# ray-project/xgboost_ray

Measured on NVIDIA H100. Metric: boosting rounds/sec, higher is better.
Workload: dtype int64 fixed-point histograms (int32 shared-memory cells), f64 gain

## Files before the change

xgboost_ray_b200/build.py:

```python
import os
import subprocess
import sys
from concurrent.futures import ThreadPoolExecutor

HERE = os.path.dirname(os.path.abspath(__file__))
CSRC = os.path.join(HERE, "csrc")
OUT = os.path.join(HERE, "libb2hist.so")
OBJ_DIR = os.path.join(CSRC, "build")

NVCC = os.environ.get("NVCC", "/usr/local/cuda/bin/nvcc")
COMMON = ["-gencode", "arch=compute_90a,code=sm_90a", "-O3", "-lineinfo", "-std=c++17",
          "-Xcompiler", "-fPIC,-ffp-contract=off", "-ccbin", "/usr/bin/g++"]
SOURCES = {
    "hist_kernel.cu": [],
    "hist_tma_kernel.cu": [],
    "split_kernel.cu": ["--fmad=false"],
    "partition_kernel.cu": ["--fmad=false"],
    "control_kernel.cu": ["--fmad=false"],
    "objective_kernel.cu": ["--fmad=false"],
    "sketch.cu": ["--fmad=false"],
    "auc_kernel.cu": ["--fmad=false"],
    "p2p_exchange.cu": [],
    "shap_kernel.cu": [],
    "engine.cu": [],
}


def _stale(target, deps):
    if not os.path.exists(target):
        return True
    t = os.path.getmtime(target)
    return any(os.path.getmtime(d) > t for d in deps)


def build(force=False, verbose=False):
    os.makedirs(OBJ_DIR, exist_ok=True)
    headers = [os.path.join(CSRC, "common.cuh"), os.path.join(CSRC, "hist_common.cuh"), os.path.join(CSRC, "sampling.cuh"), os.path.join(CSRC, "p2p.cuh"), os.path.join(CSRC, "level_finalize.cuh"), os.path.join(HERE, "..", "include", "b2hist.h"), __file__]
    jobs = []
    objs = []
    for src, extra in SOURCES.items():
        sp = os.path.join(CSRC, src)
        op = os.path.join(OBJ_DIR, src.replace(".cu", ".o"))
        objs.append(op)
        if force or _stale(op, [sp] + headers):
            jobs.append([NVCC] + COMMON + extra + ["-c", sp, "-o", op])

    def run(cmd):
        if verbose:
            print(" ".join(cmd), flush=True)
        r = subprocess.run(cmd, capture_output=True, text=True)
        if r.returncode != 0:
            raise RuntimeError("nvcc failed:\n%s\n%s\n%s" % (" ".join(cmd), r.stdout, r.stderr))
        return r

    with ThreadPoolExecutor(max_workers=6) as ex:
        list(ex.map(run, jobs))
    if force or jobs or _stale(OUT, objs):
        run([NVCC, "-shared", "-o", OUT] + objs + ["-ldl", "-ccbin", "/usr/bin/g++"])
    return OUT


if __name__ == "__main__":
    print(build(force="--force" in sys.argv, verbose=True))
```

xgboost_ray_b200/csrc/common.cuh:

```cuda
#pragma once
#include <cuda_runtime.h>
#include <stdint.h>

#define B2_GROUP_SLOTS 32
#define B2_BINS 256
#define B2_MISSING_BIN 255
#define B2_PLANE_ELEMS (B2_BINS * B2_GROUP_SLOTS)
#define B2_GROUP_ELEMS (2 * B2_PLANE_ELEMS)

struct B2HistWork {
  int32_t seg_begin;
  int32_t seg_count;
  int32_t hist_index;
  int32_t chunk_begin;
};

#define B2_HIST_MAX_TYPES 8
struct B2HistPlan {
  int32_t n_types;
  int32_t cta_begin[B2_HIST_MAX_TYPES + 1];
  int32_t narrow_w;
};

struct B2SplitWork {
  int32_t seg_begin, seg_count;
  int32_t feature;
  int32_t split_bin;
  int32_t default_left;
  int32_t has_missing;
  int32_t chunk_begin;
  int32_t is_cat;
  uint32_t cat_bits[8];
};

struct B2SplitCand {
  float loss_chg;
  int32_t feature;
  int32_t bin;
  int32_t default_left;
  int64_t left_g, left_h;
  uint32_t order;
  int32_t is_cat;
  uint32_t cat_bits[8];
};

struct B2EvalNode {
  int64_t sum_g, sum_h;
  int32_t hist_index;
  float root_gain;
};

struct B2TreeNodeDev {
  int32_t left, right;
  int32_t feature;
  float cond;
  float value;
  int32_t default_left;
  int32_t cat_slot;
  int32_t pad;
};

#define B2_SHAP_MAX_PATH 16
#define B2_PATH_MISSING_OK 1u
#define B2_PATH_HAS_HI 2u
#define B2_PATH_OUTSIDE_OK 4u
struct B2PathElem {
  int32_t feature;
  int32_t cat_slot;
  float lo, hi;
  uint32_t flags;
  uint32_t pad;
  double zero_fraction;
};
struct B2PathInfo {
  int32_t elem_begin;
  int32_t len;
  int32_t cls;
  int32_t pad;
  double value;
};

__device__ __forceinline__ int b2_tree_step(const B2TreeNodeDev& nd, float v, float missing, int missing_is_nan,
                                            const uint32_t* __restrict__ cat_table) {
  const bool miss = isnan(v) || (!missing_is_nan && v == missing);
  if (miss) return nd.default_left ? nd.left : nd.right;
  if (nd.cat_slot >= 0) {
    bool in_set = false;
    if (v >= 0.0f && v < 256.0f) { const int c = (int)v; in_set = (cat_table[(size_t)nd.cat_slot * 8 + (c >> 5)] >> (c & 31)) & 1u; }
    return in_set ? nd.right : nd.left;
  }
  return v < nd.cond ? nd.left : nd.right;
}

__device__ __forceinline__ int b2_tree_leaf(const B2TreeNodeDev* __restrict__ tn, const float* __restrict__ x, float missing,
                                            int missing_is_nan, const uint32_t* __restrict__ cat_table, float* leaf_value) {
  int nid = 0;
  B2TreeNodeDev nd = tn[0];
  while (nd.feature >= 0) {
    nid = b2_tree_step(nd, x[nd.feature], missing, missing_is_nan, cat_table);
    nd = tn[nid];
  }
  *leaf_value = nd.value;
  return nid;
}

struct B2LevelCtl {
  int32_t n_nodes;
  int32_t n_split;
  int32_t part_chunks;
  int32_t hist_n_work;
  int32_t hist_total_chunks;
  int32_t hist_chunk_rows;
  int32_t n_pairs;
  int32_t leaf_base_next;
};
struct B2NodeSeg { int32_t nid, begin, count, buf; };
struct B2LeafDev { int32_t nid, buf, begin, count; };
struct B2SegWork {
  int32_t seg_begin, seg_count, id, chunk_begin;
  int32_t buf, pad0, pad1, pad2;
};
struct B2TreeDev {
  int32_t *left, *right, *parent, *feature, *split_bin, *default_left, *split_type;
  uint32_t* cat_bits;
  float* loss_chg;
  long long *sum_g, *sum_h;
  float *leaf_weight, *leaf_value;
  int32_t* n_nodes;
};
struct B2CtlParams { double mcw, lambda, alpha, max_delta_step; float gamma, eta; };

struct B2ColSample {
  const uint8_t* level_mask;
  const uint32_t* fwq;
  double bynode;
  int32_t n_level;
  int32_t n_features;
  uint32_t seed, tree;
};

struct B2FinalizeArgs {
  B2LevelCtl* ctl_nxt;
  B2NodeSeg* seg_nxt;
  B2EvalNode* ev_nxt;
  const int32_t* pair_parent_hist;
  B2HistWork* hist_work;
  int32_t* triples;
  long long* stat_rows;
  uint32_t* done;
  int32_t max_pairs, need_hist, n_streams, window_rows, chunk_rows_override;
};

struct B2SiblingSub {
  const long long* parent_level;
  const int32_t* triples;
  long long* sib_out;
  int32_t sib_base;
};

#define B2_P2P_MAX_WORLD 8
enum { kSlotHist = 0, kSlotCand = 1, kSlotAbsmax = 2, kSlotLeaf = 3, kSlotClose = 4, kP2PSlots = 5 };
struct B2P2P {
  long long* build[B2_P2P_MAX_WORLD];
  B2SplitCand* cands[B2_P2P_MAX_WORLD];
  long long* misc[B2_P2P_MAX_WORLD];
  uint32_t* flags[B2_P2P_MAX_WORLD];
  uint32_t* epoch;
  uint32_t* done;
  uint32_t* err;
  const uint32_t* abort_flag;
  int32_t world, rank;
  int32_t cand_cap, misc_stride;
  long long spin_limit;
};

struct B2TrainParamDev {
  double min_child_weight, lambda, alpha;
  double inv_scale_g, inv_scale_h;
  double max_delta_step;
  int32_t max_cat_to_onehot, max_cat_threshold;
};

#ifdef __CUDACC__
__device__ __forceinline__ double b2_thr_l1(double g, double a) {
  if (g > a) return __dadd_rn(g, -a);
  if (g < -a) return __dadd_rn(g, a);
  return 0.0;
}
__device__ __forceinline__ double b2_calc_weight(double G, double H, double mcw, double lambda, double alpha, double mds) {
  if (H < mcw || H <= 0.0) return 0.0;
  const double t = (alpha == 0.0) ? G : b2_thr_l1(G, alpha);
  double dw = __ddiv_rn(-t, __dadd_rn(H, lambda));
  if (mds != 0.0 && fabs(dw) > mds) dw = copysign(mds, dw);
  return dw;
}
__device__ __forceinline__ double b2_calc_gain(double G, double H, double mcw, double lambda, double alpha, double mds) {
  if (H < mcw || H <= 0.0) return 0.0;
  if (mds == 0.0) {
    const double t = (alpha == 0.0) ? G : b2_thr_l1(G, alpha);
    return __ddiv_rn(__dmul_rn(t, t), __dadd_rn(H, lambda));
  }
  const double w = b2_calc_weight(G, H, mcw, lambda, alpha, mds);
  const double ret = -__dadd_rn(__dmul_rn(__dmul_rn(2.0, G), w), __dmul_rn(__dadd_rn(H, lambda), __dmul_rn(w, w)));
  return alpha == 0.0 ? ret : __dadd_rn(ret, __dmul_rn(alpha, fabs(w)));
}
#endif
```

xgboost_ray_b200/csrc/control_kernel.cu:

```cuda
#include <string.h>

#include <cub/block/block_scan.cuh>

#include "common.cuh"
#include "p2p.cuh"

namespace b2 {

constexpr int kCtlThreads = 1024;
constexpr int kPartChunkRows = 2048;
constexpr int kSplitChunkRows = 8192;

__device__ __forceinline__ double c_calc_gain(double G, double H, const B2CtlParams& p) {
  return b2_calc_gain(G, H, p.mcw, p.lambda, p.alpha, p.max_delta_step);
}
__device__ __forceinline__ float c_calc_weight(double G, double H, const B2CtlParams& p) {
  return __double2float_rn(b2_calc_weight(G, H, p.mcw, p.lambda, p.alpha, p.max_delta_step));
}

struct TileScan {
  typedef cub::BlockScan<int, kCtlThreads> Scan;
  Scan::TempStorage* tmp;
  int carry;
  __device__ TileScan(Scan::TempStorage* t) : tmp(t), carry(0) {}
  __device__ int step(int v) {
    int ex, total;
    Scan(*tmp).ExclusiveSum(v, ex, total);
    __syncthreads();
    int r = carry + ex;
    carry += total;
    return r;
  }
};

__global__ void __launch_bounds__(kCtlThreads)
decide_kernel(B2LevelCtl* __restrict__ ctl_cur, B2LevelCtl* __restrict__ ctl_nxt, const B2NodeSeg* __restrict__ seg_cur,
              B2NodeSeg* __restrict__ seg_nxt, const B2EvalNode* __restrict__ ev_cur, B2EvalNode* __restrict__ ev_nxt,
              const B2SplitCand* __restrict__ cands, int cands_per_node, int cand_ranks, int cand_rank_stride, int can_split,
              B2TreeDev tree,
              B2SplitWork* __restrict__ split_work, int32_t* __restrict__ pair_parent_hist, B2LeafDev* __restrict__ leaves,
              int32_t* __restrict__ n_leaves, const uint8_t* __restrict__ has_missing, const int32_t* __restrict__ qexp,
              int qbits, B2CtlParams p, int32_t* __restrict__ part_counters, const B2SplitCand* __restrict__ local_cands,
              int use_p2p, B2P2P pp) {
  __shared__ typename TileScan::Scan::TempStorage tmp;
  __shared__ int s_node_base, s_leaf_base;
  const int n = ctl_cur->n_nodes;
  if (part_counters) for (int i = threadIdx.x; i < 2 * n; i += kCtlThreads) part_counters[i] = 0;
  if (use_p2p && can_split) {
    constexpr int kWords = sizeof(B2SplitCand) / 8;
    static_assert(sizeof(B2SplitCand) % 8 == 0, "candidates are copied as 64-bit words");
    const uint32_t epoch = p2p_next_epoch(pp, kSlotCand);
    const int total = n * cands_per_node * kWords;
    for (int w = 0; w < pp.world; ++w) {
      long long* dst = reinterpret_cast<long long*>(pp.cands[w] + (size_t)pp.rank * pp.cand_cap);
      for (int t = threadIdx.x; t < total; t += kCtlThreads) st_volatile_u64(dst + t, reinterpret_cast<const long long*>(local_cands)[t]);
    }
    __syncthreads();
    p2p_signal(pp, kSlotCand, epoch);
    p2p_wait(pp, kSlotCand, epoch);
    p2p_finish_single(pp, kSlotCand, epoch);
  }
  const double inv_sg = ldexp(1.0, qexp[0] - qbits), inv_sh = ldexp(1.0, qexp[1] - qbits);
  if (threadIdx.x == 0) { s_node_base = *tree.n_nodes; s_leaf_base = *n_leaves; }
  __syncthreads();
  TileScan scan_split(&tmp), scan_leaf(&tmp), scan_chunks(&tmp);
  for (int base = 0; base < n; base += kCtlThreads) {
    const int i = base + threadIdx.x;
    const bool in = i < n;
    B2SplitCand best; best.feature = -1; best.loss_chg = 0.f; best.order = 0xffffffffu; best.bin = 0; best.default_left = 0;
    best.left_g = 0; best.left_h = 0; best.is_cat = 0;
    B2EvalNode nd; nd.sum_g = 0; nd.sum_h = 0; nd.hist_index = 0; nd.root_gain = 0.f;
    B2NodeSeg sg; sg.nid = 0; sg.begin = 0; sg.count = 0; sg.buf = 0;
    bool expand = false;
    if (in) {
      nd = ev_cur[i]; sg = seg_cur[i];
      if (can_split) {
        for (int w = 0; w < cand_ranks; ++w)
          for (int g = 0; g < cands_per_node; ++g) {
            B2SplitCand c;
            if (use_p2p) {
              constexpr int kW = sizeof(B2SplitCand) / 8;
              const long long* src = reinterpret_cast<const long long*>(cands + (size_t)w * cand_rank_stride + (size_t)i * cands_per_node + g);
#pragma unroll
              for (int t = 0; t < kW; ++t) reinterpret_cast<unsigned long long*>(&c)[t] = ld_volatile_u64(src + t);
            } else c = cands[(size_t)w * cand_rank_stride + (size_t)i * cands_per_node + g];
            if (c.feature < 0) continue;
            if (best.feature < 0 || c.loss_chg > best.loss_chg || (c.loss_chg == best.loss_chg && c.order < best.order)) best = c;
          }
        if (best.feature >= 0)
          expand = best.loss_chg > 1e-6f && best.left_h != 0 && (nd.sum_h - best.left_h) != 0 && !(best.loss_chg < p.gamma);
      }
    }
    const int rank = scan_split.step(expand ? 1 : 0);
    const int lrank = scan_leaf.step((in && !expand) ? 1 : 0);
    const int chunks = expand ? (sg.count + kSplitChunkRows - 1) / kSplitChunkRows : 0;
    const int chunk_begin = scan_chunks.step(chunks);
    if (in && !expand) {
      B2LeafDev lf; lf.nid = sg.nid; lf.buf = sg.buf; lf.begin = sg.begin; lf.count = sg.count;
      leaves[s_leaf_base + lrank] = lf;
    }
    if (expand) {
      const int l = s_node_base + 2 * rank, r = l + 1;
      const int nid = sg.nid;
      tree.left[nid] = l; tree.right[nid] = r; tree.feature[nid] = best.feature; tree.split_bin[nid] = best.bin;
      tree.default_left[nid] = best.default_left; tree.loss_chg[nid] = best.loss_chg;
      tree.split_type[nid] = best.is_cat;
      if (best.is_cat) {
#pragma unroll
        for (int w8 = 0; w8 < 8; ++w8) tree.cat_bits[(size_t)nid * 8 + w8] = best.cat_bits[w8];
      }
      tree.left[l] = -1; tree.right[l] = -1; tree.feature[l] = -1; tree.parent[l] = nid;
      tree.left[r] = -1; tree.right[r] = -1; tree.feature[r] = -1; tree.parent[r] = nid;
      const long long lg = best.left_g, lh = best.left_h, rg = nd.sum_g - lg, rh = nd.sum_h - lh;
      tree.sum_g[l] = lg; tree.sum_h[l] = lh; tree.sum_g[r] = rg; tree.sum_h[r] = rh;
      B2SplitWork sw;
      sw.seg_begin = sg.begin; sw.seg_count = sg.count; sw.feature = best.feature; sw.split_bin = best.bin;
      sw.default_left = best.default_left; sw.has_missing = has_missing[best.feature]; sw.chunk_begin = chunk_begin;
      sw.is_cat = best.is_cat;
#pragma unroll
      for (int w8 = 0; w8 < 8; ++w8) sw.cat_bits[w8] = best.is_cat ? best.cat_bits[w8] : 0u;
      split_work[rank] = sw;
      pair_parent_hist[rank] = nd.hist_index;
      const double GL = __dmul_rn(__ll2double_rn(lg), inv_sg), HL = __dmul_rn(__ll2double_rn(lh), inv_sh);
      const double GR = __dmul_rn(__ll2double_rn(rg), inv_sg), HR = __dmul_rn(__ll2double_rn(rh), inv_sh);
      B2EvalNode el, er;
      el.sum_g = lg; el.sum_h = lh; el.hist_index = -1; el.root_gain = __double2float_rn(c_calc_gain(GL, HL, p));
      er.sum_g = rg; er.sum_h = rh; er.hist_index = -1; er.root_gain = __double2float_rn(c_calc_gain(GR, HR, p));
      ev_nxt[2 * rank] = el; ev_nxt[2 * rank + 1] = er;
      B2NodeSeg sl, sr;
      sl.nid = l; sl.buf = sg.buf ^ 1; sl.begin = sg.begin; sl.count = 0;
      sr.nid = r; sr.buf = sg.buf ^ 1; sr.begin = sg.begin; sr.count = sg.count;
      seg_nxt[2 * rank] = sl; seg_nxt[2 * rank + 1] = sr;
    }
  }
  __syncthreads();
  if (threadIdx.x == 0) {
    const int n_split = scan_split.carry;
    ctl_cur->n_split = n_split; ctl_cur->part_chunks = scan_chunks.carry;
    ctl_cur->leaf_base_next = s_leaf_base + scan_leaf.carry;
    ctl_nxt->n_nodes = 2 * n_split; ctl_nxt->n_split = 0; ctl_nxt->part_chunks = 0;
    ctl_nxt->hist_n_work = 0; ctl_nxt->hist_total_chunks = 0; ctl_nxt->n_pairs = 0;
    *tree.n_nodes = s_node_base + 2 * n_split;
    *n_leaves = s_leaf_base + scan_leaf.carry;
  }
}

__global__ void __launch_bounds__(kCtlThreads)
leaf_plan_kernel(const B2LeafDev* __restrict__ leaves, const int32_t* __restrict__ n_leaves, B2SegWork* __restrict__ work,
                 B2LevelCtl* __restrict__ leaf_ctl) {
  __shared__ typename TileScan::Scan::TempStorage tmp;
  const int n = *n_leaves;
  TileScan scan(&tmp);
  for (int base = 0; base < n; base += kCtlThreads) {
    const int i = base + threadIdx.x;
    int chunks = 0; B2LeafDev lf; lf.nid = 0; lf.buf = 0; lf.begin = 0; lf.count = 0;
    if (i < n) { lf = leaves[i]; chunks = (lf.count + kPartChunkRows - 1) / kPartChunkRows; }
    const int cb = scan.step(chunks);
    if (i < n) {
      B2SegWork w; w.seg_begin = lf.begin; w.seg_count = lf.count; w.id = i; w.chunk_begin = cb; w.buf = lf.buf;
      w.pad0 = lf.nid == 0 ? 1 : 0;
      w.pad1 = w.pad2 = 0; work[i] = w;
    }
  }
  __syncthreads();
  if (threadIdx.x == 0) { leaf_ctl->hist_n_work = n; leaf_ctl->hist_total_chunks = scan.carry; }
}

__global__ void leaf_values_kernel(const B2LeafDev* __restrict__ leaves, const int32_t* __restrict__ n_leaves,
                                   const long long* __restrict__ sums, const int32_t* __restrict__ qexp, int leaf_bits,
                                   B2CtlParams p, float* __restrict__ leaf_value, B2TreeDev tree, int32_t* __restrict__ qexp_out) {
  const int n = *n_leaves;
  if (blockIdx.x == 0 && threadIdx.x < 2) qexp_out[threadIdx.x] = qexp[threadIdx.x];
  const double kg = ldexp(1.0, leaf_bits - qexp[0]), kh = ldexp(1.0, leaf_bits - qexp[1]);
  for (int i = blockIdx.x * blockDim.x + threadIdx.x; i < n; i += gridDim.x * blockDim.x) {
    const double G = __ddiv_rn(__ll2double_rn(sums[2 * i]), kg), H = __ddiv_rn(__ll2double_rn(sums[2 * i + 1]), kh);
    const float w = c_calc_weight(G, H, p);
    const float v = __fmul_rn(w, p.eta);
    leaf_value[i] = v;
    tree.leaf_weight[leaves[i].nid] = w;
    tree.leaf_value[leaves[i].nid] = v;
  }
}

__global__ void tree_init_kernel(B2TreeDev tree, B2LevelCtl* ctl0, B2NodeSeg* seg0, B2EvalNode* ev0, int32_t* n_leaves,
                                 int n_rows, B2HistWork* hist_work0) {
  if (threadIdx.x == 0 && blockIdx.x == 0) {
    B2HistWork hw; hw.seg_begin = 0; hw.seg_count = n_rows; hw.hist_index = 0; hw.chunk_begin = 0; hist_work0[0] = hw;
    ctl0->leaf_base_next = 0;
    *tree.n_nodes = 1; *n_leaves = 0;
    tree.left[0] = -1; tree.right[0] = -1; tree.parent[0] = -1; tree.feature[0] = -1;
    ctl0->n_nodes = 1; ctl0->n_split = 0; ctl0->part_chunks = 0; ctl0->hist_n_work = 0; ctl0->hist_total_chunks = 0;
    ctl0->n_pairs = 0;
    B2NodeSeg s; s.nid = 0; s.buf = 0; s.begin = 0; s.count = n_rows; seg0[0] = s;
    B2EvalNode e; e.sum_g = 0; e.sum_h = 0; e.hist_index = 0; e.root_gain = 0.f; ev0[0] = e;
  }
}

}

extern "C" {
int b2_launch_decide(B2LevelCtl* ctl_cur, B2LevelCtl* ctl_nxt, const B2NodeSeg* seg_cur, B2NodeSeg* seg_nxt,
                     const B2EvalNode* ev_cur, B2EvalNode* ev_nxt, const B2SplitCand* cands, int cands_per_node, int cand_ranks,
                     int cand_rank_stride, int can_split, B2TreeDev tree, B2SplitWork* split_work, int32_t* pair_parent_hist, B2LeafDev* leaves, int32_t* n_leaves,
                     const uint8_t* has_missing, const int32_t* qexp, int qbits, B2CtlParams p, int32_t* part_counters,
                     const B2SplitCand* local_cands, const void* p2p, cudaStream_t s) {
  B2P2P pp;
  if (p2p) pp = *reinterpret_cast<const B2P2P*>(p2p); else memset(&pp, 0, sizeof(pp));
  b2::decide_kernel<<<1, b2::kCtlThreads, 0, s>>>(ctl_cur, ctl_nxt, seg_cur, seg_nxt, ev_cur, ev_nxt, cands, cands_per_node,
                                                 cand_ranks, cand_rank_stride, can_split, tree, split_work, pair_parent_hist, leaves, n_leaves, has_missing, qexp, qbits, p,
                                                 part_counters, local_cands, p2p ? 1 : 0, pp);
  return (int)cudaGetLastError();
}
int b2_launch_leaf_plan(const B2LeafDev* leaves, const int32_t* n_leaves, B2SegWork* work, B2LevelCtl* leaf_ctl, cudaStream_t s) {
  b2::leaf_plan_kernel<<<1, b2::kCtlThreads, 0, s>>>(leaves, n_leaves, work, leaf_ctl);
  return (int)cudaGetLastError();
}
int b2_launch_leaf_values(const B2LeafDev* leaves, const int32_t* n_leaves, const long long* sums, const int32_t* qexp,
                          int leaf_bits, B2CtlParams p, float* leaf_value, B2TreeDev tree, int32_t* qexp_out, cudaStream_t s) {
  b2::leaf_values_kernel<<<8, 256, 0, s>>>(leaves, n_leaves, sums, qexp, leaf_bits, p, leaf_value, tree, qexp_out);
  return (int)cudaGetLastError();
}
int b2_launch_tree_init(B2TreeDev tree, B2LevelCtl* ctl0, B2NodeSeg* seg0, B2EvalNode* ev0, int32_t* n_leaves, int n_rows,
                        B2HistWork* hist_work0, cudaStream_t s) {
  b2::tree_init_kernel<<<1, 32, 0, s>>>(tree, ctl0, seg0, ev0, n_leaves, n_rows, hist_work0);
  return (int)cudaGetLastError();
}
}
```

xgboost_ray_b200/csrc/engine.cu:

```cuda
#include <cuda_runtime.h>
#include <dlfcn.h>
#include <errno.h>
#include <sys/types.h>
#include <sys/uio.h>
#include <math.h>
#include <stdarg.h>
#include <stdio.h>
#include <stdlib.h>
#include <string.h>

#include <algorithm>
#include <atomic>
#include <chrono>
#include <map>
#include <mutex>
#include <set>
#include <string>
#include <thread>
#include <vector>

#include "../../include/b2hist.h"
#include "common.cuh"
#include "sampling.cuh"

extern "C" {
int b2_launch_hist(const uint8_t*, int, const int2*, const int32_t*, const B2HistWork*, int, int, int, int, int, long long*,
                   const B2LevelCtl*, int, int, int, int, cudaStream_t);
int b2_make_bins_tensor_map(void*, const uint8_t*, int64_t, int, int);
int b2_launch_hist_tma(const uint8_t*, int, const void*, const int2*, const int32_t*, const B2HistWork*, int, int, int, int, int, long long*,
                       const B2LevelCtl*, int, int, int64_t, int, cudaStream_t);
int b2_launch_hist_subtract(const long long*, long long*, const int32_t*, int, int64_t, const B2LevelCtl*, cudaStream_t);
int b2_launch_eval_splits(const long long*, int, const B2EvalNode*, int, const int32_t*, const int32_t*, const int32_t*,
                          const uint8_t*, const uint8_t*, const int32_t*, int, B2TrainParamDev, B2SplitCand*, int, const B2LevelCtl*,
                          int, int, B2ColSample, const B2NodeSeg*, B2SiblingSub, cudaStream_t);
int b2_launch_subsample(float2*, int64_t, uint32_t, uint32_t, uint32_t, double, int, cudaStream_t);
int b2_p2p_flag_words(int);
int b2_launch_p2p_reduce_subtract(const void*, const long long*, long long*, const int32_t*, const B2LevelCtl*, int, int, int64_t, int,
                                  cudaStream_t);
int b2_launch_p2p_quant_exponent(const void*, const uint32_t*, int32_t*, cudaStream_t);
int b2_launch_p2p_leaf_sums(const void*, const int32_t*, long long*, cudaStream_t);
int b2_hist_variant();
int b2_launch_p2p_close(const void*, cudaStream_t);
int b2_launch_gather_interleaved_rows(const void*, float*, int, cudaStream_t);
int b2_launch_final_assign(const uint8_t*, int64_t, const int32_t*, const B2SplitWork*, const B2LevelCtl*, int, const float2*,
                           const int32_t*, int, long long*, uint16_t*, int, int, cudaStream_t);
int b2_launch_margin_update(float*, int, int, const uint16_t*, const float*, int64_t, int, cudaStream_t);
int b2_leaf_acc_max_depth();
int b2_launch_leaf_accumulate(const float2*, const uint16_t*, int64_t, int, const int32_t*, int, long long*, int, cudaStream_t);
int b2_gradient_fused_max_classes();
int b2_launch_sum_fixed(const float2*, int64_t, const int32_t*, int, long long*, int, cudaStream_t);
int b2_cat_ctas();
int b2_launch_eval_cat_splits(const long long*, int, const B2EvalNode*, int, const int32_t*, int, const int32_t*, const int32_t*,
                              const int32_t*, int, B2TrainParamDev, B2SplitCand*, int, int, const B2LevelCtl*, int, int,
                              B2ColSample, const B2NodeSeg*, cudaStream_t);
int b2_launch_cat_stats(const float*, int64_t, int, float, const int32_t*, int, int32_t*, int, cudaStream_t);
int b2_launch_root_totals(const long long*, int, B2EvalNode*, const int32_t*, int, B2TrainParamDev, int, long long*, long long*,
                          cudaStream_t);
int b2_part_chunk_rows();
int b2_split_chunk_rows();
int b2_launch_partition(const uint8_t*, int64_t, const int32_t*, int32_t*, const B2SplitWork*, const B2LevelCtl*, int, int32_t*,
                        int, B2FinalizeArgs, int, cudaStream_t);
int b2_launch_leaf_sums(const float2*, const int32_t*, const int32_t*, const void*, const B2LevelCtl*, int, const int32_t*, int,
                        long long*, uint16_t*, int, cudaStream_t);
int b2_launch_pred_update(float*, int, int, const int32_t*, const int32_t*, const void*, const B2LevelCtl*, int, const float*, int,
                          cudaStream_t);
int b2_launch_decide(B2LevelCtl*, B2LevelCtl*, const B2NodeSeg*, B2NodeSeg*, const B2EvalNode*, B2EvalNode*, const B2SplitCand*,
                     int, int, int, int, B2TreeDev, B2SplitWork*, int32_t*, B2LeafDev*, int32_t*, const uint8_t*, const int32_t*, int,
                     B2CtlParams, int32_t*, const B2SplitCand*, const void*, cudaStream_t);
int b2_launch_leaf_plan(const B2LeafDev*, const int32_t*, B2SegWork*, B2LevelCtl*, cudaStream_t);
int b2_launch_leaf_values(const B2LeafDev*, const int32_t*, const long long*, const int32_t*, int, B2CtlParams, float*, B2TreeDev,
                          int32_t*, cudaStream_t);
int b2_launch_tree_init(B2TreeDev, B2LevelCtl*, B2NodeSeg*, B2EvalNode*, int32_t*, int, B2HistWork*, cudaStream_t);
int b2_launch_iota(int32_t*, int64_t, cudaStream_t);
int b2_launch_gradient(int, int, const float*, const float*, const float*, int64_t, float, float, float2*, uint32_t*, uint32_t*, int,
                       cudaStream_t);
int b2_launch_label_check(int, const float*, int64_t, uint32_t*, int, cudaStream_t);
int b2_launch_pack_custom(const float*, const float*, int, int64_t, float2*, int, cudaStream_t);
int b2_launch_absmax(const float2*, int64_t, uint32_t*, int, cudaStream_t);
int b2_launch_quant_exponent(const uint32_t*, int32_t*, cudaStream_t);
int b2_launch_quantize(const float2*, int64_t, const int32_t*, int, int2*, int, cudaStream_t);
int b2_launch_metric(int, int, int, float, const float*, const float*, const float*, int64_t, double*, int, cudaStream_t);
int b2_launch_predict(const float*, int64_t, int, float, const B2TreeNodeDev*, const int32_t*, const uint32_t*, int, int, int, int,
                      float*, int, cudaStream_t);
int b2_launch_fill(float*, int64_t, float, int, cudaStream_t);
size_t b2_shap_contribs_smem(int, int, int);
int b2_launch_shap_contribs(const float*, int64_t, int64_t, int, float, const B2PathElem*, const B2PathInfo*, int, int,
                            const uint32_t*, int, const double*, const float*, float, double*, int, size_t, float*, int, cudaStream_t);
int b2_launch_shap_interactions(const float*, int64_t, int64_t, int, float, const B2PathElem*, const B2PathInfo*, int, int,
                                const uint32_t*, int, const double*, const float*, float, double*, float*, int, cudaStream_t);
int b2_launch_leaf_index(const float*, int64_t, int64_t, int, float, const B2TreeNodeDev*, const int32_t*, const uint32_t*, int, int,
                         float*, int, cudaStream_t);
size_t b2_auc_temp_bytes(int64_t);
int b2_auc_binary(const float*, const float*, const float*, int64_t, void*, size_t, double*, int, cudaStream_t);
int b2_launch_transform(int, int, float*, int64_t, int, cudaStream_t);
int b2_extract_batch();
int b2_launch_extract_keys(const float*, int64_t, int, int, int, float, uint32_t*, int64_t, int, cudaStream_t);
size_t b2_sort_temp_bytes(int64_t);
int b2_sketch_column(const uint32_t*, const int32_t*, uint32_t*, int32_t*, long long*, int64_t, long long, void*, size_t, int32_t*,
                     int32_t*, float*, long long*, int32_t*, long long*, int, float*, int32_t*, float*, int32_t*, int, cudaStream_t);
int b2_launch_weight_absmax(const float*, int64_t, uint32_t*, int, cudaStream_t);
int b2_launch_weight_quantize(const float*, int64_t, int64_t, const uint32_t*, int32_t*, int, cudaStream_t);
int b2_launch_bin(const float*, int64_t, int, float, const int32_t*, const float*, const int32_t*, const uint8_t*, int, uint8_t*,
                  uint8_t*, int64_t, int, cudaStream_t);
}

namespace {

thread_local std::string g_last_error;
struct B2Error { std::string msg; };
[[noreturn]] void fail(const char* fmt, ...) {
  char buf[1024];
  va_list ap; va_start(ap, fmt); vsnprintf(buf, sizeof(buf), fmt, ap); va_end(ap);
  throw B2Error{buf};
}
#define CUDA_CHECK(expr)                                                                       \
  do {                                                                                         \
    cudaError_t e_ = (expr);                                                                   \
    if (e_ != cudaSuccess) fail("CUDA error %s at %s:%d: %s", cudaGetErrorName(e_), __FILE__, __LINE__, cudaGetErrorString(e_)); \
  } while (0)
#define LAUNCH_CHECK(expr)                                                                     \
  do {                                                                                         \
    int e_ = (expr);                                                                           \
    if (e_ != 0) fail("kernel launch failed (%s) at %s:%d", cudaGetErrorString((cudaError_t)e_), __FILE__, __LINE__); \
  } while (0)
#define API_BEGIN try {
#define API_END                                            \
  }                                                        \
  catch (const B2Error& e) { g_last_error = e.msg; return -1; } \
  catch (const std::exception& e) { g_last_error = e.what(); return -1; } \
  return 0;

struct Ctx {
  int device = -1;
  cudaStream_t stream = nullptr;
  int num_sms = 0;
};
std::mutex g_ctx_mu;
std::map<int, Ctx*> g_ctx;
Ctx* get_ctx(int device) {
  std::lock_guard<std::mutex> lk(g_ctx_mu);
  auto it = g_ctx.find(device);
  if (it != g_ctx.end()) { CUDA_CHECK(cudaSetDevice(device)); return it->second; }
  int n = 0;
  cudaError_t e = cudaGetDeviceCount(&n);
  if (e != cudaSuccess || n == 0) fail("no CUDA device available (%s): libb2hist has no CPU fallback", cudaGetErrorString(e));
  if (device < 0 || device >= n) fail("invalid device %d (have %d)", device, n);
  CUDA_CHECK(cudaSetDevice(device));
  Ctx* c = new Ctx();
  c->device = device;
  CUDA_CHECK(cudaStreamCreateWithFlags(&c->stream, cudaStreamNonBlocking));
  cudaDeviceProp prop;
  CUDA_CHECK(cudaGetDeviceProperties(&prop, device));
  if (prop.major != 9 || prop.minor != 0)
    fail("device %d is sm_%d%d; this engine is built for sm_90a (H100) only", device, prop.major, prop.minor);
  c->num_sms = prop.multiProcessorCount;
  g_ctx[device] = c;
  return c;
}

struct DevPool {
  std::mutex mu;
  std::multimap<size_t, void*> free_blocks;
  size_t cached = 0;
};
DevPool g_dev_pool[64];
size_t pool_cap_bytes() {
  static size_t cap = 0;
  if (!cap) { const char* e = getenv("B2_POOL_MAX_GB"); double gb = e ? atof(e) : 24.0; cap = (size_t)(gb < 0 ? 0 : gb * 1e9) + 1; }
  return cap;
}
void pool_trim(DevPool& pool, size_t keep) {
  while (pool.cached > keep && !pool.free_blocks.empty()) {
    auto it = std::prev(pool.free_blocks.end());
    cudaFree(it->second);
    pool.cached -= it->first;
    pool.free_blocks.erase(it);
  }
}
void* pool_alloc(size_t bytes, size_t* got, int* dev_out) {
  int dev = 0; cudaGetDevice(&dev);
  if (dev < 0 || dev >= 64) dev = 0;
  *dev_out = dev;
  bytes = (bytes + 511) & ~(size_t)511;
  DevPool& pool = g_dev_pool[dev];
  {
    std::lock_guard<std::mutex> lk(pool.mu);
    auto it = pool.free_blocks.lower_bound(bytes);
    if (it != pool.free_blocks.end() && it->first <= bytes + bytes / 4 + ((size_t)1 << 20)) {
      void* p = it->second; *got = it->first;
      pool.cached -= it->first;
      pool.free_blocks.erase(it);
      return p;
    }
  }
  void* p = nullptr;
  cudaError_t e = cudaMalloc(&p, bytes);
  if (e != cudaSuccess) {
    cudaGetLastError();
    { std::lock_guard<std::mutex> lk(pool.mu); pool_trim(pool, 0); }
    e = cudaMalloc(&p, bytes);
  }
  if (e != cudaSuccess) { cudaGetLastError(); fail("cudaMalloc of %zu bytes failed: %s", bytes, cudaGetErrorString(e)); }
  *got = bytes;
  return p;
}
void pool_free(void* p, size_t bytes, int dev) {
  if (!p) return;
  if (dev < 0 || dev >= 64) dev = 0;
  DevPool& pool = g_dev_pool[dev];
  std::lock_guard<std::mutex> lk(pool.mu);
  if (bytes > pool_cap_bytes()) { cudaFree(p); return; }
  pool.free_blocks.emplace(bytes, p);
  pool.cached += bytes;
  if (pool.cached > pool_cap_bytes()) pool_trim(pool, pool_cap_bytes() / 2);
}

template <typename T>
struct DevBuf {
  T* p = nullptr;
  size_t cap = 0;
  size_t block_bytes = 0;
  int dev = 0;
  void ensure(size_t n) {
    if (n <= cap) return;
    release();
    size_t got = 0;
    p = (T*)pool_alloc(n * sizeof(T), &got, &dev);
    block_bytes = got;
    cap = n;
  }
  void release() { if (p) pool_free(p, block_bytes, dev); p = nullptr; cap = 0; block_bytes = 0; }
  ~DevBuf() { release(); }
};

struct PinnedPool {
  static constexpr int kWorkers = 16, kSlots = 2;
  static constexpr size_t kSlice = (size_t)8 << 20;
  void* buf[kWorkers][kSlots] = {};
  cudaStream_t stream[kWorkers] = {};
  cudaEvent_t done[kWorkers][kSlots] = {};
  bool ready = false;
  std::mutex mu;
  int n_init = 0;
  void init(int n) {
    for (int w = n_init; w < n; ++w) {
      CUDA_CHECK(cudaStreamCreateWithFlags(&stream[w], cudaStreamNonBlocking));
      for (int k = 0; k < kSlots; ++k) {
        CUDA_CHECK(cudaMallocHost(&buf[w][k], kSlice));
        CUDA_CHECK(cudaEventCreateWithFlags(&done[w][k], cudaEventDisableTiming));
      }
      n_init = w + 1;
    }
  }
};
std::map<int, PinnedPool*> g_pools;

struct UploadSource {
  const void* src = nullptr;
  long long pid = 0;
  uint64_t remote_addr = 0;
  size_t row_bytes = 0, row_stride = 0;
};
bool fetch_slice(const UploadSource& u, void* dst, size_t off, size_t len, std::string* err) {
  if (u.pid == 0) { memcpy(dst, (const char*)u.src + off, len); return true; }
  if (u.row_stride == u.row_bytes) {
    size_t done = 0;
    while (done < len) {
      struct iovec l = {(char*)dst + done, len - done}, r = {(void*)(uintptr_t)(u.remote_addr + off + done), len - done};
      const ssize_t got = process_vm_readv((pid_t)u.pid, &l, 1, &r, 1, 0);
      if (got <= 0) { if (err) *err = std::string("process_vm_readv: ") + strerror(errno); return false; }
      done += (size_t)got;
    }
    return true;
  }
  constexpr size_t kSpan = (size_t)4 << 20;
  static thread_local std::vector<char> scratch;
  if (scratch.size() < kSpan + u.row_stride) scratch.resize(kSpan + u.row_stride);
  const size_t rows_per_batch = std::max<size_t>(1, kSpan / u.row_stride);
  size_t done = 0;
  while (done < len) {
    const size_t pos = off + done, row0 = pos / u.row_bytes;
    const size_t last_byte = std::min(off + len, (row0 + rows_per_batch) * u.row_bytes) - 1;
    const size_t row1 = last_byte / u.row_bytes;
    const size_t span = (row1 - row0) * u.row_stride + u.row_bytes;
    size_t got_total = 0;
    while (got_total < span) {
      struct iovec l = {scratch.data() + got_total, span - got_total};
      struct iovec r = {(void*)(uintptr_t)(u.remote_addr + row0 * u.row_stride + got_total), span - got_total};
      const ssize_t got = process_vm_readv((pid_t)u.pid, &l, 1, &r, 1, 0);
      if (got <= 0) { if (err) *err = std::string("process_vm_readv: ") + strerror(errno); return false; }
      got_total += (size_t)got;
    }
    for (size_t row = row0; row <= row1; ++row) {
      const size_t b0 = std::max(pos, row * u.row_bytes), b1 = std::min(off + len, (row + 1) * u.row_bytes);
      memcpy((char*)dst + (b0 - off), scratch.data() + (row - row0) * u.row_stride + (b0 - row * u.row_bytes), b1 - b0);
    }
    done = std::min(off + len, (row1 + 1) * u.row_bytes) - off;
  }
  return true;
}

void upload_pipelined(Ctx* ctx, void* dst, const UploadSource& u, size_t bytes);
void upload_pipelined(Ctx* ctx, void* dst, const void* src, size_t bytes) {
  UploadSource u; u.src = src;
  upload_pipelined(ctx, dst, u, bytes);
}
void upload_pipelined(Ctx* ctx, void* dst, const UploadSource& u, size_t bytes) {
  const void* src = u.src;
  if (u.pid == 0 && bytes < ((size_t)64 << 20)) {
    if (bytes) CUDA_CHECK(cudaMemcpyAsync(dst, src, bytes, cudaMemcpyHostToDevice, ctx->stream));
    CUDA_CHECK(cudaStreamSynchronize(ctx->stream));
    return;
  }
  PinnedPool* pool;
  {
    std::lock_guard<std::mutex> lk(g_ctx_mu);
    PinnedPool*& p = g_pools[ctx->device];
    if (!p) p = new PinnedPool();
    pool = p;
  }
  std::lock_guard<std::mutex> lk(pool->mu);
  CUDA_CHECK(cudaStreamSynchronize(ctx->stream));
  const size_t n_slices = (bytes + PinnedPool::kSlice - 1) / PinnedPool::kSlice;
  static int n_workers = 0;
  if (n_workers == 0) {
    const char* e = getenv("B2_UPLOAD_WORKERS");
    n_workers = e ? atoi(e) : 8;
    if (n_workers < 1) n_workers = 1;
    if (n_workers > PinnedPool::kWorkers) n_workers = PinnedPool::kWorkers;
  }
  const int W = n_workers;
  pool->init(W);
  std::atomic<int> failed{0};
  std::mutex err_mu; std::string fetch_err;
  auto worker = [&](int w) {
    if (cudaSetDevice(ctx->device) != cudaSuccess) { failed = 1; return; }
    int use = 0;
    for (size_t i = w; i < n_slices; i += W, ++use) {
      const int k = use % PinnedPool::kSlots;
      const size_t off = i * PinnedPool::kSlice, len = std::min(PinnedPool::kSlice, bytes - off);
      if (use >= PinnedPool::kSlots && cudaEventSynchronize(pool->done[w][k]) != cudaSuccess) { failed = 1; return; }
      std::string e;
      if (!fetch_slice(u, pool->buf[w][k], off, len, &e)) { std::lock_guard<std::mutex> lk(err_mu); fetch_err = e; failed = 2; return; }
      if (cudaMemcpyAsync((char*)dst + off, pool->buf[w][k], len, cudaMemcpyHostToDevice, pool->stream[w]) != cudaSuccess ||
          cudaEventRecord(pool->done[w][k], pool->stream[w]) != cudaSuccess) { failed = 1; return; }
    }
    if (cudaStreamSynchronize(pool->stream[w]) != cudaSuccess) failed = 1;
  };
  std::vector<std::thread> th;
  for (int w = 0; w < W; ++w) th.emplace_back(worker, w);
  for (auto& t : th) t.join();
  if (failed.load() == 2) fail("reading the shard out of the driver process failed: %s", fetch_err.c_str());
  if (failed.load()) fail("pipelined host->device upload failed: %s", cudaGetErrorString(cudaGetLastError()));
}

typedef struct ncclComm* ncclComm_t;
typedef struct { char internal[128]; } ncclUniqueId;
enum { kNcclSum = 0, kNcclMax = 2, kNcclMin = 3 };
enum { kNcclUint8 = 1, kNcclInt32 = 2, kNcclUint32 = 3, kNcclInt64 = 4, kNcclUint64 = 5, kNcclFloat32 = 7, kNcclFloat64 = 8 };
struct NcclApi {
  void* lib = nullptr;
  int (*GetUniqueId)(ncclUniqueId*) = nullptr;
  int (*CommInitRank)(ncclComm_t*, int, ncclUniqueId, int) = nullptr;
  int (*AllReduce)(const void*, void*, size_t, int, int, ncclComm_t, cudaStream_t) = nullptr;
  int (*AllGather)(const void*, void*, size_t, int, ncclComm_t, cudaStream_t) = nullptr;
  int (*ReduceScatter)(const void*, void*, size_t, int, int, ncclComm_t, cudaStream_t) = nullptr;
  int (*CommAbort)(ncclComm_t) = nullptr;
  int (*CommDestroy)(ncclComm_t) = nullptr;
  const char* (*GetErrorString)(int) = nullptr;
};
NcclApi* nccl() {
// ... 98 lines not shown
  m->feat_byte.assign(F, 0);
  m->narrow_w = 0;
  const int r = F % B2_GROUP_SLOTS;
  const bool v4_layout = b2_hist_variant() == 4 && F > 96 && F <= 112;
  const bool narrow = (narrow_on || v4_layout) && r > 0 && r <= 16;
  if (narrow) { m->narrow_w = 1; while (m->narrow_w < r) m->narrow_w <<= 1; }
  const int base = F / m->n_groups, rem = F % m->n_groups;
  int f = 0;
  for (int g = 0; g < m->n_groups; ++g) {
    const int sz = narrow ? (g + 1 < m->n_groups ? B2_GROUP_SLOTS : r) : base + (g < rem ? 1 : 0);
    m->group_first[g] = f; m->group_size[g] = sz;
    for (int s = 0; s < sz; ++s) m->feat_byte[f + s] = g * B2_GROUP_SLOTS + s;
    f += sz;
  }
}

template <typename T>
void upload(DevBuf<T>& d, const std::vector<T>& h, cudaStream_t s) {
  d.ensure(h.size() ? h.size() : 1);
  if (!h.empty()) CUDA_CHECK(cudaMemcpyAsync(d.p, h.data(), h.size() * sizeof(T), cudaMemcpyHostToDevice, s));
}

void upload_cuts(Matrix* m) {
  cudaStream_t s = m->ctx->stream;
  m->nbins.resize(m->F);
  for (int f = 0; f < m->F; ++f) m->nbins[f] = m->cut_ptrs[f + 1] - m->cut_ptrs[f];
  upload(m->d_group_first, m->group_first, s); upload(m->d_group_size, m->group_size, s);
  upload(m->d_feat_byte, m->feat_byte, s); upload(m->d_cut_ptrs, m->cut_ptrs, s);
  upload(m->d_cut_vals, m->cut_vals, s); upload(m->d_nbins, m->nbins, s);
  upload(m->d_has_missing, m->has_missing, s);
  if (m->is_cat.empty()) m->is_cat.assign(m->F, 0);
  upload(m->d_is_cat, m->is_cat, s); upload(m->d_cat_feats, m->cat_feats, s);
  CUDA_CHECK(cudaStreamSynchronize(s));
}

void make_cuts(Matrix* m, Comm* comm, int max_bin) {
  Ctx* ctx = m->ctx; cudaStream_t s = ctx->stream;
  if (max_bin < 2 || max_bin > 256) fail("max_bin must be in [2, 256] (uint8 bin matrix), got %d", max_bin);
  if (!m->has_raw) fail("matrix has no raw data to sketch");
  const int world = comm ? comm->world : 1, rank = comm ? comm->rank : 0;
  DevBuf<long long> d_cnt; d_cnt.ensure(2);
  long long h_cnt[2] = {m->n, m->n};
  if (world > 1) {
    CUDA_CHECK(cudaMemcpyAsync(d_cnt.p, h_cnt, sizeof(h_cnt), cudaMemcpyHostToDevice, s));
    allreduce(comm, d_cnt.p, 1, kNcclInt64, kNcclMax, s);
    allreduce(comm, d_cnt.p + 1, 1, kNcclInt64, kNcclSum, s);
    CUDA_CHECK(cudaMemcpyAsync(h_cnt, d_cnt.p, sizeof(h_cnt), cudaMemcpyDeviceToHost, s));
    CUDA_CHECK(cudaStreamSynchronize(s));
  }
  const int64_t n_pad = h_cnt[0], n_total = n_pad * world; const long long n_global = h_cnt[1];
  const int B = b2_extract_batch(); const int F = m->F;
  DevBuf<uint32_t> keys_local, keys_all, keys_sorted;
  DevBuf<int32_t> flags, idx, m_scratch; DevBuf<float> uval; DevBuf<long long> rmin, nvalid;
  DevBuf<int32_t> d_tab;
  DevBuf<uint8_t> temp;
  const size_t nt = (size_t)std::max<int64_t>(n_total, 1);
  keys_local.ensure((size_t)std::max<int64_t>(n_pad, 1) * B);
  if (world > 1) keys_all.ensure(nt);
  keys_sorted.ensure(nt); flags.ensure(nt); idx.ensure(nt); uval.ensure(nt); rmin.ensure(nt); m_scratch.ensure(1); nvalid.ensure(2);
  DevBuf<int32_t> wq_local, wq_all, wq_sorted; DevBuf<long long> wpre; DevBuf<uint32_t> d_wmax;
  const int32_t* wq = nullptr;
  {
    long long h_has[1] = {m->n_weight > 0 ? 1 : 0};
    if (world > 1) {
      CUDA_CHECK(cudaMemcpyAsync(d_cnt.p, h_has, sizeof(h_has), cudaMemcpyHostToDevice, s));
      allreduce(comm, d_cnt.p, 1, kNcclInt64, kNcclMax, s);
      CUDA_CHECK(cudaMemcpyAsync(h_has, d_cnt.p, sizeof(h_has), cudaMemcpyDeviceToHost, s));
      CUDA_CHECK(cudaStreamSynchronize(s));
    }
    if (h_has[0]) {
      if (m->n_weight != m->n) fail("sample weights are set on some ranks only (this rank has %lld for %lld rows)", (long long)m->n_weight, (long long)m->n);
      d_wmax.ensure(2);
      CUDA_CHECK(cudaMemsetAsync(d_wmax.p, 0, 2 * sizeof(uint32_t), s));
      LAUNCH_CHECK(b2_launch_weight_absmax(m->weight.p, m->n, d_wmax.p, ctx->num_sms, s));
      allreduce(comm, d_wmax.p, 2, kNcclUint32, kNcclMax, s);
      uint32_t h_w[2];
      CUDA_CHECK(cudaMemcpyAsync(h_w, d_wmax.p, sizeof(h_w), cudaMemcpyDeviceToHost, s));
      CUDA_CHECK(cudaStreamSynchronize(s));
      if (h_w[1]) fail("sample weights must be finite and non-negative");
      wq_local.ensure((size_t)std::max<int64_t>(n_pad, 1));
      LAUNCH_CHECK(b2_launch_weight_quantize(m->weight.p, m->n, n_pad, d_wmax.p, wq_local.p, ctx->num_sms, s));
      wq = wq_local.p;
      if (world > 1) {
        wq_all.ensure(nt);
        NCCL_CHECK(nccl()->AllGather(wq_local.p, wq_all.p, (size_t)n_pad, kNcclInt32, comm->comm, s));
        wq = wq_all.p;
      }
      wq_sorted.ensure(nt); wpre.ensure(nt);
    }
  }
  const size_t temp_bytes = b2_sort_temp_bytes(n_total > 0 ? n_total : 1);
  temp.ensure(temp_bytes ? temp_bytes : 1);
  const size_t tab_n = (size_t)F * 256 + 3 * (size_t)F;
  d_tab.ensure(tab_n);
  CUDA_CHECK(cudaMemsetAsync(d_tab.p, 0, tab_n * sizeof(int32_t), s));
  float* d_cuts = (float*)d_tab.p; int32_t* d_ncuts = d_tab.p + (size_t)F * 256;
  float* d_mins = (float*)(d_ncuts + F); int32_t* d_hasmiss = d_ncuts + 2 * (size_t)F;
  if (m->is_cat.empty()) m->is_cat.assign(F, 0);
  for (int f0 = 0; f0 < F; f0 += B) {
    const int nf = std::min(B, F - f0);
    bool any_numeric = false;
    for (int j = 0; j < nf; ++j) any_numeric = any_numeric || !m->is_cat[f0 + j];
    if (!any_numeric) continue;
    LAUNCH_CHECK(b2_launch_extract_keys(m->raw.p, m->n, F, f0, nf, m->missing, keys_local.p, n_pad, ctx->num_sms, s));
    for (int j = 0; j < nf; ++j) {
      const int f = f0 + j;
      if (m->is_cat[f]) continue;
      const uint32_t* kin = keys_local.p + (size_t)j * n_pad;
      if (world > 1) {
        NCCL_CHECK(nccl()->AllGather(kin, keys_all.p, (size_t)n_pad, kNcclUint32, comm->comm, s));
        kin = keys_all.p;
        if (f % world != rank) continue;
      }
      LAUNCH_CHECK(b2_sketch_column(kin, wq, keys_sorted.p, wq_sorted.p, wpre.p, n_total, n_global, temp.p, temp_bytes, flags.p, idx.p, uval.p, rmin.p,
                                    m_scratch.p, nvalid.p, max_bin, d_cuts + (size_t)f * 256, d_ncuts + f, d_mins + f,
                                    d_hasmiss + f, ctx->num_sms, s));
    }
  }
  allreduce(comm, d_tab.p, tab_n, kNcclInt32, kNcclSum, s);
  std::vector<int32_t> h_tab(tab_n);
  CUDA_CHECK(cudaMemcpyAsync(h_tab.data(), d_tab.p, tab_n * sizeof(int32_t), cudaMemcpyDeviceToHost, s));
  const int n_cat = (int)m->cat_feats.size();
  std::vector<int32_t> h_cat((size_t)std::max(n_cat, 1) * 3, 0);
  DevBuf<int32_t> d_cat, d_catf;
  if (n_cat > 0) {
    for (int i = 0; i < n_cat; ++i) { h_cat[i * 3] = -1; h_cat[i * 3 + 1] = 0; h_cat[i * 3 + 2] = 0; }
    d_cat.ensure((size_t)n_cat * 3); d_catf.ensure((size_t)n_cat);
    CUDA_CHECK(cudaMemcpyAsync(d_cat.p, h_cat.data(), (size_t)n_cat * 3 * sizeof(int32_t), cudaMemcpyHostToDevice, s));
    CUDA_CHECK(cudaMemcpyAsync(d_catf.p, m->cat_feats.data(), (size_t)n_cat * sizeof(int32_t), cudaMemcpyHostToDevice, s));
    LAUNCH_CHECK(b2_launch_cat_stats(m->raw.p, m->n, F, m->missing, d_catf.p, n_cat, d_cat.p, ctx->num_sms, s));
    allreduce(comm, d_cat.p, (size_t)n_cat * 3, kNcclInt32, kNcclMax, s);
    CUDA_CHECK(cudaMemcpyAsync(h_cat.data(), d_cat.p, (size_t)n_cat * 3 * sizeof(int32_t), cudaMemcpyDeviceToHost, s));
  }
  CUDA_CHECK(cudaStreamSynchronize(s));
  for (int i = 0; i < n_cat; ++i) {
    const int f = m->cat_feats[i], mx = h_cat[i * 3], miss = h_cat[i * 3 + 1];
    if (h_cat[i * 3 + 2] || (miss && mx > 254))
      fail("categorical feature %d: category codes must be integers in [0, %d]%s", f, miss ? 254 : 255,
           miss ? " (the feature has missing values; bin 255 is the missing sentinel)" : "");
    int32_t* t = h_tab.data();
    float* cuts_f = (float*)t + (size_t)f * 256;
    const int nc = mx < 0 ? 1 : mx + 1;
    for (int k = 0; k < nc; ++k) cuts_f[k] = (float)k;
    t[(size_t)F * 256 + f] = nc;
    ((float*)(t + (size_t)F * 256 + F))[f] = -1e-5f;
    t[(size_t)F * 256 + 2 * (size_t)F + f] = miss;
  }
  const float* h_cuts = (const float*)h_tab.data(); const int32_t* h_nc = h_tab.data() + (size_t)F * 256;
  const float* h_mins = (const float*)(h_nc + F); const int32_t* h_hm = h_nc + 2 * (size_t)F;
  m->cut_ptrs.assign(F + 1, 0);
  m->cut_vals.clear(); m->min_vals.assign(h_mins, h_mins + F); m->has_missing.assign(F, 0);
  for (int f = 0; f < F; ++f) {
    if (h_nc[f] < 1 || h_nc[f] > 256) fail("sketch produced %d cuts for feature %d", h_nc[f], f);
    m->cut_ptrs[f + 1] = m->cut_ptrs[f] + h_nc[f];
    m->cut_vals.insert(m->cut_vals.end(), h_cuts + (size_t)f * 256, h_cuts + (size_t)f * 256 + h_nc[f]);
    m->has_missing[f] = h_hm[f] ? 1 : 0;
  }
  m->max_bin = max_bin;
}

void bin_matrix(Matrix* m) {
  Ctx* ctx = m->ctx; cudaStream_t s = ctx->stream;
  setup_groups(m);
  upload_cuts(m);
  m->bins.ensure((size_t)std::max<int64_t>(m->n, 1) * m->row_stride);
  CUDA_CHECK(cudaMemsetAsync(m->bins.p, 0, (size_t)std::max<int64_t>(m->n, 1) * m->row_stride, s));
  m->col_stride = (std::max<int64_t>(m->n, 1) + 127) & ~(int64_t)127;
  m->bins_col.ensure((size_t)m->col_stride * m->F);
  LAUNCH_CHECK(b2_launch_bin(m->raw.p, m->n, m->F, m->missing, m->d_cut_ptrs.p, m->d_cut_vals.p, m->d_feat_byte.p,
                             m->any_cat() ? m->d_is_cat.p : nullptr, m->row_stride, m->bins.p, m->bins_col.p, m->col_stride,
                             ctx->num_sms, s));
  CUDA_CHECK(cudaStreamSynchronize(s));
  m->has_tmap = b2_make_bins_tensor_map(m->tmap_tile, m->bins.p, m->n, m->row_stride, 64) == 0;
  m->quantized = true;
}

enum { kObjSquaredError = 0, kObjLogistic = 1, kObjSoftprob = 2, kObjRegLogistic = 3, kObjLogitRaw = 4, kObjSquaredLog = 5,
       kObjPseudoHuber = 6, kObjPoisson = 7, kObjGamma = 8, kObjTweedie = 9 };
bool obj_log_link(int o) { return o == kObjPoisson || o == kObjGamma || o == kObjTweedie; }
bool obj_sigmoid(int o) { return o == kObjLogistic || o == kObjRegLogistic; }
bool obj_checks_finite(int o) { return o >= kObjSquaredLog; }
struct Params {
  int objective = kObjSquaredError;
  std::string objective_name = "reg:squarederror";
  int num_class = 1;
  int num_parallel_tree = 1;
  int max_depth = 6;
  float eta = 0.3f, gamma = 0.0f, min_child_weight = 1.0f, lambda = 1.0f, alpha = 0.0f, base_score = 0.5f;
  int qbits = 18;
  int hist_chunk_rows = 0;
  int profile = 1;
  int num_feature = 0;
  int device = 0;
  int max_cat_to_onehot = 4, max_cat_threshold = 64;
  float scale_pos_weight = 1.0f, max_delta_step = 0.0f;
  bool max_delta_step_set = false;
  float huber_slope = 1.0f;
  float tweedie_variance_power = 1.5f;
  float subsample = 1.0f, colsample_bytree = 1.0f, colsample_bylevel = 1.0f, colsample_bynode = 1.0f;
  int seed = 0;
  bool base_score_set = false;
  bool use_cols() const { return colsample_bytree < 1.0f || colsample_bylevel < 1.0f || colsample_bynode < 1.0f; }
};

struct TreeHost {
  std::vector<int32_t> left, right, parent, feature, split_bin;
  std::vector<float> cond, value, base_weight, loss_chg;
  std::vector<double> sum_hess;
  std::vector<uint8_t> default_left;
  std::vector<uint8_t> split_type;
  std::vector<uint32_t> cat_bits;
  bool any_cat = false;
  int add(int par) {
    int id = (int)left.size();
    left.push_back(-1); right.push_back(-1); parent.push_back(par); feature.push_back(-1); split_bin.push_back(-1);
    cond.push_back(0.f); value.push_back(0.f); base_weight.push_back(0.f); loss_chg.push_back(0.f); sum_hess.push_back(0.0);
    default_left.push_back(0); split_type.push_back(0); cat_bits.insert(cat_bits.end(), 8, 0u);
    return id;
  }
  int size() const { return (int)left.size(); }
};


struct Timers {
  double hist_ms = 0, round_ms = 0;
  double shap_ms = 0;
  long long shap_rows = 0;
  double phase_ms[8] = {0, 0, 0, 0, 0, 0, 0, 0};
  long long hist_launches = 0, hist_rows = 0, kernel_launches = 0, rounds = 0;
  double hist_bytes = 0, allreduce_bytes = 0;
  void reset() { *this = Timers(); }
};

struct EvalCache { DevBuf<float> margin; int n_trees_applied = 0; int64_t n = 0; uint64_t margin_version = 0; };

struct Booster : HandleBase {
  Ctx* ctx = nullptr;
  Params p;
  Matrix* train = nullptr;
  int n_features = 0;
  Comm* comm = nullptr;
  std::vector<TreeHost> trees;
  std::atomic<bool> cancel{false};
  DevBuf<B2TreeNodeDev> d_nodes; DevBuf<int32_t> d_tree_offset; int d_trees_synced = 0;
  std::vector<B2TreeNodeDev> h_nodes; std::vector<int32_t> h_tree_offset;
  DevBuf<uint32_t> d_cat_table; std::vector<uint32_t> h_cat_table;
  DevBuf<B2PathElem> d_path_elems; DevBuf<B2PathInfo> d_paths; DevBuf<uint32_t> d_path_cats;
  std::vector<int32_t> tree_path_offset;
  std::vector<double> tree_expected;
  int paths_synced = -1;
  bool margin_ready = false;
  DevBuf<float> margin;
  DevBuf<float2> gh;
  DevBuf<float2> gh_round;
  DevBuf<int2> q;
  DevBuf<int32_t> ridx[2];
  DevBuf<long long> hist[2];
  template <typename T> struct View { T* p = nullptr; };
  DevBuf<uint8_t> xarena;
  size_t xoff_cands = 0, xoff_misc = 0, xoff_flags = 0, x_misc_stride = 0;
  View<long long> hist_build;
  View<B2SplitCand> d_cands_all;
  int shards = 1, log2_shards = 0, sp = 32, cpn = 1;
  int cpn_num = 1;
  View<uint32_t> t_cat;
  DevBuf<uint8_t> d_col_masks;
  struct P2PState {
    bool enabled = false, tried = false;
    B2P2P pp;
    DevBuf<uint32_t> words;
    uint32_t* flags = nullptr;
    long long* misc = nullptr;
    std::vector<void*> opened;
    int cand_cap = 0;
  } p2p;
  struct TreeGraph {
    cudaGraphExec_t exec = nullptr;
    std::vector<std::pair<cudaEvent_t, cudaEvent_t>> hist_ev;
    long long hist_launches = 0, kernel_launches = 0;
    double allreduce_bytes = 0;
  };
  std::map<int, TreeGraph> graphs;
  std::map<int, int> direct_trees;
  bool graph_failed = false;
  bool absmax_fused = false;
  bool labels_checked = false;
  DevBuf<uint32_t> d_grad_err;
  uint32_t* h_grad_err = nullptr;
  DevBuf<uint16_t> pos;
  size_t slice_elems = 0;
  size_t node_elems = 0;
  DevBuf<uint32_t> d_absmax; DevBuf<int32_t> d_qexp;
  int ctl_depth = 0;
  DevBuf<uint8_t> t_block;
  View<int32_t> t_i32;
  View<float> t_f32;
  View<long long> t_i64;
  View<int32_t> t_qexp;
  DevBuf<B2LevelCtl> d_ctl;
  DevBuf<B2NodeSeg> d_seg[2]; DevBuf<B2EvalNode> d_ev[2];
  DevBuf<B2HistWork> d_hist_work; DevBuf<B2SplitWork> d_split_work; DevBuf<B2SegWork> d_seg_work;
  DevBuf<B2SplitCand> d_cands; DevBuf<int32_t> d_counters, d_triples, d_pair_parent;
  DevBuf<uint32_t> d_part_done;
  DevBuf<B2LeafDev> d_leaves;
  DevBuf<long long> d_leaf_sums; DevBuf<float> d_leaf_values; DevBuf<double> d_metric;
  std::vector<void*> staging;
  size_t staging_bytes = 0;
  DevBuf<float> d_custom_g, d_custom_h;
  std::map<uint64_t, EvalCache*> eval_cache;
  Timers t;
  std::vector<cudaEvent_t> ev_pool; size_t ev_used = 0;
  std::vector<std::pair<cudaEvent_t, cudaEvent_t>> hist_events;
  std::vector<std::pair<int, cudaEvent_t>> phase_marks;
  cudaEvent_t round_start = nullptr, round_stop = nullptr;
  ~Booster() {
    for (auto& kv : graphs) {
      if (kv.second.exec) cudaGraphExecDestroy(kv.second.exec);
      for (auto& pr : kv.second.hist_ev) { cudaEventDestroy(pr.first); cudaEventDestroy(pr.second); }
    }
    if (ctx) cudaStreamSynchronize(ctx->stream);
    for (void* q : p2p.opened) cudaIpcCloseMemHandle(q);
    for (auto e : ev_pool) cudaEventDestroy(e);
    if (round_start) cudaEventDestroy(round_start);
    if (round_stop) cudaEventDestroy(round_stop);
    for (auto& kv : eval_cache) delete kv.second;
    for (void* h : staging) cudaFreeHost(h);
    if (h_grad_err) cudaFreeHost(h_grad_err);
  }
};

cudaEvent_t get_event(Booster* b) {
  if (b->ev_used == b->ev_pool.size()) { cudaEvent_t e; CUDA_CHECK(cudaEventCreate(&e)); b->ev_pool.push_back(e); }
  return b->ev_pool[b->ev_used++];
}
void mark_phase(Booster* b, int phase) {
  if (b->p.profile < 2) return;
  cudaEvent_t e = get_event(b);
  CUDA_CHECK(cudaEventRecord(e, b->ctx->stream));
  b->phase_marks.push_back({phase, e});
}
void resolve_events(Booster* b) {
  for (size_t i = 1; i < b->phase_marks.size(); ++i) {
    float ms = 0.f;
    if (b->phase_marks[i].first >= 0 && cudaEventElapsedTime(&ms, b->phase_marks[i - 1].second, b->phase_marks[i].second) == cudaSuccess)
      b->t.phase_ms[b->phase_marks[i].first] += ms;
  }
  b->phase_marks.clear();
  for (auto& pr : b->hist_events) {
    float ms = 0.f;
    if (cudaEventElapsedTime(&ms, pr.first, pr.second) == cudaSuccess) b->t.hist_ms += ms;
  }
  b->hist_events.clear();
  b->ev_used = 0;
}

void parse_params(const char* text, Params* p, int* max_bin_out) {
  std::string s(text ? text : "");
  size_t pos = 0;
  while (pos < s.size()) {
    size_t nl = s.find('\n', pos);
    if (nl == std::string::npos) nl = s.size();
    std::string line = s.substr(pos, nl - pos);
    pos = nl + 1;
    size_t eq = line.find('=');
    if (eq == std::string::npos) continue;
    std::string k = line.substr(0, eq), v = line.substr(eq + 1);
    auto f = [&]() { return (float)atof(v.c_str()); };
    auto i = [&]() { return atoi(v.c_str()); };
    if (k == "objective") {
      p->objective_name = v;
      if (v == "reg:squarederror" || v == "reg:linear") p->objective = kObjSquaredError;
      else if (v == "binary:logistic") p->objective = kObjLogistic;
      else if (v == "multi:softprob" || v == "multi:softmax") p->objective = kObjSoftprob;
      else if (v == "reg:logistic") p->objective = kObjRegLogistic;
      else if (v == "binary:logitraw") p->objective = kObjLogitRaw;
      else if (v == "reg:squaredlogerror") p->objective = kObjSquaredLog;
      else if (v == "reg:pseudohubererror") p->objective = kObjPseudoHuber;
      else if (v == "count:poisson") p->objective = kObjPoisson;
      else if (v == "reg:gamma") p->objective = kObjGamma;
      else if (v == "reg:tweedie") p->objective = kObjTweedie;
      else fail("unsupported objective '%s' (supported: reg:squarederror, reg:logistic, binary:logistic, binary:logitraw, "
                "reg:squaredlogerror, reg:pseudohubererror, count:poisson, reg:gamma, reg:tweedie, multi:softprob, "
                "multi:softmax)", v.c_str());
    } else if (k == "num_class") p->num_class = i();
    else if (k == "num_parallel_tree") p->num_parallel_tree = i();
    else if (k == "max_depth") p->max_depth = i();
    else if (k == "eta" || k == "learning_rate") p->eta = f();
    else if (k == "gamma" || k == "min_split_loss") p->gamma = f();
    else if (k == "min_child_weight") p->min_child_weight = f();
    else if (k == "lambda" || k == "reg_lambda") p->lambda = f();
    else if (k == "alpha" || k == "reg_alpha") p->alpha = f();
    else if (k == "base_score") { p->base_score = f(); p->base_score_set = true; }
    else if (k == "hist_qbits") p->qbits = i();
    else if (k == "hist_chunk_rows") p->hist_chunk_rows = i();
    else if (k == "profile") p->profile = i();
    else if (k == "num_feature") p->num_feature = i();
    else if (k == "device") p->device = i();
    else if (k == "subsample") p->subsample = f();
    else if (k == "colsample_bytree") p->colsample_bytree = f();
    else if (k == "colsample_bylevel") p->colsample_bylevel = f();
    else if (k == "colsample_bynode") p->colsample_bynode = f();
    else if (k == "seed" || k == "random_state") p->seed = i();
    else if (k == "scale_pos_weight") p->scale_pos_weight = f();
    else if (k == "max_delta_step") { p->max_delta_step = f(); p->max_delta_step_set = true; }
    else if (k == "huber_slope") p->huber_slope = f();
    else if (k == "tweedie_variance_power") p->tweedie_variance_power = f();
    else if (k == "max_cat_to_onehot") p->max_cat_to_onehot = i();
    else if (k == "max_cat_threshold") p->max_cat_threshold = i();
    else if (k == "max_bin") { if (max_bin_out) *max_bin_out = i(); }
  }
  if (p->objective != kObjSoftprob) p->num_class = 1;
  if (p->objective == kObjSoftprob && p->num_class < 2) fail("multi:softprob needs num_class >= 2");
  if (p->max_depth < 1 || p->max_depth > 14) fail("max_depth must be in [1, 14], got %d", p->max_depth);
  if (p->num_parallel_tree < 1 || p->num_parallel_tree > 4096) fail("num_parallel_tree must be in [1, 4096], got %d", p->num_parallel_tree);
  if (p->qbits < 8 || p->qbits > 24) fail("hist_qbits must be in [8, 24], got %d", p->qbits);
  for (float v : {p->subsample, p->colsample_bytree, p->colsample_bylevel, p->colsample_bynode})
    if (!(v > 0.0f && v <= 1.0f)) fail("subsample / colsample_* must be in (0, 1], got %g", (double)v);
  if (p->max_cat_to_onehot < 1) fail("max_cat_to_onehot must be >= 1, got %d", p->max_cat_to_onehot);
  if (p->max_cat_threshold < 1) fail("max_cat_threshold must be >= 1, got %d", p->max_cat_threshold);
  if (p->objective == kObjPoisson) {
    if (!p->max_delta_step_set) p->max_delta_step = 0.7f;
    if (!(p->max_delta_step >= 0.0f)) fail("max_delta_step must be >= 0 for count:poisson, got %g", (double)p->max_delta_step);
  }
  if (p->objective == kObjPseudoHuber && !(p->huber_slope > 0.0f))
    fail("huber_slope must be > 0 for reg:pseudohubererror, got %g", (double)p->huber_slope);
  if (p->objective == kObjTweedie && !(p->tweedie_variance_power >= 1.0f && p->tweedie_variance_power < 2.0f))
    fail("tweedie_variance_power must be in [1, 2), got %g", (double)p->tweedie_variance_power);
  if (p->base_score_set) {
    if (p->objective == kObjRegLogistic && !(p->base_score > 0.0f && p->base_score < 1.0f))
      fail("base_score must be in (0, 1) for reg:logistic, got %g", (double)p->base_score);
    if (obj_log_link(p->objective) && !(p->base_score > 0.0f))
      fail("base_score must be > 0 for %s, got %g", p->objective_name.c_str(), (double)p->base_score);
  }
}

float objective_param(const Params& p) {
  if (p.objective == kObjPseudoHuber) return p.huber_slope;
  if (p.objective == kObjPoisson) return p.max_delta_step;
  if (p.objective == kObjTweedie) return p.tweedie_variance_power;
  return 0.0f;
}

float base_margin_value(const Params& p) {
  if (obj_sigmoid(p.objective)) return -logf(1.0f / p.base_score - 1.0f);
  if (obj_log_link(p.objective)) return logf(p.base_score);
  return p.base_score;
}

double h_thr_l1(double g, double a) { if (g > a) return g - a; if (g < -a) return g + a; return 0.0; }
float h_calc_weight(const Params& p, double G, double H) {
  if (H < (double)p.min_child_weight || H <= 0.0) return 0.0f;
  double t = p.alpha == 0.0f ? G : h_thr_l1(G, (double)p.alpha);
  double dw = -t / (H + (double)p.lambda);
  if (p.max_delta_step != 0.0f && fabs(dw) > (double)p.max_delta_step) dw = copysign((double)p.max_delta_step, dw);
  return (float)dw;
}

int window_rows_for(int qbits) {
  return 1 << (30 - qbits);
}

int pick_chunk_rows(Booster* b, int64_t rows) {
  if (b->p.hist_chunk_rows > 0) return b->p.hist_chunk_rows;
  const int n_streams = std::max(1, b->ctx->num_sms * 3 / b->train->n_groups);
  const int64_t per_stream = rows / n_streams;
  int64_t target = per_stream >= 16384 ? per_stream / 4 : per_stream;
  int c = 512;
  while (c < target && c < 8192) c <<= 1;
  const int w = window_rows_for(b->p.qbits);
  if (c > w) c = w;
  return c;
}

struct TreeLayout {
  size_t max_nodes, i32_count, f32_count, i64_count, bytes;
  size_t off_f32, off_i64, off_qexp, off_cat;
};
TreeLayout tree_layout(int max_depth) {
  TreeLayout L;
  L.max_nodes = ((size_t)1 << (max_depth + 1));
  L.i32_count = 7 * L.max_nodes + 2;
  L.f32_count = 3 * L.max_nodes;
  L.i64_count = 2 * L.max_nodes + (size_t)max_depth + 2;
  L.off_f32 = L.i32_count * 4;
  L.off_i64 = (L.off_f32 + L.f32_count * 4 + 7) & ~(size_t)7;
  L.off_qexp = L.off_i64 + L.i64_count * 8;
  L.off_cat = L.off_qexp + 16;
  L.bytes = L.off_cat + L.max_nodes * 8 * sizeof(uint32_t);
  return L;
}
B2TreeDev tree_dev(Booster* b) {
  const TreeLayout L = tree_layout(b->ctl_depth);
  B2TreeDev t;
  int32_t* i = b->t_i32.p; const size_t m = L.max_nodes;
  t.left = i; t.right = i + m; t.parent = i + 2 * m; t.feature = i + 3 * m; t.split_bin = i + 4 * m; t.default_left = i + 5 * m;
  t.split_type = i + 6 * m;
  t.n_nodes = i + 7 * m;
  t.cat_bits = b->t_cat.p;
  t.loss_chg = b->t_f32.p; t.leaf_weight = b->t_f32.p + m; t.leaf_value = b->t_f32.p + 2 * m;
  t.sum_g = b->t_i64.p; t.sum_h = b->t_i64.p + m;
  return t;
}

int p2p_timeout_seconds() {
  const char* e = getenv("B2_P2P_TIMEOUT_S");
  int v = e ? atoi(e) : 60;
  return v < 1 ? 1 : v;
}
void p2p_setup(Booster* b) {
  Booster::P2PState& st = b->p2p;
  if (st.tried || b->shards <= 1) return;
  st.tried = true;
  const char* env = getenv("B2_EXCHANGE");
  if (env && (strcmp(env, "nccl") == 0 || strcmp(env, "NCCL") == 0)) return;
  Comm* c = b->comm; cudaStream_t s = b->ctx->stream; const int W = c->world;
  if (W > B2_P2P_MAX_WORLD) return;
  const size_t misc_stride = b->x_misc_stride;
  const size_t n_flags = (size_t)b2_p2p_flag_words(W), n_words = 2 * (size_t)kP2PSlots + 2;
  st.words.ensure(n_words);
  CUDA_CHECK(cudaMemsetAsync(st.flags, 0, n_flags * sizeof(uint32_t), s));
  CUDA_CHECK(cudaMemsetAsync(st.words.p, 0, n_words * sizeof(uint32_t), s));
  CUDA_CHECK(cudaMemsetAsync(st.misc, 0, (size_t)W * misc_stride * sizeof(long long), s));
  cudaIpcMemHandle_t mine; int ok = 1;
  if (cudaIpcGetMemHandle(&mine, b->xarena.p) != cudaSuccess) { ok = 0; cudaGetLastError(); memset(&mine, 0, sizeof(mine)); }
  DevBuf<uint8_t> d_mine, d_all; d_mine.ensure(sizeof(mine)); d_all.ensure(sizeof(mine) * (size_t)W);
  CUDA_CHECK(cudaMemcpyAsync(d_mine.p, &mine, sizeof(mine), cudaMemcpyHostToDevice, s));
  NCCL_CHECK(nccl()->AllGather(d_mine.p, d_all.p, sizeof(mine), kNcclUint8, c->comm, s));
  std::vector<cudaIpcMemHandle_t> all((size_t)W);
  CUDA_CHECK(cudaMemcpyAsync(all.data(), d_all.p, sizeof(mine) * (size_t)W, cudaMemcpyDeviceToHost, s));
  CUDA_CHECK(cudaStreamSynchronize(s));
  memset(&st.pp, 0, sizeof(st.pp));
  st.pp.world = W; st.pp.rank = c->rank; st.pp.cand_cap = st.cand_cap; st.pp.misc_stride = (int32_t)misc_stride;
  st.pp.epoch = st.words.p; st.pp.done = st.words.p + kP2PSlots; st.pp.err = st.words.p + 2 * kP2PSlots;
  st.pp.abort_flag = c->d_abort ? c->d_abort : st.words.p + 2 * kP2PSlots + 1;
  st.pp.spin_limit = (long long)p2p_timeout_seconds() * 1000000LL;
  for (int w = 0; w < W && ok; ++w) {
    uint8_t* base = b->xarena.p;
    if (w != c->rank) {
      void* q = nullptr;
      if (cudaIpcOpenMemHandle(&q, all[w], cudaIpcMemLazyEnablePeerAccess) != cudaSuccess) { ok = 0; cudaGetLastError(); break; }
      st.opened.push_back(q);
      base = (uint8_t*)q;
    }
    st.pp.build[w] = (long long*)base; st.pp.cands[w] = (B2SplitCand*)(base + b->xoff_cands);
    st.pp.misc[w] = (long long*)(base + b->xoff_misc); st.pp.flags[w] = (uint32_t*)(base + b->xoff_flags);
  }
  DevBuf<int32_t> d_ok; d_ok.ensure(1);
  int32_t neg = ok ? 0 : 1;
  CUDA_CHECK(cudaMemcpyAsync(d_ok.p, &neg, sizeof(neg), cudaMemcpyHostToDevice, s));
  allreduce(c, d_ok.p, 1, kNcclInt32, kNcclMax, s);
  CUDA_CHECK(cudaMemcpyAsync(&neg, d_ok.p, sizeof(neg), cudaMemcpyDeviceToHost, s));
  CUDA_CHECK(cudaStreamSynchronize(s));
  if (neg) {
    for (void* q : st.opened) cudaIpcCloseMemHandle(q);
    st.opened.clear();
    if (getenv("B2_EXCHANGE")) fprintf(stderr, "[b2hist] peer mapping failed on some rank; histogram exchange stays on NCCL\n");
    return;
  }
  st.enabled = true;
}

void ensure_ctl_tables(Booster* b) {
  const int D = b->p.max_depth; const int G = b->train->n_groups;
  if (b->ctl_depth == D) return;
  if (b->ctl_depth != 0 && b->p2p.enabled) fail("max_depth cannot change while the peer-memory exchange is mapped");
  for (auto& kv : b->graphs) {
    if (kv.second.exec) cudaGraphExecDestroy(kv.second.exec);
    for (auto& pr : kv.second.hist_ev) { cudaEventDestroy(pr.first); cudaEventDestroy(pr.second); }
  }
  b->graphs.clear(); b->direct_trees.clear();
  b->ctl_depth = D;
  const TreeLayout L = tree_layout(D);
  const size_t lcap = (size_t)1 << D, half = (size_t)1 << (D > 0 ? D - 1 : 0);
  b->t_block.ensure(L.bytes);
  b->t_i32.p = (int32_t*)b->t_block.p; b->t_f32.p = (float*)(b->t_block.p + L.off_f32);
  b->t_i64.p = (long long*)(b->t_block.p + L.off_i64); b->t_qexp.p = (int32_t*)(b->t_block.p + L.off_qexp);
  b->t_cat.p = (uint32_t*)(b->t_block.p + L.off_cat);
  b->d_ctl.ensure(3);
  for (int k = 0; k < 2; ++k) { b->d_seg[k].ensure(lcap); b->d_ev[k].ensure(lcap); }
  b->d_hist_work.ensure(half); b->d_split_work.ensure(half);
  b->d_counters.ensure(2 * half); b->d_triples.ensure(3 * half); b->d_pair_parent.ensure(half);
  if (!b->d_part_done.p) { b->d_part_done.ensure(1); CUDA_CHECK(cudaMemsetAsync(b->d_part_done.p, 0, sizeof(uint32_t), b->ctx->stream)); }
  b->d_leaves.ensure(L.max_nodes); b->d_seg_work.ensure(L.max_nodes);
  b->d_leaf_sums.ensure(2 * lcap); b->d_leaf_values.ensure(lcap);
  b->node_elems = (size_t)G * B2_GROUP_ELEMS;
  const int world = b->comm ? b->comm->world : 1;
  b->shards = (world > 1 && world <= 32 && (32 % world) == 0) ? world : 1;
  b->log2_shards = 0; while ((1 << b->log2_shards) < b->shards) b->log2_shards++;
  b->sp = B2_GROUP_SLOTS / b->shards;
  b->slice_elems = (size_t)G * 2 * B2_BINS * b->sp;
  b->cpn_num = (G * b->sp + 31) / 32;
  b->cpn = b->cpn_num + (b->train->any_cat() ? b2_cat_ctas() : 0);
  b->hist[0].ensure(half * b->slice_elems); b->hist[1].ensure(half * b->slice_elems);
  if (b->shards > 1) {
    auto up = [](size_t v) { return (v + 255) & ~(size_t)255; };
    const size_t build_bytes = up(half * b->node_elems * sizeof(long long));
    const size_t cands_bytes = up(half * b->cpn * b->shards * sizeof(B2SplitCand));
    b->x_misc_stride = 2 + 2 * lcap;
    const size_t misc_bytes = up((size_t)b->shards * b->x_misc_stride * sizeof(long long));
    const size_t flag_bytes = up((size_t)b2_p2p_flag_words(b->shards) * sizeof(uint32_t));
    b->xoff_cands = build_bytes; b->xoff_misc = b->xoff_cands + cands_bytes; b->xoff_flags = b->xoff_misc + misc_bytes;
    b->xarena.ensure(b->xoff_flags + flag_bytes);
    b->hist_build.p = (long long*)b->xarena.p;
    b->d_cands_all.p = (B2SplitCand*)(b->xarena.p + b->xoff_cands);
    b->p2p.misc = (long long*)(b->xarena.p + b->xoff_misc);
    b->p2p.flags = (uint32_t*)(b->xarena.p + b->xoff_flags);
  }
  b->d_cands.ensure(half * b->cpn);
  CUDA_CHECK(cudaMemsetAsync(b->t_i64.p, 0, L.i64_count * 8, b->ctx->stream));
  b->p2p.cand_cap = (int)(half * b->cpn);
  p2p_setup(b);
}

struct TreeStats {
  long long hist_launches = 0, kernel_launches = 0;
  double allreduce_bytes = 0;
  std::vector<std::pair<cudaEvent_t, cudaEvent_t>> hist_ev;
  bool capturing = false;
};
void record_hist_launch(Booster* b, TreeStats& st, cudaEvent_t& e0, cudaEvent_t& e1, bool begin) {
  if (!b->p.profile) return;
  cudaStream_t s = b->ctx->stream;
  if (begin) {
    if (st.capturing) { CUDA_CHECK(cudaEventCreate(&e0)); CUDA_CHECK(cudaEventCreate(&e1)); }
    else { e0 = get_event(b); e1 = get_event(b); }
    CUDA_CHECK(cudaEventRecordWithFlags(e0, s, st.capturing ? cudaEventRecordExternal : cudaEventRecordDefault));
  } else {
    CUDA_CHECK(cudaEventRecordWithFlags(e1, s, st.capturing ? cudaEventRecordExternal : cudaEventRecordDefault));
    st.hist_ev.push_back({e0, e1});
  }
}

bool use_tma_hist() {
  static int v = -1;
  if (v < 0) { const char* e = getenv("B2_HIST_TMA"); v = (e && atoi(e) != 0) ? 1 : 0; }
  return v == 1;
}
bool env_flag(const char* name, bool dflt) {
  const char* e = getenv(name);
  return e ? atoi(e) != 0 : dflt;
}

long long* build_target(Booster* b, long long* level_buf) { return b->shards > 1 ? b->hist_build.p : level_buf; }

void exchange_and_subtract(Booster* b, TreeStats& st, const long long* parent_level, long long* level_buf, const int32_t* triples,
                           const B2LevelCtl* ctl_nxt, int nb, int node_cap) {
  cudaStream_t s = b->ctx->stream;
  const bool multi = b->comm && b->comm->world > 1;
  if (multi && b->comm->aborted.load()) fail("communicator aborted");
  if (multi && b->p2p.enabled) {
    LAUNCH_CHECK(b2_launch_p2p_reduce_subtract(&b->p2p.pp, parent_level, level_buf, triples, ctl_nxt, nb, node_cap,
                                               (int64_t)b->slice_elems, b->ctx->num_sms, s));
    st.allreduce_bytes += (double)nb * b->node_elems * 8 * (b->shards - 1) / b->shards;
    st.kernel_launches++;
    mark_phase(b, 2);
    return;
  }
  if (multi && b->shards > 1) {
    NCCL_CHECK(nccl()->ReduceScatter(b->hist_build.p, level_buf, (size_t)nb * b->slice_elems, kNcclInt64, kNcclSum, b->comm->comm, s));
    st.allreduce_bytes += (double)nb * b->node_elems * 8 * (b->shards - 1) / b->shards;
  } else if (multi) {
    NCCL_CHECK(nccl()->AllReduce(level_buf, level_buf, (size_t)nb * b->node_elems, kNcclInt64, kNcclSum, b->comm->comm, s));
    st.allreduce_bytes += (double)nb * b->node_elems * 8;
  }
  mark_phase(b, 2);
  if (triples) {
    LAUNCH_CHECK(b2_launch_hist_subtract(parent_level, level_buf, triples, nb, (int64_t)b->slice_elems, ctl_nxt, s));
    st.kernel_launches++;
  }
  mark_phase(b, 3);
}

void grow_tree(Booster* b, int k, int slot, TreeStats& st) {
  Matrix* m = b->train; Ctx* ctx = b->ctx; cudaStream_t s = ctx->stream; const Params& p = b->p;
  const int64_t n = m->n; const int K = p.num_class; const int G = m->n_groups; const int D = p.max_depth;
  const float2* gh = b->gh.p + (size_t)k * n;
  ensure_ctl_tables(b);
  const TreeLayout L = tree_layout(D);
  const bool multi = b->comm && b->comm->world > 1;
  const bool p2p = multi && b->p2p.enabled;
  static const bool leaf_fused = env_flag("B2_LEAF_FUSED", true);
  const bool leaf_stream = leaf_fused && D >= 1 && D <= b2_leaf_acc_max_depth();
  const bool sub_in_scan = !p2p && !m->any_cat();
  mark_phase(b, -1);
  const uint32_t tree_index = (uint32_t)b->trees.size() + (uint32_t)slot;
  uint32_t* d_absmax = b->d_absmax.p + 2 * k;
  if (p.subsample < 1.0f) {
    LAUNCH_CHECK(b2_launch_subsample(b->gh.p + (size_t)k * n, n, (uint32_t)p.seed, tree_index, b->comm ? (uint32_t)b->comm->rank : 0u,
                                     (double)p.subsample, ctx->num_sms, s));
    st.kernel_launches++;
  }
  std::vector<int> n_level_feats(D > 0 ? D : 1, m->F);
  if (p.use_cols()) {
    const int F = m->F;
    const uint32_t* fwq = m->fwq.empty() ? nullptr : m->fwq.data();
    std::vector<uint8_t> mask_tree(F), masks((size_t)std::max(D, 1) * F);
    for (int f = 0; f < F; ++f)
      mask_tree[f] = b2_col_selected((uint32_t)p.seed, tree_index, B2_SCOPE_TREE, f, nullptr, fwq, F, b2_sample_count((double)p.colsample_bytree, F));
    int n_tree = 0; for (int f = 0; f < F; ++f) n_tree += mask_tree[f];
    for (int d = 0; d < D; ++d) {
      int cnt = 0;
      for (int f = 0; f < F; ++f) {
        masks[(size_t)d * F + f] = b2_col_selected((uint32_t)p.seed, tree_index, B2_SCOPE_LEVEL(d), f, mask_tree.data(), fwq, F,
                                                   b2_sample_count((double)p.colsample_bylevel, n_tree));
        cnt += masks[(size_t)d * F + f];
      }
      n_level_feats[d] = cnt;
    }
    b->d_col_masks.ensure(masks.size());
    CUDA_CHECK(cudaMemcpyAsync(b->d_col_masks.p, masks.data(), masks.size(), cudaMemcpyHostToDevice, s));
  }
  if (!b->absmax_fused) {
    CUDA_CHECK(cudaMemsetAsync(d_absmax, 0, 2 * sizeof(uint32_t), s));
    LAUNCH_CHECK(b2_launch_absmax(gh, n, d_absmax, ctx->num_sms, s));
    st.kernel_launches++;
  }
  if (p2p) LAUNCH_CHECK(b2_launch_p2p_quant_exponent(&b->p2p.pp, d_absmax, b->d_qexp.p, s));
  else {
    allreduce(b->comm, d_absmax, 2, kNcclUint32, kNcclMax, s);
    LAUNCH_CHECK(b2_launch_quant_exponent(d_absmax, b->d_qexp.p, s));
  }
  LAUNCH_CHECK(b2_launch_quantize(gh, n, b->d_qexp.p, p.qbits, b->q.p, ctx->num_sms, s));
  st.kernel_launches += 2;

  B2TrainParamDev dp;
  dp.min_child_weight = (double)p.min_child_weight; dp.lambda = (double)p.lambda; dp.alpha = (double)p.alpha;
  dp.inv_scale_g = dp.inv_scale_h = 1.0;
  dp.max_cat_to_onehot = p.max_cat_to_onehot; dp.max_cat_threshold = p.max_cat_threshold;
  dp.max_delta_step = (double)p.max_delta_step;
  B2CtlParams cp; cp.mcw = dp.min_child_weight; cp.lambda = dp.lambda; cp.alpha = dp.alpha; cp.max_delta_step = dp.max_delta_step; cp.gamma = p.gamma; cp.eta = p.eta / (float)p.num_parallel_tree;
  const B2TreeDev tree = tree_dev(b);
  int32_t* d_n_leaves = tree.n_nodes + 1;
  long long* d_level_rows = b->t_i64.p + 2 * L.max_nodes;
  B2LevelCtl* ctl = b->d_ctl.p;
  const int window = window_rows_for(p.qbits);
  const int n_streams = std::max(1, ctx->num_sms * 3 / G);
  const int pchunk = b2_split_chunk_rows(), lchunk = b2_part_chunk_rows();
  const int max_part_chunks_total = (int)((n + pchunk - 1) / pchunk);
  const size_t lcap = (size_t)1 << D;
  const int max_leaf_chunks = (int)((n + lchunk - 1) / lchunk) + (int)lcap;

  LAUNCH_CHECK(b2_launch_tree_init(tree, ctl, b->d_seg[0].p, b->d_ev[0].p, d_n_leaves, (int)n, b->d_hist_work.p, s));
  CUDA_CHECK(cudaMemsetAsync(b->d_leaf_sums.p, 0, 2 * lcap * sizeof(long long), s));
  mark_phase(b, 0);
  const int sh = b->log2_shards;
  const int shard_rank = b->shards > 1 ? b->comm->rank : 0;
  CUDA_CHECK(cudaMemsetAsync(build_target(b, b->hist[0].p), 0, b->node_elems * sizeof(long long), s));
  {
    const int chunk_rows = pick_chunk_rows(b, n);
    const int chunks = (int)((n + chunk_rows - 1) / chunk_rows);
    if (n > 0) {
      cudaEvent_t e0 = nullptr, e1 = nullptr;
      record_hist_launch(b, st, e0, e1, true);
      if (use_tma_hist() && m->has_tmap)
        LAUNCH_CHECK(b2_launch_hist_tma(m->bins.p, m->row_stride, m->tmap_tile, b->q.p, nullptr, b->d_hist_work.p, 1, chunks, chunk_rows, window, G,
                                        build_target(b, b->hist[0].p), nullptr, sh, 1, n, ctx->num_sms, s));
      else
        LAUNCH_CHECK(b2_launch_hist(m->bins.p, m->row_stride, b->q.p, nullptr, b->d_hist_work.p, 1, chunks, chunk_rows, window, G,
                                    build_target(b, b->hist[0].p), nullptr, sh, 1, m->narrow_w, ctx->num_sms, s));
      record_hist_launch(b, st, e0, e1, false);
      st.hist_launches++; st.kernel_launches++;
    }
  }
  mark_phase(b, 1);
  exchange_and_subtract(b, st, nullptr, b->hist[0].p, nullptr, nullptr, 1, 1);
  LAUNCH_CHECK(b2_launch_root_totals(b->hist[0].p, G, b->d_ev[0].p, b->d_qexp.p, p.qbits, dp, sh, tree.sum_g, tree.sum_h, s));
  st.kernel_launches += 2;
  int hb = 0;
  for (int d = 0; d <= D; ++d) {
    const int cur = d & 1, nxt = cur ^ 1;
    const int max_nodes_level = 1 << d;
    const bool can_split = d < D;
    const bool last_split_level = d == D - 1;
    const B2SplitCand* cands_for_decide = b->d_cands.p;
    int cand_rank_stride = max_nodes_level * b->cpn;
    if (can_split) {
      B2ColSample cs;
      cs.level_mask = p.use_cols() ? b->d_col_masks.p + (size_t)d * m->F : nullptr;
      cs.fwq = m->fwq.empty() ? nullptr : m->d_fwq.p;
      cs.bynode = (double)p.colsample_bynode; cs.n_level = n_level_feats[d]; cs.n_features = m->F;
      cs.seed = (uint32_t)p.seed; cs.tree = p.use_cols() ? tree_index : 0u;
      B2SiblingSub sub{nullptr, nullptr, nullptr, 0};
      if (sub_in_scan && d > 0) {
        sub.parent_level = b->hist[hb ^ 1].p; sub.triples = b->d_triples.p;
        sub.sib_out = d + 1 < D ? b->hist[hb].p : nullptr; sub.sib_base = max_nodes_level / 2;
      }
      LAUNCH_CHECK(b2_launch_eval_splits(b->hist[hb].p, G, b->d_ev[cur].p, max_nodes_level, m->d_group_first.p, m->d_group_size.p,
                                         m->d_nbins.p, m->d_has_missing.p, m->any_cat() ? m->d_is_cat.p : nullptr, b->d_qexp.p,
                                         p.qbits, dp, b->d_cands.p, b->cpn, ctl + cur, sh, shard_rank, cs, b->d_seg[cur].p, sub, s));
      st.kernel_launches++;
      if (m->any_cat()) {
        LAUNCH_CHECK(b2_launch_eval_cat_splits(b->hist[hb].p, G, b->d_ev[cur].p, max_nodes_level, m->d_cat_feats.p,
                                               (int)m->cat_feats.size(), m->d_feat_byte.p, m->d_nbins.p, b->d_qexp.p, p.qbits, dp,
                                               b->d_cands.p, b->cpn, b->cpn_num, ctl + cur, sh, shard_rank, cs, b->d_seg[cur].p, s));
        st.kernel_launches++;
      }
      if (p2p) {
        cands_for_decide = b->d_cands_all.p;
        cand_rank_stride = b->p2p.cand_cap;
      } else if (b->shards > 1) {
        const size_t bytes = (size_t)max_nodes_level * b->cpn * sizeof(B2SplitCand);
        NCCL_CHECK(nccl()->AllGather(b->d_cands.p, b->d_cands_all.p, bytes, kNcclUint8, b->comm->comm, s));
        cands_for_decide = b->d_cands_all.p;
      }
    }
    LAUNCH_CHECK(b2_launch_decide(ctl + cur, ctl + nxt, b->d_seg[cur].p, b->d_seg[nxt].p, b->d_ev[cur].p, b->d_ev[nxt].p,
                                  cands_for_decide, b->cpn, b->shards, cand_rank_stride, can_split ? 1 : 0, tree,
                                  b->d_split_work.p, b->d_pair_parent.p, b->d_leaves.p,
                                  d_n_leaves, m->d_has_missing.p, b->d_qexp.p, p.qbits, cp, can_split ? b->d_counters.p : nullptr, b->d_cands.p,
                                  (p2p && can_split) ? &b->p2p.pp : nullptr, s));
    st.kernel_launches++;
    mark_phase(b, 4);
    if (!can_split) break;
    const int32_t* ridx_in = d == 0 ? nullptr : b->ridx[cur].p;
    if (last_split_level && leaf_fused) {
      long long* sums = leaf_stream ? nullptr : b->d_leaf_sums.p;
      LAUNCH_CHECK(b2_launch_leaf_plan(b->d_leaves.p, &ctl[cur].leaf_base_next, b->d_seg_work.p, ctl + 2, s));
      LAUNCH_CHECK(b2_launch_leaf_sums(gh, b->ridx[0].p, b->ridx[1].p, b->d_seg_work.p, ctl + 2, max_leaf_chunks, b->d_qexp.p, 40,
                                       sums, b->pos.p, ctx->num_sms, s));
      LAUNCH_CHECK(b2_launch_final_assign(m->bins_col.p, m->col_stride, ridx_in, b->d_split_work.p, ctl + cur,
                                          max_part_chunks_total + max_nodes_level, gh, b->d_qexp.p, 40, sums, b->pos.p,
                                          m->any_cat() ? 1 : 0, ctx->num_sms, s));
      st.kernel_launches += 3;
      mark_phase(b, 5);
      continue;
    }
    const bool need_hist = d + 1 < D;
    B2FinalizeArgs fin;
    fin.ctl_nxt = ctl + nxt; fin.seg_nxt = b->d_seg[nxt].p; fin.ev_nxt = b->d_ev[nxt].p; fin.pair_parent_hist = b->d_pair_parent.p;
    fin.hist_work = b->d_hist_work.p; fin.triples = b->d_triples.p; fin.stat_rows = d_level_rows + d + 1; fin.done = b->d_part_done.p;
    fin.max_pairs = max_nodes_level; fin.need_hist = need_hist ? 1 : 0; fin.n_streams = n_streams; fin.window_rows = window;
    fin.chunk_rows_override = p.hist_chunk_rows;
    LAUNCH_CHECK(b2_launch_partition(m->bins_col.p, m->col_stride, ridx_in, b->ridx[nxt].p, b->d_split_work.p, ctl + cur,
                                     max_part_chunks_total + max_nodes_level, b->d_counters.p, m->any_cat() ? 1 : 0, fin,
                                     ctx->num_sms, s));
    st.kernel_launches++;
    mark_phase(b, 5);
    if (need_hist) {
      const int nh = hb ^ 1;
      long long* tgt = build_target(b, b->hist[nh].p);
      CUDA_CHECK(cudaMemsetAsync(tgt, 0, (size_t)max_nodes_level * b->node_elems * sizeof(long long), s));
      cudaEvent_t e0 = nullptr, e1 = nullptr;
      record_hist_launch(b, st, e0, e1, true);
      if (use_tma_hist() && m->has_tmap)
        LAUNCH_CHECK(b2_launch_hist_tma(m->bins.p, m->row_stride, m->tmap_tile, b->q.p, b->ridx[nxt].p, b->d_hist_work.p, 0, 0, 0, window, G, tgt, ctl + nxt, sh,
                                        max_nodes_level, n, ctx->num_sms, s));
      else
        LAUNCH_CHECK(b2_launch_hist(m->bins.p, m->row_stride, b->q.p, b->ridx[nxt].p, b->d_hist_work.p, 0, 0, 0, window, G, tgt,
                                    ctl + nxt, sh, max_nodes_level, m->narrow_w, ctx->num_sms, s));
      record_hist_launch(b, st, e0, e1, false);
      st.hist_launches++; st.kernel_launches++;
      mark_phase(b, 1);
      exchange_and_subtract(b, st, b->hist[hb].p, b->hist[nh].p, sub_in_scan ? nullptr : b->d_triples.p, ctl + nxt,
                            max_nodes_level, max_nodes_level);
      hb = nh;
    }
  }
  if (!leaf_fused) {
    LAUNCH_CHECK(b2_launch_leaf_plan(b->d_leaves.p, d_n_leaves, b->d_seg_work.p, ctl + 2, s));
    LAUNCH_CHECK(b2_launch_leaf_sums(gh, b->ridx[0].p, b->ridx[1].p, b->d_seg_work.p, ctl + 2, max_leaf_chunks, b->d_qexp.p, 40,
                                     b->d_leaf_sums.p, nullptr, ctx->num_sms, s));
    st.kernel_launches += 2;
  } else if (leaf_stream) {
    LAUNCH_CHECK(b2_launch_leaf_accumulate(gh, b->pos.p, n, D, b->d_qexp.p, 40, b->d_leaf_sums.p, ctx->num_sms, s));
    st.kernel_launches++;
  }
  if (p2p) { LAUNCH_CHECK(b2_launch_p2p_leaf_sums(&b->p2p.pp, d_n_leaves, b->d_leaf_sums.p, s)); st.kernel_launches++; }
  else allreduce(b->comm, b->d_leaf_sums.p, 2 * lcap, kNcclInt64, kNcclSum, s);
  LAUNCH_CHECK(b2_launch_leaf_values(b->d_leaves.p, d_n_leaves, b->d_leaf_sums.p, b->d_qexp.p, 40, cp, b->d_leaf_values.p, tree, b->t_qexp.p, s));
  if (leaf_fused)
    LAUNCH_CHECK(b2_launch_margin_update(b->margin.p, K, k, b->pos.p, b->d_leaf_values.p, n, ctx->num_sms, s));
  else
    LAUNCH_CHECK(b2_launch_pred_update(b->margin.p, K, k, b->ridx[0].p, b->ridx[1].p, b->d_seg_work.p, ctl + 2, max_leaf_chunks,
                                       b->d_leaf_values.p, ctx->num_sms, s));
  st.kernel_launches += 2;
  mark_phase(b, 6);
  char* stg = (char*)b->staging[slot];
  CUDA_CHECK(cudaMemcpyAsync(stg, b->t_block.p, m->any_cat() ? L.bytes : L.off_cat, cudaMemcpyDeviceToHost, s));
}

void apply_tree_stats(Booster* b, long long hist_launches, long long kernel_launches, double allreduce_bytes,
                      const std::vector<std::pair<cudaEvent_t, cudaEvent_t>>& ev) {
  b->t.hist_launches += hist_launches; b->t.kernel_launches += kernel_launches; b->t.allreduce_bytes += allreduce_bytes;
  for (auto& pr : ev) b->hist_events.push_back(pr);
}

void prepare_tree_buffers(Booster* b, int slot) {
  Matrix* m = b->train; const int64_t n = m->n;
  ensure_ctl_tables(b);
  const TreeLayout L = tree_layout(b->p.max_depth);
  const size_t rows = (size_t)std::max<int64_t>(n, 1);
  b->d_absmax.ensure(2 * (size_t)b->p.num_class); b->d_qexp.ensure(2);
  b->q.ensure(rows); b->ridx[0].ensure(rows); b->ridx[1].ensure(rows); b->pos.ensure(rows);
  if (b->staging_bytes != L.bytes) {
    for (void* h : b->staging) cudaFreeHost(h);
    b->staging.clear(); b->staging_bytes = L.bytes;
  }
  while ((int)b->staging.size() <= slot) { void* h = nullptr; CUDA_CHECK(cudaMallocHost(&h, L.bytes)); b->staging.push_back(h); }
}

void run_tree(Booster* b, int k, int slot) {
  cudaStream_t s = b->ctx->stream; const Params& p = b->p;
  prepare_tree_buffers(b, slot);
  static const bool want_graph = env_flag("B2_GRAPH", true);
  const bool eligible = want_graph && !b->graph_failed && b->absmax_fused && p.subsample >= 1.0f && !p.use_cols() &&
                        p.profile < 2 && !use_tma_hist() && p.num_parallel_tree == 1;
  auto direct = [&]() {
    TreeStats st;
    grow_tree(b, k, slot, st);
    apply_tree_stats(b, st.hist_launches, st.kernel_launches, st.allreduce_bytes, st.hist_ev);
    b->direct_trees[k]++;
  };
  if (!eligible) { direct(); return; }
  auto it = b->graphs.find(k);
  if (it == b->graphs.end()) {
    if (b->direct_trees[k] == 0) { direct(); return; }
    TreeStats st; st.capturing = true;
    cudaGraph_t graph = nullptr; cudaGraphExec_t exec = nullptr;
    bool ok = cudaStreamBeginCapture(s, cudaStreamCaptureModeThreadLocal) == cudaSuccess;
    if (ok) {
      try { grow_tree(b, k, slot, st); }
      catch (const B2Error& e) { cudaStreamEndCapture(s, &graph); if (graph) cudaGraphDestroy(graph); cudaGetLastError(); throw; }
      ok = cudaStreamEndCapture(s, &graph) == cudaSuccess && graph != nullptr;
    }
    if (ok) ok = cudaGraphInstantiate(&exec, graph, 0) == cudaSuccess;
    if (graph) cudaGraphDestroy(graph);
    if (!ok) {
      cudaGetLastError();
      for (auto& pr : st.hist_ev) { cudaEventDestroy(pr.first); cudaEventDestroy(pr.second); }
      b->graph_failed = true;
      fprintf(stderr, "[b2hist] CUDA graph capture of the tree failed; continuing with direct launches\n");
      direct();
      return;
    }
    Booster::TreeGraph g;
    g.exec = exec; g.hist_ev = st.hist_ev; g.hist_launches = st.hist_launches; g.kernel_launches = st.kernel_launches;
    g.allreduce_bytes = st.allreduce_bytes;
    it = b->graphs.emplace(k, std::move(g)).first;
  }
  CUDA_CHECK(cudaGraphLaunch(it->second.exec, s));
  apply_tree_stats(b, it->second.hist_launches, it->second.kernel_launches, it->second.allreduce_bytes, it->second.hist_ev);
}

void materialize_tree(Booster* b, int slot) {
  Matrix* m = b->train; const Params& p = b->p;
  const TreeLayout L = tree_layout(p.max_depth);
  const char* st = (const char*)b->staging[slot];
  const int32_t* i32 = (const int32_t*)st; const size_t mx = L.max_nodes;
  const float* f32 = (const float*)(st + L.off_f32);
  const long long* i64 = (const long long*)(st + L.off_i64);
  const int32_t* qexp = (const int32_t*)(st + L.off_qexp);
  const int nn = i32[7 * mx];
  const uint32_t* cat = (const uint32_t*)(st + L.off_cat);
  if (nn < 1 || (size_t)nn > mx) fail("corrupt tree read-back (n_nodes=%d)", nn);
  const double inv_sg = ldexp(1.0, qexp[0] - p.qbits), inv_sh = ldexp(1.0, qexp[1] - p.qbits);
  TreeHost t;
  for (int i = 0; i < nn; ++i) {
    t.add(i32[2 * mx + i]);
    t.left[i] = i32[i]; t.right[i] = i32[mx + i]; t.feature[i] = i32[3 * mx + i];
    const double G = (double)i64[i] * inv_sg, H = (double)i64[mx + i] * inv_sh;
    t.sum_hess[i] = H;
    if (t.feature[i] >= 0) {
      const int f = t.feature[i], bin = i32[4 * mx + i];
      t.split_bin[i] = bin; t.default_left[i] = (uint8_t)i32[5 * mx + i]; t.loss_chg[i] = f32[i];
      if (m->any_cat() && i32[6 * mx + i]) {
        t.split_type[i] = 1; t.any_cat = true;
        for (int w8 = 0; w8 < 8; ++w8) t.cat_bits[(size_t)i * 8 + w8] = cat[(size_t)i * 8 + w8];
        t.cond[i] = bin >= 0 ? (float)bin : NAN;
      } else
      t.cond[i] = bin < 0 ? m->min_vals[f] : m->cut_vals[m->cut_ptrs[f] + bin];
      t.base_weight[i] = h_calc_weight(p, G, H);
      t.value[i] = t.base_weight[i];
    } else {
      t.base_weight[i] = f32[mx + i];
      t.value[i] = f32[2 * mx + i];
    }
  }
  const long long* level_rows = i64 + 2 * mx;
  long long rows = m->n; int launches_nonempty = m->n > 0 ? 1 : 0;
  for (int d = 1; d < p.max_depth; ++d) { rows += level_rows[d]; if (level_rows[d] > 0) launches_nonempty++; }
  long long gathered = rows - m->n;
  int built_nodes = 0;
  for (int i = 0; i < nn; ++i) if (t.feature[i] >= 0) built_nodes++;
  b->t.hist_rows += rows;
  b->t.hist_bytes += (double)rows * (m->F + 8) + (double)gathered * 4 + (double)(built_nodes + 1) * m->F * 256.0 * 16.0;
  b->trees.push_back(std::move(t));
}

void sync_device_trees(Booster* b) {
  if (b->d_trees_synced == (int)b->trees.size()) return;
  b->h_nodes.clear(); b->h_tree_offset.clear(); b->h_cat_table.clear();
  for (auto& t : b->trees) {
    b->h_tree_offset.push_back((int32_t)b->h_nodes.size());
    for (int i = 0; i < t.size(); ++i) {
      int32_t cat_slot = -1;
      if (t.feature[i] >= 0 && t.split_type[i]) {
        cat_slot = (int32_t)(b->h_cat_table.size() / 8);
        b->h_cat_table.insert(b->h_cat_table.end(), t.cat_bits.begin() + (size_t)i * 8, t.cat_bits.begin() + (size_t)i * 8 + 8);
      }
      b->h_nodes.push_back(B2TreeNodeDev{t.left[i], t.right[i], t.feature[i], t.cond[i], t.value[i], (int32_t)t.default_left[i],
                                         cat_slot, 0});
    }
  }
  cudaStream_t s = b->ctx->stream;
  upload(b->d_nodes, b->h_nodes, s); upload(b->d_tree_offset, b->h_tree_offset, s); upload(b->d_cat_table, b->h_cat_table, s);
  CUDA_CHECK(cudaStreamSynchronize(s));
  b->d_trees_synced = (int)b->trees.size();
}

struct PathBuildElem {
  int32_t feature; bool is_cat; float lo, hi; uint32_t flags; uint32_t bits[8]; double z;
};
void walk_paths(const TreeHost& t, int nid, std::vector<PathBuildElem>& path, int tree, int cls, Booster* b,
                std::vector<B2PathElem>& elems, std::vector<B2PathInfo>& infos, std::vector<uint32_t>& cats, double* expected) {
  if (t.feature[nid] < 0) {
    if (path.size() + 1 > B2_SHAP_MAX_PATH)
      fail("tree %d has a leaf below %d distinct features; TreeSHAP supports at most %d (max_depth <= 14)", tree,
           (int)path.size(), B2_SHAP_MAX_PATH - 1);
    B2PathInfo pi{(int32_t)elems.size(), (int32_t)path.size() + 1, cls, 0, (double)t.value[nid]};
    elems.push_back(B2PathElem{-1, -1, 0.f, 0.f, 0u, 0u, 1.0});
    double zprod = 1.0;
    for (const PathBuildElem& e : path) {
      int32_t slot = -1;
      if (e.is_cat) { slot = (int32_t)(cats.size() / 8); cats.insert(cats.end(), e.bits, e.bits + 8); }
      elems.push_back(B2PathElem{e.feature, slot, e.lo, e.hi, e.flags, 0u, e.z});
      zprod *= e.z;
    }
    *expected += (double)t.value[nid] * zprod;
    infos.push_back(pi);
    return;
  }
  const int f = t.feature[nid];
  const bool is_cat = t.split_type[nid] != 0;
  const double cover = t.sum_hess[nid];
  for (int side = 0; side < 2; ++side) {
    const int child = side == 0 ? t.left[nid] : t.right[nid];
    const bool left = side == 0;
    std::vector<PathBuildElem> next = path;
    PathBuildElem* e = nullptr;
    for (auto& x : next) if (x.feature == f) e = &x;
    if (!e) {
      PathBuildElem ne;
      ne.feature = f; ne.is_cat = is_cat; ne.lo = -INFINITY; ne.hi = INFINITY;
      ne.flags = B2_PATH_MISSING_OK | B2_PATH_OUTSIDE_OK; ne.z = 1.0;
      for (int w = 0; w < 8; ++w) ne.bits[w] = 0xffffffffu;
      next.push_back(ne); e = &next.back();
    }
    e->z *= cover > 0.0 ? t.sum_hess[child] / cover : 0.0;
    if ((t.default_left[nid] != 0) != left) e->flags &= ~B2_PATH_MISSING_OK;
    if (is_cat) {
      e->is_cat = true;
      for (int w = 0; w < 8; ++w) e->bits[w] &= left ? ~t.cat_bits[(size_t)nid * 8 + w] : t.cat_bits[(size_t)nid * 8 + w];
      if (!left) e->flags &= ~B2_PATH_OUTSIDE_OK;
    } else if (left) {
      if (!(e->flags & B2_PATH_HAS_HI) || t.cond[nid] < e->hi) e->hi = t.cond[nid];
      e->flags |= B2_PATH_HAS_HI;
    } else if (t.cond[nid] > e->lo) {
      e->lo = t.cond[nid];
    }
    walk_paths(t, child, next, tree, cls, b, elems, infos, cats, expected);
  }
}

void build_paths(Booster* b) {
  if (b->paths_synced == (int)b->trees.size()) return;
  std::vector<B2PathElem> elems; std::vector<B2PathInfo> infos; std::vector<uint32_t> cats;
  b->tree_path_offset.assign(1, 0); b->tree_expected.clear();
  const int K = b->p.num_class, npt = std::max(1, b->p.num_parallel_tree);
  for (int t = 0; t < (int)b->trees.size(); ++t) {
    std::vector<PathBuildElem> path;
    double expected = 0.0;
    walk_paths(b->trees[t], 0, path, t, (t / npt) % K, b, elems, infos, cats, &expected);
    b->tree_path_offset.push_back((int32_t)infos.size());
    b->tree_expected.push_back(expected);
  }
  cudaStream_t s = b->ctx->stream;
  upload(b->d_path_elems, elems, s); upload(b->d_paths, infos, s); upload(b->d_path_cats, cats, s);
  CUDA_CHECK(cudaStreamSynchronize(s));
  b->paths_synced = (int)b->trees.size();
}

void init_margin(Booster* b, float* margin, Matrix* m) {
  const int K = b->p.num_class; cudaStream_t s = b->ctx->stream;
  if (m->n_base_margin > 0) {
    if (m->n_base_margin != m->n * K) fail("base_margin has %lld values, expected %lld", (long long)m->n_base_margin, (long long)(m->n * K));
    CUDA_CHECK(cudaMemcpyAsync(margin, m->base_margin.p, (size_t)m->n * K * sizeof(float), cudaMemcpyDeviceToDevice, s));
  } else {
    LAUNCH_CHECK(b2_launch_fill(margin, m->n * K, base_margin_value(b->p), b->ctx->num_sms, s));
  }
}

void estimate_base_score(Booster* b) {
  Matrix* m = b->train; cudaStream_t s = b->ctx->stream; Params& p = b->p;
  if (p.base_score_set || p.objective == kObjSoftprob) { p.base_score_set = true; return; }
  if (!b->trees.empty()) fail("continuing from existing trees needs an explicit base_score (the source model's intercept)");
  if (m->n_label != m->n) fail("train matrix has %lld labels for %lld rows", (long long)m->n_label, (long long)m->n);
  const int64_t n = m->n;
  DevBuf<float> zeros; DevBuf<float2> gh; DevBuf<long long> sums;
  zeros.ensure((size_t)std::max<int64_t>(n, 1)); gh.ensure((size_t)std::max<int64_t>(n, 1)); sums.ensure(2);
  CUDA_CHECK(cudaMemsetAsync(zeros.p, 0, (size_t)std::max<int64_t>(n, 1) * sizeof(float), s));
  LAUNCH_CHECK(b2_launch_gradient(p.objective, 1, zeros.p, m->label.p, m->n_weight ? m->weight.p : nullptr, n, p.scale_pos_weight,
                                  objective_param(p), gh.p, nullptr, nullptr, b->ctx->num_sms, s));
  b->d_absmax.ensure(2); b->d_qexp.ensure(2);
  CUDA_CHECK(cudaMemsetAsync(b->d_absmax.p, 0, 2 * sizeof(uint32_t), s));
  LAUNCH_CHECK(b2_launch_absmax(gh.p, n, b->d_absmax.p, b->ctx->num_sms, s));
  allreduce(b->comm, b->d_absmax.p, 2, kNcclUint32, kNcclMax, s);
  LAUNCH_CHECK(b2_launch_quant_exponent(b->d_absmax.p, b->d_qexp.p, s));
  CUDA_CHECK(cudaMemsetAsync(sums.p, 0, 2 * sizeof(long long), s));
  LAUNCH_CHECK(b2_launch_sum_fixed(gh.p, n, b->d_qexp.p, 40, sums.p, b->ctx->num_sms, s));
  allreduce(b->comm, sums.p, 2, kNcclInt64, kNcclSum, s);
  long long h_s[2]; int32_t h_e[2];
  CUDA_CHECK(cudaMemcpyAsync(h_s, sums.p, sizeof(h_s), cudaMemcpyDeviceToHost, s));
  CUDA_CHECK(cudaMemcpyAsync(h_e, b->d_qexp.p, sizeof(h_e), cudaMemcpyDeviceToHost, s));
  CUDA_CHECK(cudaStreamSynchronize(s));
// ... 952 lines not shown
```

xgboost_ray_b200/csrc/partition_kernel.cu:

```cuda
#include <stdlib.h>

#include "common.cuh"
#include "level_finalize.cuh"

namespace b2 {

constexpr int kPartThreads = 256;
constexpr int kPartChunk = 2048;

typedef B2SegWork SegWork;

constexpr int kSplitChunk = 8192;
constexpr int kSplitPasses = kSplitChunk / kPartChunk;

template <int kMode, bool kRoot>
__global__ void __launch_bounds__(kPartThreads)
partition_kernel(const uint8_t* __restrict__ bins_col, int64_t col_stride, const int32_t* __restrict__ ridx_in,
                 int32_t* __restrict__ ridx_out, const B2SplitWork* __restrict__ work, const B2LevelCtl* __restrict__ ctl,
                 int32_t* counters , B2FinalizeArgs fin) {
  const int n_work = ctl->n_split, total_chunks = ctl->part_chunks;
  constexpr int kIters = kPartChunk / kPartThreads;
  constexpr int kWarps = kPartThreads / 32;
  constexpr int kCounts = kSplitPasses * kIters * kWarps;
  __shared__ uint32_t s_rid[kSplitChunk];
  __shared__ int s_cnt[kCounts];
  __shared__ int s_base_left, s_base_right;
  __shared__ uint32_t s_cat[8];
  const int lane = threadIdx.x & 31, warp = threadIdx.x >> 5;
  for (int chunk = blockIdx.x; chunk < total_chunks; chunk += gridDim.x) {
    int lo = 0, hi = n_work - 1;
    while (lo < hi) {
      int mid = (lo + hi + 1) >> 1;
      if (__ldg(&work[mid].chunk_begin) <= chunk) lo = mid; else hi = mid - 1;
    }
    const B2SplitWork w = work[lo];
    const int row0 = (chunk - w.chunk_begin) * kSplitChunk;
    const int nrows = min(kSplitChunk, w.seg_count - row0);
    constexpr bool kCat = kMode != 0;
    if (kMode == 1) {
      if (threadIdx.x < 8) s_cat[threadIdx.x] = w.is_cat ? __ldg(&work[lo].cat_bits[threadIdx.x]) : 0u;
      __syncthreads();
    }
    const bool is_cat = kCat && w.is_cat != 0, has_missing = w.has_missing != 0, default_left = w.default_left != 0;
#pragma unroll 1
    for (int pass = 0; pass < kSplitPasses; ++pass) {
      const int pbase = pass * kPartChunk;
      if (pbase >= nrows) {
        if (threadIdx.x < kIters * kWarps) s_cnt[pass * kIters * kWarps + threadIdx.x] = 0;
        continue;
      }
      int rid[kIters]; bool left[kIters]; int bin[kIters];
      const int32_t* rsrc = kRoot ? nullptr : ridx_in + w.seg_begin + row0 + pbase + threadIdx.x;
#pragma unroll
      for (int it = 0; it < kIters; ++it) {
        const int r = pbase + it * kPartThreads + threadIdx.x;
        rid[it] = kRoot ? (r < nrows ? w.seg_begin + row0 + r : 0) : (r < nrows ? __ldg(rsrc + it * kPartThreads) : 0);
      }
      const uint8_t* col = bins_col + (int64_t)w.feature * col_stride;
#pragma unroll
      for (int it = 0; it < kIters; ++it) bin[it] = (int)__ldg(col + rid[it]);
#pragma unroll
      for (int it = 0; it < kIters; ++it) {
        const int r = pbase + it * kPartThreads + threadIdx.x;
        const bool valid = r < nrows;
        const int b = bin[it];
        bool l;
        if (kCat) {
          const uint32_t word = s_cat[b >> 5];
          const bool in_set = ((word >> (b & 31)) & 1u) != 0u;
          const bool go_left = is_cat ? !in_set : (b <= w.split_bin);
          l = (has_missing && b == B2_MISSING_BIN) ? default_left : go_left;
        } else {
          l = (w.has_missing && b == B2_MISSING_BIN) ? (w.default_left != 0) : (b <= w.split_bin);
        }
        left[it] = valid && l;
      }
#pragma unroll
      for (int it = 0; it < kIters; ++it) {
        const unsigned bal = __ballot_sync(0xffffffffu, left[it]);
        if (lane == 0) s_cnt[(pass * kIters + it) * kWarps + warp] = __popc(bal);
        s_rid[pbase + it * kPartThreads + threadIdx.x] = (uint32_t)rid[it] | (left[it] ? 0x80000000u : 0u);
      }
    }
    __syncthreads();
    if (warp == 0) {
      int c[kCounts / 32], sum = 0;
#pragma unroll
      for (int k = 0; k < kCounts / 32; ++k) { c[k] = s_cnt[lane * (kCounts / 32) + k]; sum += c[k]; }
      int incl = sum;
#pragma unroll
      for (int o = 1; o < 32; o <<= 1) { const int v = __shfl_up_sync(0xffffffffu, incl, o); if (lane >= o) incl += v; }
      int run = incl - sum;
#pragma unroll
      for (int k = 0; k < kCounts / 32; ++k) { s_cnt[lane * (kCounts / 32) + k] = run; run += c[k]; }
      if (lane == 31) {
        const unsigned long long old = atomicAdd(reinterpret_cast<unsigned long long*>(counters + 2 * lo),
                                                 ((unsigned long long)(unsigned)nrows << 32) | (unsigned long long)(unsigned)incl);
        s_base_left = (int)(unsigned)(old & 0xffffffffull);
        s_base_right = (int)(unsigned)(old >> 32) - s_base_left;
      }
    }
    __syncthreads();
    const int base_l = s_base_left, base_r = s_base_right;
#pragma unroll 1
    for (int pass = 0; pass < kSplitPasses; ++pass) {
      const int pbase = pass * kPartChunk;
      if (pbase >= nrows) break;
#pragma unroll
      for (int it = 0; it < kIters; ++it) {
        const int r = pbase + it * kPartThreads + threadIdx.x;
        const uint32_t v = s_rid[r];
        const bool l = (v & 0x80000000u) != 0u;
        const unsigned bal = __ballot_sync(0xffffffffu, l);
        if (r < nrows) {
          const int lrank = s_cnt[(pass * kIters + it) * kWarps + warp] + __popc(bal & ((1u << lane) - 1u));
          if (l) ridx_out[w.seg_begin + base_l + lrank] = (int32_t)(v & 0x7fffffffu);
          else {
            const int rrank = r - lrank;
            ridx_out[w.seg_begin + w.seg_count - 1 - (base_r + rrank)] = (int32_t)v;
          }
        }
      }
    }
    __syncthreads();
  }
  __shared__ FinalizeScratch<kPartThreads> s_fin;
  __shared__ bool s_last;
  __syncthreads();
  if (threadIdx.x == 0) {
    __threadfence();
    const unsigned prev = atomicAdd(fin.done, 1u);
    s_last = prev == gridDim.x - 1;
    if (s_last) { __threadfence(); *fin.done = 0u; }
  }
  __syncthreads();
  if (!s_last) return;
  finalize_level_block<kPartThreads>(s_fin, ctl, work, counters, fin);
}

__global__ void __launch_bounds__(256)
leaf_sums_kernel(const float2* __restrict__ gh, const int32_t* __restrict__ ridx0, const int32_t* __restrict__ ridx1,
                 const SegWork* __restrict__ work, const B2LevelCtl* __restrict__ ctl, const int32_t* __restrict__ qexp,
                 int leaf_bits, long long* __restrict__ sums ,
                 uint16_t* __restrict__ pos ) {
  const int n_work = ctl->hist_n_work, total_chunks = ctl->hist_total_chunks;
  __shared__ long long sg[8], sh[8];
  const double kg = ldexp(1.0, leaf_bits - qexp[0]), kh = ldexp(1.0, leaf_bits - qexp[1]);
  for (int chunk = blockIdx.x; chunk < total_chunks; chunk += gridDim.x) {
    int lo = 0, hi = n_work - 1;
    while (lo < hi) {
      int mid = (lo + hi + 1) >> 1;
      if (__ldg(&work[mid].chunk_begin) <= chunk) lo = mid; else hi = mid - 1;
    }
    const SegWork w = work[lo];
    const int32_t* ridx = w.pad0 ? nullptr : (w.buf ? ridx1 : ridx0);
    const int row0 = (chunk - w.chunk_begin) * kPartChunk;
    const int nrows = min(kPartChunk, w.seg_count - row0);
    if (!sums) {
      for (int r = threadIdx.x; r < nrows; r += blockDim.x)
        pos[ridx ? __ldg(ridx + w.seg_begin + row0 + r) : (w.seg_begin + row0 + r)] = (uint16_t)w.id;
      continue;
    }
    long long ag = 0, ah = 0;
    for (int r = threadIdx.x; r < nrows; r += blockDim.x) {
      const int row = ridx ? __ldg(ridx + w.seg_begin + row0 + r) : (w.seg_begin + row0 + r);
      if (pos) pos[row] = (uint16_t)w.id;
      const float2 v = __ldg(gh + row);
      ag += __double2ll_rn(__dmul_rn((double)v.x, kg));
      ah += __double2ll_rn(__dmul_rn((double)v.y, kh));
    }
#pragma unroll
    for (int o = 16; o > 0; o >>= 1) { ag += __shfl_xor_sync(0xffffffffu, ag, o); ah += __shfl_xor_sync(0xffffffffu, ah, o); }
    if ((threadIdx.x & 31) == 0) { sg[threadIdx.x >> 5] = ag; sh[threadIdx.x >> 5] = ah; }
    __syncthreads();
    if (threadIdx.x == 0) {
      long long tg = 0, th = 0;
      for (int i = 0; i < 8; ++i) { tg += sg[i]; th += sh[i]; }
      atomicAdd((unsigned long long*)&sums[2 * w.id], (unsigned long long)tg);
      atomicAdd((unsigned long long*)&sums[2 * w.id + 1], (unsigned long long)th);
    }
    __syncthreads();
  }
}

__global__ void __launch_bounds__(256)
pred_update_kernel(float* __restrict__ margin, int K, int k, const int32_t* __restrict__ ridx0,
                   const int32_t* __restrict__ ridx1, const SegWork* __restrict__ work, const B2LevelCtl* __restrict__ ctl,
                   const float* __restrict__ leaf_value) {
  const int n_work = ctl->hist_n_work, total_chunks = ctl->hist_total_chunks;
  for (int chunk = blockIdx.x; chunk < total_chunks; chunk += gridDim.x) {
    int lo = 0, hi = n_work - 1;
    while (lo < hi) {
      int mid = (lo + hi + 1) >> 1;
      if (__ldg(&work[mid].chunk_begin) <= chunk) lo = mid; else hi = mid - 1;
    }
    const SegWork w = work[lo];
    const int32_t* ridx = w.pad0 ? nullptr : (w.buf ? ridx1 : ridx0);
    const int row0 = (chunk - w.chunk_begin) * kPartChunk;
    const int nrows = min(kPartChunk, w.seg_count - row0);
    const float v = __ldg(leaf_value + w.id);
    for (int r = threadIdx.x; r < nrows; r += blockDim.x) {
      const int64_t row = ridx ? __ldg(ridx + w.seg_begin + row0 + r) : (w.seg_begin + row0 + r);
      margin[row * K + k] += v;
    }
  }
}

template <bool kCat, bool kRoot, bool kSums>
__global__ void __launch_bounds__(kPartThreads)
final_assign_kernel(const uint8_t* __restrict__ bins_col, int64_t col_stride, const int32_t* __restrict__ ridx_in,
                    const B2SplitWork* __restrict__ work, const B2LevelCtl* __restrict__ ctl, const float2* __restrict__ gh,
                    const int32_t* __restrict__ qexp, int leaf_bits, long long* __restrict__ sums,
                    uint16_t* __restrict__ pos) {
  const int n_work = ctl->n_split, total_chunks = ctl->part_chunks, leaf_base = ctl->leaf_base_next;
  __shared__ long long s_acc[kPartThreads / 32][4];
  const double kg = kSums ? ldexp(1.0, leaf_bits - qexp[0]) : 0.0, kh = kSums ? ldexp(1.0, leaf_bits - qexp[1]) : 0.0;
  const int lane = threadIdx.x & 31, warp = threadIdx.x >> 5;
  for (int chunk = blockIdx.x; chunk < total_chunks; chunk += gridDim.x) {
    int lo = 0, hi = n_work - 1;
    while (lo < hi) {
      int mid = (lo + hi + 1) >> 1;
      if (__ldg(&work[mid].chunk_begin) <= chunk) lo = mid; else hi = mid - 1;
    }
    const B2SplitWork w = work[lo];
    const int row0 = (chunk - w.chunk_begin) * kSplitChunk;
    const int nrows = min(kSplitChunk, w.seg_count - row0);
    const bool is_cat = kCat && w.is_cat != 0;
    const int leaf_l = leaf_base + 2 * lo;
    long long lg = 0, lh = 0, rg = 0, rh = 0;
    constexpr int kBatch = kSums ? 4 : 8;
    const uint8_t* col = bins_col + (int64_t)w.feature * col_stride;
    for (int r0 = threadIdx.x; r0 < nrows; r0 += kBatch * kPartThreads) {
      int rid[kBatch]; int bin[kBatch]; float2 v[kBatch];
#pragma unroll
      for (int k = 0; k < kBatch; ++k) {
        const int r = r0 + k * kPartThreads;
        rid[k] = r < nrows ? (kRoot ? w.seg_begin + row0 + r : __ldg(ridx_in + w.seg_begin + row0 + r)) : -1;
      }
#pragma unroll
      for (int k = 0; k < kBatch; ++k) {
        bin[k] = (int)__ldg(col + (rid[k] < 0 ? 0 : rid[k]));
        if (kSums) v[k] = __ldg(gh + (rid[k] < 0 ? 0 : rid[k]));
      }
#pragma unroll
      for (int k = 0; k < kBatch; ++k) {
        if (rid[k] < 0) continue;
        const int b = bin[k];
        bool go_left = b <= w.split_bin;
        if (kCat && is_cat) go_left = ((__ldg(&work[lo].cat_bits[b >> 5]) >> (b & 31)) & 1u) == 0u;
        const bool l = (w.has_missing && b == B2_MISSING_BIN) ? (w.default_left != 0) : go_left;
        if (kSums) {
          const long long qg = __double2ll_rn(__dmul_rn((double)v[k].x, kg)), qh = __double2ll_rn(__dmul_rn((double)v[k].y, kh));
          if (l) { lg += qg; lh += qh; } else { rg += qg; rh += qh; }
        }
        pos[rid[k]] = (uint16_t)(leaf_l + (l ? 0 : 1));
      }
    }
    if (!kSums) continue;
#pragma unroll
    for (int o = 16; o > 0; o >>= 1) {
      lg += __shfl_xor_sync(0xffffffffu, lg, o); lh += __shfl_xor_sync(0xffffffffu, lh, o);
      rg += __shfl_xor_sync(0xffffffffu, rg, o); rh += __shfl_xor_sync(0xffffffffu, rh, o);
    }
    if (lane == 0) { s_acc[warp][0] = lg; s_acc[warp][1] = lh; s_acc[warp][2] = rg; s_acc[warp][3] = rh; }
    __syncthreads();
    if (threadIdx.x < 4) {
      long long t = 0;
      for (int i = 0; i < kPartThreads / 32; ++i) t += s_acc[i][threadIdx.x];
      atomicAdd((unsigned long long*)&sums[2 * leaf_l + threadIdx.x], (unsigned long long)t);
    }
    __syncthreads();
  }
}

__global__ void __launch_bounds__(256)
margin_update_kernel(float* __restrict__ margin, int K, int k, const uint16_t* __restrict__ pos,
                     const float* __restrict__ leaf_value, int64_t n) {
  for (int64_t i = (int64_t)blockIdx.x * blockDim.x + threadIdx.x; i < n; i += (int64_t)gridDim.x * blockDim.x)
    margin[i * K + k] += __ldg(leaf_value + pos[i]);
}

constexpr int kLeafAccThreads = 512;
constexpr int kLeafAccMaxDepth = 11;
constexpr int kLeafAccSmem = 32 * 1024;
__device__ __forceinline__ void acc_add64(uint32_t* lo, uint32_t* hi, long long q) {
  const uint32_t l = (uint32_t)(unsigned long long)q, h = (uint32_t)((unsigned long long)q >> 32);
  const uint32_t old = atomicAdd(lo, l);
  const uint32_t hadd = h + ((uint32_t)(old + l) < old ? 1u : 0u);
  if (hadd != 0u) atomicAdd(hi, hadd);
}
__global__ void __launch_bounds__(kLeafAccThreads)
leaf_accumulate_kernel(const float2* __restrict__ gh, const uint16_t* __restrict__ pos, int64_t n, int n_acc, int log2_copies,
                       const int32_t* __restrict__ qexp, int leaf_bits, long long* __restrict__ sums ) {
  extern __shared__ uint32_t s_acc[];
  const int copies = 1 << log2_copies, plane = n_acc << log2_copies;
  for (int i = threadIdx.x; i < 4 * plane; i += blockDim.x) s_acc[i] = 0u;
  __syncthreads();
  uint32_t *glo = s_acc, *ghi = s_acc + plane, *hlo = s_acc + 2 * plane, *hhi = s_acc + 3 * plane;
  const int copy = threadIdx.x & (copies - 1);
  const double kg = ldexp(1.0, leaf_bits - qexp[0]), kh = ldexp(1.0, leaf_bits - qexp[1]);
  constexpr int kBatch = 4;
  const int64_t stride = (int64_t)gridDim.x * blockDim.x;
  int64_t i = (int64_t)blockIdx.x * blockDim.x + threadIdx.x;
  for (; i + (kBatch - 1) * stride < n; i += kBatch * stride) {
    int leaf[kBatch]; float2 v[kBatch];
#pragma unroll
    for (int b = 0; b < kBatch; ++b) { leaf[b] = pos[i + b * stride]; v[b] = __ldg(gh + i + b * stride); }
#pragma unroll
    for (int b = 0; b < kBatch; ++b) {
      const int a = (leaf[b] << log2_copies) + copy;
      acc_add64(glo + a, ghi + a, __double2ll_rn(__dmul_rn((double)v[b].x, kg)));
      acc_add64(hlo + a, hhi + a, __double2ll_rn(__dmul_rn((double)v[b].y, kh)));
    }
  }
  for (; i < n; i += stride) {
    const int a = ((int)pos[i] << log2_copies) + copy;
    const float2 v = __ldg(gh + i);
    acc_add64(glo + a, ghi + a, __double2ll_rn(__dmul_rn((double)v.x, kg)));
    acc_add64(hlo + a, hhi + a, __double2ll_rn(__dmul_rn((double)v.y, kh)));
  }
  __syncthreads();
  for (int j = threadIdx.x; j < 2 * n_acc; j += blockDim.x) {
    const uint32_t* lo = (j & 1) ? hlo : glo;
    const uint32_t* hi = (j & 1) ? hhi : ghi;
    unsigned long long t = 0ull;
    for (int c = 0; c < copies; ++c) {
      const int a = ((j >> 1) << log2_copies) + c;
      t += ((unsigned long long)hi[a] << 32) | (unsigned long long)lo[a];
    }
    if (t != 0ull) atomicAdd((unsigned long long*)&sums[j], t);
  }
}

__global__ void iota_kernel(int32_t* out, int64_t n) {
  for (int64_t i = (int64_t)blockIdx.x * blockDim.x + threadIdx.x; i < n; i += (int64_t)gridDim.x * blockDim.x) out[i] = (int32_t)i;
}

}

extern "C" {
int b2_part_chunk_rows() { return b2::kPartChunk; }
int b2_split_chunk_rows() { return b2::kSplitChunk; }

int b2_launch_partition(const uint8_t* bins_col, int64_t col_stride, const int32_t* ridx_in, int32_t* ridx_out,
                        const B2SplitWork* work, const B2LevelCtl* ctl, int max_chunks, int32_t* counters, int any_categorical,
                        B2FinalizeArgs fin, int num_sms, cudaStream_t stream) {
  if (max_chunks <= 0) max_chunks = 1;
  int grid = max_chunks < num_sms * 6 ? max_chunks : num_sms * 6;
#define B2_PART_LAUNCH(MODE)                                                                                                  \
  do {                                                                                                                        \
    if (ridx_in) b2::partition_kernel<MODE, false><<<grid, b2::kPartThreads, 0, stream>>>(bins_col, col_stride, ridx_in, ridx_out, work, ctl, counters, fin); \
    else b2::partition_kernel<MODE, true><<<grid, b2::kPartThreads, 0, stream>>>(bins_col, col_stride, ridx_in, ridx_out, work, ctl, counters, fin);    \
  } while (0)
  if (any_categorical) B2_PART_LAUNCH(1);
  else B2_PART_LAUNCH(0);
#undef B2_PART_LAUNCH
  return (int)cudaGetLastError();
}
int b2_launch_leaf_sums(const float2* gh, const int32_t* ridx0, const int32_t* ridx1, const void* work, const B2LevelCtl* ctl,
                        int max_chunks, const int32_t* qexp, int leaf_bits, long long* sums, uint16_t* pos, int num_sms,
                        cudaStream_t stream) {
  if (max_chunks <= 0) return 0;
  int grid = max_chunks < num_sms * 8 ? max_chunks : num_sms * 8;
  b2::leaf_sums_kernel<<<grid, 256, 0, stream>>>(gh, ridx0, ridx1, (const b2::SegWork*)work, ctl, qexp, leaf_bits, sums, pos);
  return (int)cudaGetLastError();
}
int b2_launch_final_assign(const uint8_t* bins_col, int64_t col_stride, const int32_t* ridx_in, const B2SplitWork* work,
                           const B2LevelCtl* ctl, int max_chunks, const float2* gh, const int32_t* qexp, int leaf_bits,
                           long long* sums, uint16_t* pos, int any_categorical, int num_sms, cudaStream_t stream) {
  if (max_chunks <= 0) return 0;
  int grid = max_chunks < num_sms * 8 ? max_chunks : num_sms * 8;
#define B2_FA_LAUNCH(CAT, ROOT)                                                                                               \
  do {                                                                                                                        \
    if (sums) b2::final_assign_kernel<CAT, ROOT, true><<<grid, b2::kPartThreads, 0, stream>>>(bins_col, col_stride, ridx_in, work, ctl, gh, qexp, leaf_bits, sums, pos); \
    else b2::final_assign_kernel<CAT, ROOT, false><<<grid, b2::kPartThreads, 0, stream>>>(bins_col, col_stride, ridx_in, work, ctl, gh, qexp, leaf_bits, sums, pos);    \
  } while (0)
  if (any_categorical) { if (ridx_in) B2_FA_LAUNCH(true, false); else B2_FA_LAUNCH(true, true); }
  else { if (ridx_in) B2_FA_LAUNCH(false, false); else B2_FA_LAUNCH(false, true); }
#undef B2_FA_LAUNCH
  return (int)cudaGetLastError();
}
int b2_leaf_acc_max_depth() { return b2::kLeafAccMaxDepth; }
int b2_launch_leaf_accumulate(const float2* gh, const uint16_t* pos, int64_t n, int max_depth, const int32_t* qexp, int leaf_bits,
                              long long* sums, int num_sms, cudaStream_t stream) {
  if (n <= 0) return 0;
  if (max_depth > b2::kLeafAccMaxDepth) return (int)cudaErrorInvalidValue;
  const int n_acc = 1 << max_depth;
  int log2_copies = 0;
  while (log2_copies < 3 && ((size_t)n_acc * 16 << (log2_copies + 1)) <= (size_t)b2::kLeafAccSmem) ++log2_copies;
  const size_t smem = (size_t)n_acc * 16 << log2_copies;
  const int64_t want = (n + b2::kLeafAccThreads - 1) / b2::kLeafAccThreads;
  const int grid = (int)(want < (int64_t)num_sms * 2 ? want : (int64_t)num_sms * 2);
  b2::leaf_accumulate_kernel<<<grid, b2::kLeafAccThreads, smem, stream>>>(gh, pos, n, n_acc, log2_copies, qexp, leaf_bits, sums);
  return (int)cudaGetLastError();
}
int b2_launch_margin_update(float* margin, int K, int k, const uint16_t* pos, const float* leaf_value, int64_t n, int num_sms,
                            cudaStream_t stream) {
  if (n <= 0) return 0;
  int64_t want = (n + 255) / 256;
  int grid = (int)(want < (int64_t)num_sms * 16 ? want : (int64_t)num_sms * 16);
  b2::margin_update_kernel<<<grid, 256, 0, stream>>>(margin, K, k, pos, leaf_value, n);
  return (int)cudaGetLastError();
}
int b2_launch_pred_update(float* margin, int K, int k, const int32_t* ridx0, const int32_t* ridx1, const void* work,
                          const B2LevelCtl* ctl, int max_chunks, const float* leaf_value, int num_sms, cudaStream_t stream) {
  if (max_chunks <= 0) return 0;
  int grid = max_chunks < num_sms * 8 ? max_chunks : num_sms * 8;
  b2::pred_update_kernel<<<grid, 256, 0, stream>>>(margin, K, k, ridx0, ridx1, (const b2::SegWork*)work, ctl, leaf_value);
  return (int)cudaGetLastError();
}
int b2_launch_iota(int32_t* out, int64_t n, cudaStream_t stream) {
  if (n <= 0) return 0;
  int grid = (int)((n + 1023) / 1024);
  if (grid > 4096) grid = 4096;
  b2::iota_kernel<<<grid, 256, 0, stream>>>(out, n);
  return (int)cudaGetLastError();
}
}
```

xgboost_ray_b200/csrc/split_kernel.cu:

```cuda
#include <cub/block/block_scan.cuh>

#include "common.cuh"
#include "sampling.cuh"

namespace b2 {

__device__ __forceinline__ double calc_gain(double G, double H, const B2TrainParamDev& p) {
  return b2_calc_gain(G, H, p.min_child_weight, p.lambda, p.alpha, p.max_delta_step);
}

struct Best {
  unsigned long long key;
  int32_t bin, default_left;
  long long lg, lh;
};

__device__ __forceinline__ void consider(Best& b, float chg, uint32_t order, int bin, int dl, long long lg, long long lh) {
  if (!(chg > 0.0f) || isinf(chg)) return;
  unsigned long long key = ((unsigned long long)__float_as_uint(chg) << 32) | (unsigned long long)(0xffffffffu - order);
  if (key > b.key) { b.key = key; b.bin = bin; b.default_left = dl; b.lg = lg; b.lh = lh; }
}

constexpr int kEvalChunks = 32;
constexpr int kEvalBinsPerChunk = 256 / kEvalChunks;

__global__ void __launch_bounds__(32 * kEvalChunks)
eval_splits_kernel(const long long* __restrict__ level_hist, int n_groups, const B2EvalNode* __restrict__ nodes,
                   const int32_t* __restrict__ group_first, const int32_t* __restrict__ group_size,
                   const int32_t* __restrict__ nbins, const uint8_t* __restrict__ has_missing,
                   const uint8_t* __restrict__ is_cat ,
                   const int32_t* __restrict__ qexp, int qbits, B2TrainParamDev p, B2SplitCand* __restrict__ cands,
                   int cand_stride, const B2LevelCtl* __restrict__ ctl, int log2_shards, int shard_rank, B2ColSample cs,
                   const B2NodeSeg* __restrict__ seg, B2SiblingSub sub) {
  const int sp = B2_GROUP_SLOTS >> log2_shards;
  const int cpn = (n_groups * sp + 31) >> 5;
  const int node = blockIdx.x / cpn, cta_in_node = blockIdx.x % cpn;
  if (ctl && node >= ctl->n_nodes) return;
  const int s = threadIdx.x & 31, q = threadIdx.x >> 5;
  __shared__ long long cs_g[kEvalChunks][32], cs_h[kEvalChunks][32];
  __shared__ unsigned long long wkey[kEvalChunks];
  const B2EvalNode nd = nodes[node];
  p.inv_scale_g = ldexp(1.0, qexp[0] - qbits);
  p.inv_scale_h = ldexp(1.0, qexp[1] - qbits);
  const int v = cta_in_node * 32 + s;
  const bool v_ok = v < n_groups * sp;
  const int group = v_ok ? v / sp : 0, sl = v_ok ? v % sp : 0;
  const int slot = (sl << log2_shards) + shard_rank;
  const size_t slice_elems = (size_t)n_groups * 2 * B2_BINS * sp;
  const size_t in_slice = (size_t)(group * 2) * B2_BINS * sp + sl;
  const bool fused = sub.parent_level != nullptr && nd.hist_index >= sub.sib_base;
  const int pair = fused ? nd.hist_index - sub.sib_base : 0;
  const long long* hg = level_hist + (size_t)(fused ? sub.triples[3 * pair + 1] : nd.hist_index) * slice_elems + in_slice;
  const long long* hh = hg + (size_t)B2_BINS * sp;
  const long long* pgp = fused ? sub.parent_level + (size_t)sub.triples[3 * pair] * slice_elems + in_slice : nullptr;
  const long long* php = fused ? pgp + (size_t)B2_BINS * sp : nullptr;
  long long* sgp = (fused && sub.sib_out) ? sub.sib_out + (size_t)nd.hist_index * slice_elems + in_slice : nullptr;
  long long* shp = sgp ? sgp + (size_t)B2_BINS * sp : nullptr;
  const int f = group_first[group] + slot;
  bool active = v_ok && slot < group_size[group] && !(is_cat && is_cat[f]);
  if (active && cs.level_mask) active = cs.level_mask[f] != 0;
  if (cs.bynode < 1.0) {
    __shared__ uint8_t s_allowed[32];
    if (q == 0)
      s_allowed[s] = active && b2_col_selected(cs.seed, cs.tree, B2_SCOPE_NODE(seg[node].nid), f, cs.level_mask, cs.fwq,
                                               cs.n_features, b2_sample_count(cs.bynode, cs.n_level));
    __syncthreads();
    active = active && s_allowed[s];
  }
  const int nf = active ? nbins[f] : 0;
  const bool fmiss = active ? (has_missing[f] != 0) : false;

  long long sg = 0, sh = 0;
  if (fused) {
    if (v_ok && (sgp || active)) {
#pragma unroll
      for (int i = 0; i < kEvalBinsPerChunk; ++i) {
        const int b = q * kEvalBinsPerChunk + i;
        const long long g = pgp[b * sp] - hg[b * sp], h = php[b * sp] - hh[b * sp];
        if (sgp) { sgp[b * sp] = g; shp[b * sp] = h; }
        if (active && b < nf) { sg += g; sh += h; }
      }
    }
  } else if (active) {
#pragma unroll
    for (int i = 0; i < kEvalBinsPerChunk; ++i) {
      int b = q * kEvalBinsPerChunk + i;
      if (b < nf) { sg += hg[b * sp]; sh += hh[b * sp]; }
    }
  }
  cs_g[q][s] = sg; cs_h[q][s] = sh;
  __syncthreads();
  long long pg = 0, ph = 0, real_g = 0, real_h = 0;
#pragma unroll 8
  for (int k = 0; k < kEvalChunks; ++k) {
    long long a = cs_g[k][s], b = cs_h[k][s];
    if (k < q) { pg += a; ph += b; }
    real_g += a; real_h += b;
  }
  const long long tot_g = nd.sum_g, tot_h = nd.sum_h;
  const double G = __dmul_rn(__ll2double_rn(tot_g), p.inv_scale_g), H = __dmul_rn(__ll2double_rn(tot_h), p.inv_scale_h);
  const double root_gain = (double)nd.root_gain;
  const bool node_has_missing = fmiss && (real_g != tot_g || real_h != tot_h);
  Best best; best.key = 0; best.bin = 0; best.default_left = 0; best.lg = 0; best.lh = 0;
  if (active) {
#pragma unroll 2
    for (int i = 0; i < kEvalBinsPerChunk; ++i) {
      const int b = q * kEvalBinsPerChunk + i;
      if (b >= nf) break;
      const long long eg_excl = pg, eh_excl = ph;
      if (!fused) { pg += hg[b * sp]; ph += hh[b * sp]; }
      else if (sgp) { pg += sgp[b * sp]; ph += shp[b * sp]; }
      else { pg += pgp[b * sp] - hg[b * sp]; ph += php[b * sp] - hh[b * sp]; }
      {
        const double lh_d = __dmul_rn(__ll2double_rn(ph), p.inv_scale_h);
        if (lh_d >= p.min_child_weight) {
          const double rh_d = __dadd_rn(H, -lh_d);
          if (rh_d >= p.min_child_weight) {
            const double lg_d = __dmul_rn(__ll2double_rn(pg), p.inv_scale_g);
            const double rg_d = __dadd_rn(G, -lg_d);
            const double gain = __dadd_rn(__dadd_rn(calc_gain(lg_d, lh_d, p), calc_gain(rg_d, rh_d, p)), -root_gain);
            consider(best, __double2float_rn(gain), (uint32_t)f * 1024u + (uint32_t)b, b, 0, pg, ph);
          }
        }
      }
      if (node_has_missing) {
        const long long rg_i = real_g - eg_excl, rh_i = real_h - eh_excl;
        const double rh_d = __dmul_rn(__ll2double_rn(rh_i), p.inv_scale_h);
        if (rh_d >= p.min_child_weight) {
          const double lh_d = __dadd_rn(H, -rh_d);
          if (lh_d >= p.min_child_weight) {
            const double rg_d = __dmul_rn(__ll2double_rn(rg_i), p.inv_scale_g);
            const double lg_d = __dadd_rn(G, -rg_d);
            const double gain = __dadd_rn(__dadd_rn(calc_gain(lg_d, lh_d, p), calc_gain(rg_d, rh_d, p)), -root_gain);
            consider(best, __double2float_rn(gain), (uint32_t)f * 1024u + 512u + (uint32_t)(255 - b), b - 1, 1,
                     tot_g - rg_i, tot_h - rh_i);
          }
        }
      }
    }
  }
  unsigned long long k = best.key;
#pragma unroll
  for (int o = 16; o > 0; o >>= 1) {
    unsigned long long other = __shfl_xor_sync(0xffffffffu, k, o);
    k = other > k ? other : k;
  }
  if (s == 0) wkey[q] = k;
  __syncthreads();
  unsigned long long kmax = 0;
#pragma unroll 8
  for (int i = 0; i < kEvalChunks; ++i) kmax = wkey[i] > kmax ? wkey[i] : kmax;
  B2SplitCand* out = cands + (size_t)node * cand_stride + cta_in_node;
  if (kmax == 0) {
    if (threadIdx.x == 0) {
      out->loss_chg = 0.0f; out->feature = -1; out->bin = 0; out->default_left = 0; out->left_g = 0; out->left_h = 0;
      out->order = 0xffffffffu; out->is_cat = 0;
    }
  } else if (best.key == kmax) {
    out->loss_chg = __uint_as_float((uint32_t)(kmax >> 32));
    out->feature = f; out->bin = best.bin; out->default_left = best.default_left;
    out->left_g = best.lg; out->left_h = best.lh; out->order = 0xffffffffu - (uint32_t)(kmax & 0xffffffffu); out->is_cat = 0;
  }
}

constexpr int kCatCtas = 4;

__device__ __forceinline__ float calc_weight_f(double G, double H, const B2TrainParamDev& p) {
  return __double2float_rn(b2_calc_weight(G, H, p.min_child_weight, p.lambda, p.alpha, p.max_delta_step));
}

__global__ void __launch_bounds__(256)
eval_cat_splits_kernel(const long long* __restrict__ level_hist, int n_groups, const B2EvalNode* __restrict__ nodes,
                       const int32_t* __restrict__ cat_feats, int n_cat, const int32_t* __restrict__ feat_byte,
                       const int32_t* __restrict__ nbins, const int32_t* __restrict__ qexp, int qbits, B2TrainParamDev p,
                       B2SplitCand* __restrict__ cands, int cand_stride, int cand_offset, const B2LevelCtl* __restrict__ ctl,
                       int log2_shards, int shard_rank, B2ColSample cs, const B2NodeSeg* __restrict__ seg) {
  const int node = blockIdx.x / kCatCtas, j = blockIdx.x % kCatCtas;
  if (ctl && node >= ctl->n_nodes) return;
  typedef cub::BlockScan<long long, 256> Scan;
  __shared__ typename Scan::TempStorage scan_tmp;
  __shared__ float s_w[256];
  __shared__ long long s_g[256], s_h[256];
  __shared__ long long s_red[2][8];
  __shared__ unsigned long long s_wkey[8];
  __shared__ unsigned long long s_best_key;
  __shared__ uint32_t s_bits[8];
  __shared__ int s_mode, s_part;
  __shared__ int s_skip;
  __shared__ B2SplitCand s_best;
  const int b = threadIdx.x, lane = b & 31, warp = b >> 5;
  const int sp = B2_GROUP_SLOTS >> log2_shards, shards = 1 << log2_shards;
  const size_t slice_elems = (size_t)n_groups * 2 * B2_BINS * sp;
  const B2EvalNode nd = nodes[node];
  p.inv_scale_g = ldexp(1.0, qexp[0] - qbits);
  p.inv_scale_h = ldexp(1.0, qexp[1] - qbits);
  const long long tot_g = nd.sum_g, tot_h = nd.sum_h;
  const double G = __dmul_rn(__ll2double_rn(tot_g), p.inv_scale_g), H = __dmul_rn(__ll2double_rn(tot_h), p.inv_scale_h);
  const double root_gain = (double)nd.root_gain;
  if (b == 0) s_best_key = 0;
  __syncthreads();
  for (int ci = j; ci < n_cat; ci += kCatCtas) {
    const int f = cat_feats[ci];
    const int fb = feat_byte[f], group = fb >> 5, slot = fb & 31;
    if ((slot & (shards - 1)) != shard_rank) continue;
    if (cs.level_mask || cs.bynode < 1.0) {
      if (b == 0) {
        bool ok = !cs.level_mask || cs.level_mask[f] != 0;
        if (ok && cs.bynode < 1.0)
          ok = b2_col_selected(cs.seed, cs.tree, B2_SCOPE_NODE(seg[node].nid), f, cs.level_mask, cs.fwq, cs.n_features,
                               b2_sample_count(cs.bynode, cs.n_level));
        s_skip = ok ? 0 : 1;
      }
      __syncthreads();
      const bool skip = s_skip != 0;
      __syncthreads();
      if (skip) continue;
    }
    const int sl = slot >> log2_shards;
    const long long* hg = level_hist + (size_t)nd.hist_index * slice_elems + (size_t)(group * 2) * B2_BINS * sp + sl;
    const long long* hh = hg + (size_t)B2_BINS * sp;
    const int nf = nbins[f];
    long long g = 0, h = 0;
    if (b < nf) { g = hg[b * sp]; h = hh[b * sp]; }
    long long rg = g, rh = h;
#pragma unroll
    for (int o = 16; o > 0; o >>= 1) { rg += __shfl_xor_sync(0xffffffffu, rg, o); rh += __shfl_xor_sync(0xffffffffu, rh, o); }
    if (lane == 0) { s_red[0][warp] = rg; s_red[1][warp] = rh; }
    __syncthreads();
    long long real_g = 0, real_h = 0;
#pragma unroll
    for (int k = 0; k < 8; ++k) { real_g += s_red[0][k]; real_h += s_red[1][k]; }
    Best best; best.key = 0; best.bin = 0; best.default_left = 0; best.lg = 0; best.lh = 0;
    int my_mode = 0, my_part = 0, rank = 0;
    if (nf < p.max_cat_to_onehot) {
      if (b < nf) {
        const long long mg = tot_g - real_g, mh = tot_h - real_h;
#pragma unroll
        for (int pass = 0; pass < 2; ++pass) {
          const long long rgi = pass ? g + mg : g, rhi = pass ? h + mh : h;
          const double rh_d = __dmul_rn(__ll2double_rn(rhi), p.inv_scale_h), lh_d = __dadd_rn(H, -rh_d);
          if (lh_d >= p.min_child_weight && rh_d >= p.min_child_weight) {
            const double rg_d = __dmul_rn(__ll2double_rn(rgi), p.inv_scale_g), lg_d = __dadd_rn(G, -rg_d);
            const double gain = __dadd_rn(__dadd_rn(calc_gain(lg_d, lh_d, p), calc_gain(rg_d, rh_d, p)), -root_gain);
            const unsigned long long before = best.key;
            consider(best, __double2float_rn(gain), (uint32_t)f * 1024u + (uint32_t)(2 * b + pass), b, pass ? 0 : 1,
                     tot_g - rgi, tot_h - rhi);
            if (best.key != before) { my_mode = 0; my_part = b; }
          }
        }
      }
    } else {
      const float w = b < nf ? calc_weight_f(__dmul_rn(__ll2double_rn(g), p.inv_scale_g), __dmul_rn(__ll2double_rn(h), p.inv_scale_h), p)
                             : 0.0f;
      s_w[b] = w; s_g[b] = 0; s_h[b] = 0;
      __syncthreads();
      if (b < nf) {
        for (int k = 0; k < nf; ++k) { const float wk = s_w[k]; rank += (wk < w || (wk == w && k < b)) ? 1 : 0; }
        s_g[rank] = g; s_h[rank] = h;
      }
      __syncthreads();
      long long pg, ph;
      Scan(scan_tmp).InclusiveSum(s_g[b], pg);
      __syncthreads();
      Scan(scan_tmp).InclusiveSum(s_h[b], ph);
      __syncthreads();
      s_g[b] = pg; s_h[b] = ph;
      __syncthreads();
      const int n_iter = min(p.max_cat_threshold, nf) - 1;
      const int k = b;
      if (k < n_iter) {
        const double rh_d = __dmul_rn(__ll2double_rn(ph), p.inv_scale_h), lh_d = __dadd_rn(H, -rh_d);
        if (lh_d >= p.min_child_weight && rh_d >= p.min_child_weight) {
          const double rg_d = __dmul_rn(__ll2double_rn(pg), p.inv_scale_g), lg_d = __dadd_rn(G, -rg_d);
          const double gain = __dadd_rn(__dadd_rn(calc_gain(lg_d, lh_d, p), calc_gain(rg_d, rh_d, p)), -root_gain);
          const unsigned long long before = best.key;
          consider(best, __double2float_rn(gain), (uint32_t)f * 1024u + (uint32_t)k, -1, 1, tot_g - pg, tot_h - ph);
          if (best.key != before) { my_mode = 1; my_part = k + 1; }
        }
      }
      if (n_iter > 0 && k >= nf - n_iter && k < nf) {
        const long long lgi = real_g - s_g[k - 1], lhi = real_h - s_h[k - 1];
        const double lh_d = __dmul_rn(__ll2double_rn(lhi), p.inv_scale_h), rh_d = __dadd_rn(H, -lh_d);
        if (lh_d >= p.min_child_weight && rh_d >= p.min_child_weight) {
          const double lg_d = __dmul_rn(__ll2double_rn(lgi), p.inv_scale_g), rg_d = __dadd_rn(G, -lg_d);
          const double gain = __dadd_rn(__dadd_rn(calc_gain(lg_d, lh_d, p), calc_gain(rg_d, rh_d, p)), -root_gain);
          const unsigned long long before = best.key;
          consider(best, __double2float_rn(gain), (uint32_t)f * 1024u + 512u + (uint32_t)(nf - 1 - k), -1, 0, lgi, lhi);
          if (best.key != before) { my_mode = 1; my_part = k; }
        }
      }
    }
    unsigned long long key = best.key;
#pragma unroll
    for (int o = 16; o > 0; o >>= 1) { unsigned long long other = __shfl_xor_sync(0xffffffffu, key, o); key = other > key ? other : key; }
    if (lane == 0) s_wkey[warp] = key;
    __syncthreads();
    unsigned long long kmax = 0;
#pragma unroll
    for (int i = 0; i < 8; ++i) kmax = s_wkey[i] > kmax ? s_wkey[i] : kmax;
    const bool better = kmax != 0 && (uint32_t)(kmax >> 32) > (uint32_t)(s_best_key >> 32);
    __syncthreads();
    if (better) {
      if (best.key == kmax) {
        s_best.loss_chg = __uint_as_float((uint32_t)(kmax >> 32)); s_best.feature = f; s_best.bin = best.bin;
        s_best.default_left = best.default_left; s_best.left_g = best.lg; s_best.left_h = best.lh;
        s_best.order = 0xffffffffu - (uint32_t)(kmax & 0xffffffffu); s_best.is_cat = 1;
        s_mode = my_mode; s_part = my_part; s_best_key = kmax;
      }
      if (b < 8) s_bits[b] = 0;
      __syncthreads();
      if (b < nf && (s_mode == 0 ? (b == s_part) : (rank < s_part))) atomicOr(&s_bits[b >> 5], 1u << (b & 31));
      __syncthreads();
    }
  }
  if (b == 0) {
    B2SplitCand* out = cands + (size_t)node * cand_stride + cand_offset + j;
    if (s_best_key == 0) {
      out->loss_chg = 0.0f; out->feature = -1; out->bin = 0; out->default_left = 0; out->left_g = 0; out->left_h = 0;
      out->order = 0xffffffffu; out->is_cat = 0;
    } else {
      *out = s_best;
#pragma unroll
      for (int i = 0; i < 8; ++i) out->cat_bits[i] = s_bits[i];
    }
  }
}

__global__ void root_totals_kernel(const long long* __restrict__ level_hist, int n_groups, B2EvalNode* nodes,
                                   const int32_t* __restrict__ qexp, int qbits, B2TrainParamDev p, int log2_shards,
                                   long long* __restrict__ tree_sum_g, long long* __restrict__ tree_sum_h) {
  __shared__ long long sg[256], sh[256];
  const int sp = B2_GROUP_SLOTS >> log2_shards;
  const size_t slice_elems = (size_t)n_groups * 2 * B2_BINS * sp;
  const long long* hg = level_hist + (size_t)nodes[0].hist_index * slice_elems;
  sg[threadIdx.x] = hg[(size_t)threadIdx.x * sp];
  sh[threadIdx.x] = hg[(size_t)(B2_BINS + threadIdx.x) * sp];
  __syncthreads();
  for (int o = 128; o > 0; o >>= 1) {
    if ((int)threadIdx.x < o) { sg[threadIdx.x] += sg[threadIdx.x + o]; sh[threadIdx.x] += sh[threadIdx.x + o]; }
    __syncthreads();
  }
  if (threadIdx.x == 0) {
    p.inv_scale_g = ldexp(1.0, qexp[0] - qbits);
    p.inv_scale_h = ldexp(1.0, qexp[1] - qbits);
    nodes[0].sum_g = sg[0]; nodes[0].sum_h = sh[0];
    tree_sum_g[0] = sg[0]; tree_sum_h[0] = sh[0];
    double G = __dmul_rn(__ll2double_rn(sg[0]), p.inv_scale_g), H = __dmul_rn(__ll2double_rn(sh[0]), p.inv_scale_h);
    nodes[0].root_gain = __double2float_rn(calc_gain(G, H, p));
  }
}

}

extern "C" {
int b2_launch_eval_splits(const long long* level_hist, int n_groups, const B2EvalNode* nodes, int n_nodes,
                          const int32_t* group_first, const int32_t* group_size, const int32_t* nbins,
                          const uint8_t* has_missing, const uint8_t* is_cat, const int32_t* qexp, int qbits, B2TrainParamDev p,
                          B2SplitCand* cands, int cand_stride, const B2LevelCtl* ctl, int log2_shards, int shard_rank,
                          B2ColSample cs, const B2NodeSeg* seg, B2SiblingSub sub, cudaStream_t stream) {
  if (n_nodes <= 0) return 0;
  const int sp = B2_GROUP_SLOTS >> log2_shards, cpn = (n_groups * sp + 31) >> 5;
  b2::eval_splits_kernel<<<n_nodes * cpn, 32 * b2::kEvalChunks, 0, stream>>>(level_hist, n_groups, nodes, group_first, group_size,
                                                                         nbins, has_missing, is_cat, qexp, qbits, p, cands,
                                                                         cand_stride, ctl, log2_shards, shard_rank, cs, seg, sub);
  return (int)cudaGetLastError();
}
int b2_cat_ctas() { return b2::kCatCtas; }
int b2_launch_eval_cat_splits(const long long* level_hist, int n_groups, const B2EvalNode* nodes, int n_nodes,
                              const int32_t* cat_feats, int n_cat, const int32_t* feat_byte, const int32_t* nbins,
                              const int32_t* qexp, int qbits, B2TrainParamDev p, B2SplitCand* cands, int cand_stride,
                              int cand_offset, const B2LevelCtl* ctl, int log2_shards, int shard_rank, B2ColSample cs,
                              const B2NodeSeg* seg, cudaStream_t stream) {
  if (n_nodes <= 0 || n_cat <= 0) return 0;
  b2::eval_cat_splits_kernel<<<n_nodes * b2::kCatCtas, 256, 0, stream>>>(level_hist, n_groups, nodes, cat_feats, n_cat, feat_byte,
                                                                        nbins, qexp, qbits, p, cands, cand_stride, cand_offset,
                                                                        ctl, log2_shards, shard_rank, cs, seg);
  return (int)cudaGetLastError();
}
int b2_launch_root_totals(const long long* level_hist, int n_groups, B2EvalNode* nodes, const int32_t* qexp, int qbits,
                          B2TrainParamDev p, int log2_shards, long long* tree_sum_g, long long* tree_sum_h,
                          cudaStream_t stream) {
  b2::root_totals_kernel<<<1, 256, 0, stream>>>(level_hist, n_groups, nodes, qexp, qbits, p, log2_shards, tree_sum_g, tree_sum_h);
  return (int)cudaGetLastError();
}
}
```

Before: 242.6.

## Fold decide into eval via last-CTA, warp-parallel candidate selection, narrow eval kernel

Moves the decide logic into a shared header and lets the split-evaluation kernel run it in the last finishing CTA, so a separate decide launch per level is no longer needed. Candidate selection becomes warp-parallel: each warp reduces one node's candidates with a packed 64-bit key instead of one thread scanning all of them serially. A new narrower evaluation kernel is used for small node counts, with the old 32-chunk kernel kept for wide levels. The cost is extra atomic completion counting and a serial tail in one CTA, plus a more complex launch API.

New measurement: 252.6 (median of 6 runs). 1.04x the previous value.

```diff
diff --git a/xgboost_ray_b200/build.py b/xgboost_ray_b200/build.py
--- a/xgboost_ray_b200/build.py
+++ b/xgboost_ray_b200/build.py
@@ -35,7 +35,7 @@
 
 def build(force=False, verbose=False):
     os.makedirs(OBJ_DIR, exist_ok=True)
-    headers = [os.path.join(CSRC, "common.cuh"), os.path.join(CSRC, "hist_common.cuh"), os.path.join(CSRC, "sampling.cuh"), os.path.join(CSRC, "p2p.cuh"), os.path.join(CSRC, "level_finalize.cuh"), os.path.join(HERE, "..", "include", "b2hist.h"), __file__]
+    headers = [os.path.join(CSRC, "common.cuh"), os.path.join(CSRC, "hist_common.cuh"), os.path.join(CSRC, "sampling.cuh"), os.path.join(CSRC, "p2p.cuh"), os.path.join(CSRC, "level_finalize.cuh"), os.path.join(CSRC, "decide.cuh"), os.path.join(HERE, "..", "include", "b2hist.h"), __file__]
     jobs = []
     objs = []
     for src, extra in SOURCES.items():
diff --git a/xgboost_ray_b200/csrc/common.cuh b/xgboost_ray_b200/csrc/common.cuh
--- a/xgboost_ray_b200/csrc/common.cuh
+++ b/xgboost_ray_b200/csrc/common.cuh
@@ -156,6 +156,28 @@
   const int32_t* triples;
   long long* sib_out;
   int32_t sib_base;
+};
+
+struct B2DecideArgs {
+  B2LevelCtl* ctl_cur;
+  B2LevelCtl* ctl_nxt;
+  const B2NodeSeg* seg_cur;
+  B2NodeSeg* seg_nxt;
+  const B2EvalNode* ev_cur;
+  B2EvalNode* ev_nxt;
+  const B2SplitCand* cands;
+  B2SplitCand* cand_best;
+  const B2SplitCand* local_cands;
+  B2TreeDev tree;
+  B2SplitWork* split_work;
+  int32_t* pair_parent_hist;
+  B2LeafDev* leaves;
+  int32_t* n_leaves;
+  const uint8_t* has_missing;
+  const int32_t* qexp;
+  int32_t* part_counters;
+  B2CtlParams p;
+  int32_t cands_per_node, cand_ranks, cand_rank_stride, can_split, qbits;
 };
 
 #define B2_P2P_MAX_WORLD 8
diff --git a/xgboost_ray_b200/csrc/control_kernel.cu b/xgboost_ray_b200/csrc/control_kernel.cu
--- a/xgboost_ray_b200/csrc/control_kernel.cu
+++ b/xgboost_ray_b200/csrc/control_kernel.cu
@@ -1,156 +1,29 @@
 #include <string.h>
 
-#include <cub/block/block_scan.cuh>
-
 #include "common.cuh"
-#include "p2p.cuh"
+#include "decide.cuh"
 
 namespace b2 {
 
 constexpr int kCtlThreads = 1024;
 constexpr int kPartChunkRows = 2048;
-constexpr int kSplitChunkRows = 8192;
 
-__device__ __forceinline__ double c_calc_gain(double G, double H, const B2CtlParams& p) {
-  return b2_calc_gain(G, H, p.mcw, p.lambda, p.alpha, p.max_delta_step);
-}
 __device__ __forceinline__ float c_calc_weight(double G, double H, const B2CtlParams& p) {
   return __double2float_rn(b2_calc_weight(G, H, p.mcw, p.lambda, p.alpha, p.max_delta_step));
 }
 
-struct TileScan {
-  typedef cub::BlockScan<int, kCtlThreads> Scan;
-  Scan::TempStorage* tmp;
-  int carry;
-  __device__ TileScan(Scan::TempStorage* t) : tmp(t), carry(0) {}
-  __device__ int step(int v) {
-    int ex, total;
-    Scan(*tmp).ExclusiveSum(v, ex, total);
-    __syncthreads();
-    int r = carry + ex;
-    carry += total;
-    return r;
-  }
-};
-
 __global__ void __launch_bounds__(kCtlThreads)
-decide_kernel(B2LevelCtl* __restrict__ ctl_cur, B2LevelCtl* __restrict__ ctl_nxt, const B2NodeSeg* __restrict__ seg_cur,
-              B2NodeSeg* __restrict__ seg_nxt, const B2EvalNode* __restrict__ ev_cur, B2EvalNode* __restrict__ ev_nxt,
-              const B2SplitCand* __restrict__ cands, int cands_per_node, int cand_ranks, int cand_rank_stride, int can_split,
-              B2TreeDev tree,
-              B2SplitWork* __restrict__ split_work, int32_t* __restrict__ pair_parent_hist, B2LeafDev* __restrict__ leaves,
-              int32_t* __restrict__ n_leaves, const uint8_t* __restrict__ has_missing, const int32_t* __restrict__ qexp,
-              int qbits, B2CtlParams p, int32_t* __restrict__ part_counters, const B2SplitCand* __restrict__ local_cands,
-              int use_p2p, B2P2P pp) {
-  __shared__ typename TileScan::Scan::TempStorage tmp;
-  __shared__ int s_node_base, s_leaf_base;
-  const int n = ctl_cur->n_nodes;
-  if (part_counters) for (int i = threadIdx.x; i < 2 * n; i += kCtlThreads) part_counters[i] = 0;
-  if (use_p2p && can_split) {
-    constexpr int kWords = sizeof(B2SplitCand) / 8;
-    static_assert(sizeof(B2SplitCand) % 8 == 0, "candidates are copied as 64-bit words");
-    const uint32_t epoch = p2p_next_epoch(pp, kSlotCand);
-    const int total = n * cands_per_node * kWords;
-    for (int w = 0; w < pp.world; ++w) {
-      long long* dst = reinterpret_cast<long long*>(pp.cands[w] + (size_t)pp.rank * pp.cand_cap);
-      for (int t = threadIdx.x; t < total; t += kCtlThreads) st_volatile_u64(dst + t, reinterpret_cast<const long long*>(local_cands)[t]);
-    }
-    __syncthreads();
-    p2p_signal(pp, kSlotCand, epoch);
-    p2p_wait(pp, kSlotCand, epoch);
-    p2p_finish_single(pp, kSlotCand, epoch);
-  }
-  const double inv_sg = ldexp(1.0, qexp[0] - qbits), inv_sh = ldexp(1.0, qexp[1] - qbits);
-  if (threadIdx.x == 0) { s_node_base = *tree.n_nodes; s_leaf_base = *n_leaves; }
-  __syncthreads();
-  TileScan scan_split(&tmp), scan_leaf(&tmp), scan_chunks(&tmp);
-  for (int base = 0; base < n; base += kCtlThreads) {
-    const int i = base + threadIdx.x;
-    const bool in = i < n;
-    B2SplitCand best; best.feature = -1; best.loss_chg = 0.f; best.order = 0xffffffffu; best.bin = 0; best.default_left = 0;
-    best.left_g = 0; best.left_h = 0; best.is_cat = 0;
-    B2EvalNode nd; nd.sum_g = 0; nd.sum_h = 0; nd.hist_index = 0; nd.root_gain = 0.f;
-    B2NodeSeg sg; sg.nid = 0; sg.begin = 0; sg.count = 0; sg.buf = 0;
-    bool expand = false;
-    if (in) {
-      nd = ev_cur[i]; sg = seg_cur[i];
-      if (can_split) {
-        for (int w = 0; w < cand_ranks; ++w)
-          for (int g = 0; g < cands_per_node; ++g) {
-            B2SplitCand c;
-            if (use_p2p) {
-              constexpr int kW = sizeof(B2SplitCand) / 8;
-              const long long* src = reinterpret_cast<const long long*>(cands + (size_t)w * cand_rank_stride + (size_t)i * cands_per_node + g);
-#pragma unroll
-              for (int t = 0; t < kW; ++t) reinterpret_cast<unsigned long long*>(&c)[t] = ld_volatile_u64(src + t);
-            } else c = cands[(size_t)w * cand_rank_stride + (size_t)i * cands_per_node + g];
-            if (c.feature < 0) continue;
-            if (best.feature < 0 || c.loss_chg > best.loss_chg || (c.loss_chg == best.loss_chg && c.order < best.order)) best = c;
-          }
-        if (best.feature >= 0)
-          expand = best.loss_chg > 1e-6f && best.left_h != 0 && (nd.sum_h - best.left_h) != 0 && !(best.loss_chg < p.gamma);
-      }
-    }
-    const int rank = scan_split.step(expand ? 1 : 0);
-    const int lrank = scan_leaf.step((in && !expand) ? 1 : 0);
-    const int chunks = expand ? (sg.count + kSplitChunkRows - 1) / kSplitChunkRows : 0;
-    const int chunk_begin = scan_chunks.step(chunks);
-    if (in && !expand) {
-      B2LeafDev lf; lf.nid = sg.nid; lf.buf = sg.buf; lf.begin = sg.begin; lf.count = sg.count;
-      leaves[s_leaf_base + lrank] = lf;
-    }
-    if (expand) {
-      const int l = s_node_base + 2 * rank, r = l + 1;
-      const int nid = sg.nid;
-      tree.left[nid] = l; tree.right[nid] = r; tree.feature[nid] = best.feature; tree.split_bin[nid] = best.bin;
-      tree.default_left[nid] = best.default_left; tree.loss_chg[nid] = best.loss_chg;
-      tree.split_type[nid] = best.is_cat;
-      if (best.is_cat) {
-#pragma unroll
-        for (int w8 = 0; w8 < 8; ++w8) tree.cat_bits[(size_t)nid * 8 + w8] = best.cat_bits[w8];
-      }
-      tree.left[l] = -1; tree.right[l] = -1; tree.feature[l] = -1; tree.parent[l] = nid;
-      tree.left[r] = -1; tree.right[r] = -1; tree.feature[r] = -1; tree.parent[r] = nid;
-      const long long lg = best.left_g, lh = best.left_h, rg = nd.sum_g - lg, rh = nd.sum_h - lh;
-      tree.sum_g[l] = lg; tree.sum_h[l] = lh; tree.sum_g[r] = rg; tree.sum_h[r] = rh;
-      B2SplitWork sw;
-      sw.seg_begin = sg.begin; sw.seg_count = sg.count; sw.feature = best.feature; sw.split_bin = best.bin;
-      sw.default_left = best.default_left; sw.has_missing = has_missing[best.feature]; sw.chunk_begin = chunk_begin;
-      sw.is_cat = best.is_cat;
-#pragma unroll
-      for (int w8 = 0; w8 < 8; ++w8) sw.cat_bits[w8] = best.is_cat ? best.cat_bits[w8] : 0u;
-      split_work[rank] = sw;
-      pair_parent_hist[rank] = nd.hist_index;
-      const double GL = __dmul_rn(__ll2double_rn(lg), inv_sg), HL = __dmul_rn(__ll2double_rn(lh), inv_sh);
-      const double GR = __dmul_rn(__ll2double_rn(rg), inv_sg), HR = __dmul_rn(__ll2double_rn(rh), inv_sh);
-      B2EvalNode el, er;
-      el.sum_g = lg; el.sum_h = lh; el.hist_index = -1; el.root_gain = __double2float_rn(c_calc_gain(GL, HL, p));
-      er.sum_g = rg; er.sum_h = rh; er.hist_index = -1; er.root_gain = __double2float_rn(c_calc_gain(GR, HR, p));
-      ev_nxt[2 * rank] = el; ev_nxt[2 * rank + 1] = er;
-      B2NodeSeg sl, sr;
-      sl.nid = l; sl.buf = sg.buf ^ 1; sl.begin = sg.begin; sl.count = 0;
-      sr.nid = r; sr.buf = sg.buf ^ 1; sr.begin = sg.begin; sr.count = sg.count;
-      seg_nxt[2 * rank] = sl; seg_nxt[2 * rank + 1] = sr;
-    }
-  }
-  __syncthreads();
-  if (threadIdx.x == 0) {
-    const int n_split = scan_split.carry;
-    ctl_cur->n_split = n_split; ctl_cur->part_chunks = scan_chunks.carry;
-    ctl_cur->leaf_base_next = s_leaf_base + scan_leaf.carry;
-    ctl_nxt->n_nodes = 2 * n_split; ctl_nxt->n_split = 0; ctl_nxt->part_chunks = 0;
-    ctl_nxt->hist_n_work = 0; ctl_nxt->hist_total_chunks = 0; ctl_nxt->n_pairs = 0;
-    *tree.n_nodes = s_node_base + 2 * n_split;
-    *n_leaves = s_leaf_base + scan_leaf.carry;
-  }
+decide_kernel(B2DecideArgs a, int use_p2p, B2P2P pp) {
+  __shared__ DecideScratch<kCtlThreads> sm;
+  decide_block<kCtlThreads>(sm, a, use_p2p != 0, pp);
 }
 
 __global__ void __launch_bounds__(kCtlThreads)
 leaf_plan_kernel(const B2LeafDev* __restrict__ leaves, const int32_t* __restrict__ n_leaves, B2SegWork* __restrict__ work,
                  B2LevelCtl* __restrict__ leaf_ctl) {
-  __shared__ typename TileScan::Scan::TempStorage tmp;
+  __shared__ typename TileScan<kCtlThreads>::Scan::TempStorage tmp;
   const int n = *n_leaves;
-  TileScan scan(&tmp);
+  TileScan<kCtlThreads> scan(&tmp);
   for (int base = 0; base < n; base += kCtlThreads) {
     const int i = base + threadIdx.x;
     int chunks = 0; B2LeafDev lf; lf.nid = 0; lf.buf = 0; lf.begin = 0; lf.count = 0;
@@ -199,16 +72,10 @@
 }
 
 extern "C" {
-int b2_launch_decide(B2LevelCtl* ctl_cur, B2LevelCtl* ctl_nxt, const B2NodeSeg* seg_cur, B2NodeSeg* seg_nxt,
-                     const B2EvalNode* ev_cur, B2EvalNode* ev_nxt, const B2SplitCand* cands, int cands_per_node, int cand_ranks,
-                     int cand_rank_stride, int can_split, B2TreeDev tree, B2SplitWork* split_work, int32_t* pair_parent_hist, B2LeafDev* leaves, int32_t* n_leaves,
-                     const uint8_t* has_missing, const int32_t* qexp, int qbits, B2CtlParams p, int32_t* part_counters,
-                     const B2SplitCand* local_cands, const void* p2p, cudaStream_t s) {
+int b2_launch_decide(const B2DecideArgs* a, const void* p2p, cudaStream_t s) {
   B2P2P pp;
   if (p2p) pp = *reinterpret_cast<const B2P2P*>(p2p); else memset(&pp, 0, sizeof(pp));
-  b2::decide_kernel<<<1, b2::kCtlThreads, 0, s>>>(ctl_cur, ctl_nxt, seg_cur, seg_nxt, ev_cur, ev_nxt, cands, cands_per_node,
-                                                 cand_ranks, cand_rank_stride, can_split, tree, split_work, pair_parent_hist, leaves, n_leaves, has_missing, qexp, qbits, p,
-                                                 part_counters, local_cands, p2p ? 1 : 0, pp);
+  b2::decide_kernel<<<1, b2::kCtlThreads, 0, s>>>(*a, p2p ? 1 : 0, pp);
   return (int)cudaGetLastError();
 }
 int b2_launch_leaf_plan(const B2LeafDev* leaves, const int32_t* n_leaves, B2SegWork* work, B2LevelCtl* leaf_ctl, cudaStream_t s) {
diff --git a/xgboost_ray_b200/csrc/decide.cuh b/xgboost_ray_b200/csrc/decide.cuh
--- /dev/null
+++ b/xgboost_ray_b200/csrc/decide.cuh
@@ -0,0 +1,173 @@
+#pragma once
+#include <stddef.h>
+
+#include <cub/block/block_scan.cuh>
+
+#include "common.cuh"
+#include "p2p.cuh"
+
+namespace b2 {
+
+constexpr int kSplitChunkRows = 8192;
+
+__device__ __forceinline__ double c_calc_gain(double G, double H, const B2CtlParams& p) {
+  return b2_calc_gain(G, H, p.mcw, p.lambda, p.alpha, p.max_delta_step);
+}
+
+template <int kThreads>
+struct TileScan {
+  typedef cub::BlockScan<int, kThreads> Scan;
+  typename Scan::TempStorage* tmp;
+  int carry;
+  __device__ TileScan(typename Scan::TempStorage* t) : tmp(t), carry(0) {}
+  __device__ int step(int v) {
+    int ex, total;
+    Scan(*tmp).ExclusiveSum(v, ex, total);
+    __syncthreads();
+    int r = carry + ex;
+    carry += total;
+    return r;
+  }
+};
+
+template <int kThreads>
+struct DecideScratch {
+  typename TileScan<kThreads>::Scan::TempStorage scan;
+  int node_base, leaf_base;
+};
+
+__device__ __forceinline__ unsigned long long cand_word(const B2SplitCand* c, int w, bool vol) {
+  const long long* src = reinterpret_cast<const long long*>(c) + w;
+  return vol ? ld_volatile_u64(src) : (unsigned long long)__ldcg(src);
+}
+
+template <int kThreads>
+__device__ void select_candidates(const B2DecideArgs& a, int n, bool vol) {
+  constexpr int kWords = sizeof(B2SplitCand) / 8;
+  static_assert(sizeof(B2SplitCand) % 8 == 0, "candidates are copied as 64-bit words");
+  static_assert(offsetof(B2SplitCand, loss_chg) == 0 && offsetof(B2SplitCand, feature) == 4 && offsetof(B2SplitCand, order) == 32,
+                "key words of a candidate");
+  const int lane = threadIdx.x & 31, per_node = a.cand_ranks * a.cands_per_node;
+  for (int i = threadIdx.x >> 5; i < n; i += kThreads / 32) {
+    unsigned long long mine = 0ull;
+    const B2SplitCand* mine_c = nullptr;
+    for (int j = lane; j < per_node; j += 32) {
+      const int w = j / a.cands_per_node, g = j - w * a.cands_per_node;
+      const B2SplitCand* c = a.cands + (size_t)w * a.cand_rank_stride + (size_t)i * a.cands_per_node + g;
+      const unsigned long long w0 = cand_word(c, 0, vol);
+      if ((int32_t)(uint32_t)(w0 >> 32) < 0) continue;
+      const unsigned long long key = ((w0 & 0xffffffffull) << 32) | (0xffffffffull - (cand_word(c, 4, vol) & 0xffffffffull));
+      if (key > mine) { mine = key; mine_c = c; }
+    }
+    unsigned long long kmax = mine;
+#pragma unroll
+    for (int o = 16; o > 0; o >>= 1) {
+      const unsigned long long other = __shfl_xor_sync(0xffffffffu, kmax, o);
+      kmax = other > kmax ? other : kmax;
+    }
+    if (kmax == 0ull) {
+      if (lane == 0) { B2SplitCand& e = a.cand_best[i]; e.feature = -1; e.loss_chg = 0.f; e.order = 0xffffffffu; e.is_cat = 0; }
+    } else if (mine == kmax) {
+      unsigned long long* dst = reinterpret_cast<unsigned long long*>(a.cand_best + i);
+#pragma unroll
+      for (int t = 0; t < kWords; ++t) dst[t] = cand_word(mine_c, t, vol);
+    }
+  }
+}
+
+template <int kThreads>
+__device__ __forceinline__ void decide_block(DecideScratch<kThreads>& sm, const B2DecideArgs& a, bool use_p2p, const B2P2P& pp) {
+  const B2TreeDev& tree = a.tree;
+  const B2CtlParams& p = a.p;
+  const int n = a.ctl_cur->n_nodes;
+  if (a.part_counters) for (int i = threadIdx.x; i < 2 * n; i += kThreads) a.part_counters[i] = 0;
+  if (use_p2p && a.can_split) {
+    constexpr int kWords = sizeof(B2SplitCand) / 8;
+    const uint32_t epoch = p2p_next_epoch(pp, kSlotCand);
+    const int total = n * a.cands_per_node * kWords;
+    for (int w = 0; w < pp.world; ++w) {
+      long long* dst = reinterpret_cast<long long*>(pp.cands[w] + (size_t)pp.rank * pp.cand_cap);
+      for (int t = threadIdx.x; t < total; t += kThreads) st_volatile_u64(dst + t, reinterpret_cast<const long long*>(a.local_cands)[t]);
+    }
+    __syncthreads();
+    p2p_signal(pp, kSlotCand, epoch);
+    p2p_wait(pp, kSlotCand, epoch);
+    p2p_finish_single(pp, kSlotCand, epoch);
+  }
+  if (a.can_split) select_candidates<kThreads>(a, n, use_p2p);
+  const double inv_sg = ldexp(1.0, a.qexp[0] - a.qbits), inv_sh = ldexp(1.0, a.qexp[1] - a.qbits);
+  if (threadIdx.x == 0) { sm.node_base = *tree.n_nodes; sm.leaf_base = *a.n_leaves; }
+  __syncthreads();
+  const int node_base = sm.node_base, leaf_base = sm.leaf_base;
+  TileScan<kThreads> scan_split(&sm.scan), scan_leaf(&sm.scan), scan_chunks(&sm.scan);
+  for (int base = 0; base < n; base += kThreads) {
+    const int i = base + threadIdx.x;
+    const bool in = i < n;
+    B2SplitCand best; best.feature = -1; best.loss_chg = 0.f; best.order = 0xffffffffu; best.bin = 0; best.default_left = 0;
+    best.left_g = 0; best.left_h = 0; best.is_cat = 0;
+    B2EvalNode nd; nd.sum_g = 0; nd.sum_h = 0; nd.hist_index = 0; nd.root_gain = 0.f;
+    B2NodeSeg sg; sg.nid = 0; sg.begin = 0; sg.count = 0; sg.buf = 0;
+    bool expand = false;
+    if (in) {
+      nd = a.ev_cur[i]; sg = a.seg_cur[i];
+      if (a.can_split) {
+        best = a.cand_best[i];
+        if (best.feature >= 0)
+          expand = best.loss_chg > 1e-6f && best.left_h != 0 && (nd.sum_h - best.left_h) != 0 && !(best.loss_chg < p.gamma);
+      }
+    }
+    const int rank = scan_split.step(expand ? 1 : 0);
+    const int lrank = scan_leaf.step((in && !expand) ? 1 : 0);
+    const int chunks = expand ? (sg.count + kSplitChunkRows - 1) / kSplitChunkRows : 0;
+    const int chunk_begin = scan_chunks.step(chunks);
+    if (in && !expand) {
+      B2LeafDev lf; lf.nid = sg.nid; lf.buf = sg.buf; lf.begin = sg.begin; lf.count = sg.count;
+      a.leaves[leaf_base + lrank] = lf;
+    }
+    if (expand) {
+      const int l = node_base + 2 * rank, r = l + 1;
+      const int nid = sg.nid;
+      tree.left[nid] = l; tree.right[nid] = r; tree.feature[nid] = best.feature; tree.split_bin[nid] = best.bin;
+      tree.default_left[nid] = best.default_left; tree.loss_chg[nid] = best.loss_chg;
+      tree.split_type[nid] = best.is_cat;
+      if (best.is_cat) {
+#pragma unroll
+        for (int w8 = 0; w8 < 8; ++w8) tree.cat_bits[(size_t)nid * 8 + w8] = best.cat_bits[w8];
+      }
+      tree.left[l] = -1; tree.right[l] = -1; tree.feature[l] = -1; tree.parent[l] = nid;
+      tree.left[r] = -1; tree.right[r] = -1; tree.feature[r] = -1; tree.parent[r] = nid;
+      const long long lg = best.left_g, lh = best.left_h, rg = nd.sum_g - lg, rh = nd.sum_h - lh;
+      tree.sum_g[l] = lg; tree.sum_h[l] = lh; tree.sum_g[r] = rg; tree.sum_h[r] = rh;
+      B2SplitWork sw;
+      sw.seg_begin = sg.begin; sw.seg_count = sg.count; sw.feature = best.feature; sw.split_bin = best.bin;
+      sw.default_left = best.default_left; sw.has_missing = a.has_missing[best.feature]; sw.chunk_begin = chunk_begin;
+      sw.is_cat = best.is_cat;
+#pragma unroll
+      for (int w8 = 0; w8 < 8; ++w8) sw.cat_bits[w8] = best.is_cat ? best.cat_bits[w8] : 0u;
+      a.split_work[rank] = sw;
+      a.pair_parent_hist[rank] = nd.hist_index;
+      const double GL = __dmul_rn(__ll2double_rn(lg), inv_sg), HL = __dmul_rn(__ll2double_rn(lh), inv_sh);
+      const double GR = __dmul_rn(__ll2double_rn(rg), inv_sg), HR = __dmul_rn(__ll2double_rn(rh), inv_sh);
+      B2EvalNode el, er;
+      el.sum_g = lg; el.sum_h = lh; el.hist_index = -1; el.root_gain = __double2float_rn(c_calc_gain(GL, HL, p));
+      er.sum_g = rg; er.sum_h = rh; er.hist_index = -1; er.root_gain = __double2float_rn(c_calc_gain(GR, HR, p));
+      a.ev_nxt[2 * rank] = el; a.ev_nxt[2 * rank + 1] = er;
+      B2NodeSeg sl, sr;
+      sl.nid = l; sl.buf = sg.buf ^ 1; sl.begin = sg.begin; sl.count = 0;
+      sr.nid = r; sr.buf = sg.buf ^ 1; sr.begin = sg.begin; sr.count = sg.count;
+      a.seg_nxt[2 * rank] = sl; a.seg_nxt[2 * rank + 1] = sr;
+    }
+  }
+  __syncthreads();
+  if (threadIdx.x == 0) {
+    const int n_split = scan_split.carry;
+    a.ctl_cur->n_split = n_split; a.ctl_cur->part_chunks = scan_chunks.carry;
+    a.ctl_cur->leaf_base_next = leaf_base + scan_leaf.carry;
+    a.ctl_nxt->n_nodes = 2 * n_split; a.ctl_nxt->n_split = 0; a.ctl_nxt->part_chunks = 0;
+    a.ctl_nxt->hist_n_work = 0; a.ctl_nxt->hist_total_chunks = 0; a.ctl_nxt->n_pairs = 0;
+    *tree.n_nodes = node_base + 2 * n_split;
+    *a.n_leaves = leaf_base + scan_leaf.carry;
+  }
+}
+
+}
diff --git a/xgboost_ray_b200/csrc/engine.cu b/xgboost_ray_b200/csrc/engine.cu
--- a/xgboost_ray_b200/csrc/engine.cu
+++ b/xgboost_ray_b200/csrc/engine.cu
@@ -32,7 +32,9 @@
 int b2_launch_hist_subtract(const long long*, long long*, const int32_t*, int, int64_t, const B2LevelCtl*, cudaStream_t);
 int b2_launch_eval_splits(const long long*, int, const B2EvalNode*, int, const int32_t*, const int32_t*, const int32_t*,
                           const uint8_t*, const uint8_t*, const int32_t*, int, B2TrainParamDev, B2SplitCand*, int, const B2LevelCtl*,
-                          int, int, B2ColSample, const B2NodeSeg*, B2SiblingSub, cudaStream_t);
+                          int, int, B2ColSample, const B2NodeSeg*, B2SiblingSub, const B2DecideArgs*, uint32_t*, cudaStream_t);
+int b2_eval_ctas_per_node(int, int, int);
+int b2_eval_narrow_max_nodes();
 int b2_launch_subsample(float2*, int64_t, uint32_t, uint32_t, uint32_t, double, int, cudaStream_t);
 int b2_p2p_flag_words(int);
 int b2_launch_p2p_reduce_subtract(const void*, const long long*, long long*, const int32_t*, const B2LevelCtl*, int, int, int64_t, int,
@@ -64,9 +66,7 @@
                         long long*, uint16_t*, int, cudaStream_t);
 int b2_launch_pred_update(float*, int, int, const int32_t*, const int32_t*, const void*, const B2LevelCtl*, int, const float*, int,
                           cudaStream_t);
-int b2_launch_decide(B2LevelCtl*, B2LevelCtl*, const B2NodeSeg*, B2NodeSeg*, const B2EvalNode*, B2EvalNode*, const B2SplitCand*,
-                     int, int, int, int, B2TreeDev, B2SplitWork*, int32_t*, B2LeafDev*, int32_t*, const uint8_t*, const int32_t*, int,
-                     B2CtlParams, int32_t*, const B2SplitCand*, const void*, cudaStream_t);
+int b2_launch_decide(const B2DecideArgs*, const void*, cudaStream_t);
 int b2_launch_leaf_plan(const B2LeafDev*, const int32_t*, B2SegWork*, B2LevelCtl*, cudaStream_t);
 int b2_launch_leaf_values(const B2LeafDev*, const int32_t*, const long long*, const int32_t*, int, B2CtlParams, float*, B2TreeDev,
                           int32_t*, cudaStream_t);
@@ -771,6 +771,8 @@
   DevBuf<B2HistWork> d_hist_work; DevBuf<B2SplitWork> d_split_work; DevBuf<B2SegWork> d_seg_work;
   DevBuf<B2SplitCand> d_cands; DevBuf<int32_t> d_counters, d_triples, d_pair_parent;
   DevBuf<uint32_t> d_part_done;
+  DevBuf<uint32_t> d_eval_done;
+  DevBuf<B2SplitCand> d_cand_best;
   DevBuf<B2LeafDev> d_leaves;
   DevBuf<long long> d_leaf_sums; DevBuf<float> d_leaf_values; DevBuf<double> d_metric;
   std::vector<void*> staging;
@@ -1050,6 +1052,8 @@
   b->d_hist_work.ensure(half); b->d_split_work.ensure(half);
   b->d_counters.ensure(2 * half); b->d_triples.ensure(3 * half); b->d_pair_parent.ensure(half);
   if (!b->d_part_done.p) { b->d_part_done.ensure(1); CUDA_CHECK(cudaMemsetAsync(b->d_part_done.p, 0, sizeof(uint32_t), b->ctx->stream)); }
+  if (!b->d_eval_done.p) { b->d_eval_done.ensure(1); CUDA_CHECK(cudaMemsetAsync(b->d_eval_done.p, 0, sizeof(uint32_t), b->ctx->stream)); }
+  b->d_cand_best.ensure(half);
   b->d_leaves.ensure(L.max_nodes); b->d_seg_work.ensure(L.max_nodes);
   b->d_leaf_sums.ensure(2 * lcap); b->d_leaf_values.ensure(lcap);
   b->node_elems = (size_t)G * B2_GROUP_ELEMS;
@@ -1058,7 +1062,7 @@
   b->log2_shards = 0; while ((1 << b->log2_shards) < b->shards) b->log2_shards++;
   b->sp = B2_GROUP_SLOTS / b->shards;
   b->slice_elems = (size_t)G * 2 * B2_BINS * b->sp;
-  b->cpn_num = (G * b->sp + 31) / 32;
+  b->cpn_num = b2_eval_ctas_per_node(G, b->log2_shards, 1);
   b->cpn = b->cpn_num + (b->train->any_cat() ? b2_cat_ctas() : 0);
   b->hist[0].ensure(half * b->slice_elems); b->hist[1].ensure(half * b->slice_elems);
   if (b->shards > 1) {
@@ -1241,8 +1245,18 @@
     const int max_nodes_level = 1 << d;
     const bool can_split = d < D;
     const bool last_split_level = d == D - 1;
-    const B2SplitCand* cands_for_decide = b->d_cands.p;
-    int cand_rank_stride = max_nodes_level * b->cpn;
+    const int cpn_num = b2_eval_ctas_per_node(G, sh, max_nodes_level);
+    const int cpn = cpn_num + (m->any_cat() ? b2_cat_ctas() : 0);
+    B2DecideArgs da;
+    da.ctl_cur = ctl + cur; da.ctl_nxt = ctl + nxt; da.seg_cur = b->d_seg[cur].p; da.seg_nxt = b->d_seg[nxt].p;
+    da.ev_cur = b->d_ev[cur].p; da.ev_nxt = b->d_ev[nxt].p;
+    da.cands = b->d_cands.p; da.cand_best = b->d_cand_best.p; da.local_cands = b->d_cands.p;
+    da.tree = tree; da.split_work = b->d_split_work.p; da.pair_parent_hist = b->d_pair_parent.p; da.leaves = b->d_leaves.p;
+    da.n_leaves = d_n_leaves; da.has_missing = m->d_has_missing.p; da.qexp = b->d_qexp.p;
+    da.part_counters = can_split ? b->d_counters.p : nullptr; da.p = cp;
+    da.cands_per_node = cpn; da.cand_ranks = b->shards; da.cand_rank_stride = max_nodes_level * cpn;
+    da.can_split = can_split ? 1 : 0; da.qbits = p.qbits;
+    const bool fold_decide = can_split && !multi && !m->any_cat() && max_nodes_level <= b2_eval_narrow_max_nodes();
     if (can_split) {
       B2ColSample cs;
       cs.level_mask = p.use_cols() ? b->d_col_masks.p + (size_t)d * m->F : nullptr;
@@ -1256,29 +1270,28 @@
       }
       LAUNCH_CHECK(b2_launch_eval_splits(b->hist[hb].p, G, b->d_ev[cur].p, max_nodes_level, m->d_group_first.p, m->d_group_size.p,
                                          m->d_nbins.p, m->d_has_missing.p, m->any_cat() ? m->d_is_cat.p : nullptr, b->d_qexp.p,
-                                         p.qbits, dp, b->d_cands.p, b->cpn, ctl + cur, sh, shard_rank, cs, b->d_seg[cur].p, sub, s));
+                                         p.qbits, dp, b->d_cands.p, cpn, ctl + cur, sh, shard_rank, cs, b->d_seg[cur].p, sub,
+                                         fold_decide ? &da : nullptr, b->d_eval_done.p, s));
       st.kernel_launches++;
       if (m->any_cat()) {
         LAUNCH_CHECK(b2_launch_eval_cat_splits(b->hist[hb].p, G, b->d_ev[cur].p, max_nodes_level, m->d_cat_feats.p,
                                                (int)m->cat_feats.size(), m->d_feat_byte.p, m->d_nbins.p, b->d_qexp.p, p.qbits, dp,
-                                               b->d_cands.p, b->cpn, b->cpn_num, ctl + cur, sh, shard_rank, cs, b->d_seg[cur].p, s));
+                                               b->d_cands.p, cpn, cpn_num, ctl + cur, sh, shard_rank, cs, b->d_seg[cur].p, s));
         st.kernel_launches++;
       }
       if (p2p) {
-        cands_for_decide = b->d_cands_all.p;
-        cand_rank_stride = b->p2p.cand_cap;
+        da.cands = b->d_cands_all.p;
+        da.cand_rank_stride = b->p2p.cand_cap;
       } else if (b->shards > 1) {
-        const size_t bytes = (size_t)max_nodes_level * b->cpn * sizeof(B2SplitCand);
+        const size_t bytes = (size_t)max_nodes_level * cpn * sizeof(B2SplitCand);
         NCCL_CHECK(nccl()->AllGather(b->d_cands.p, b->d_cands_all.p, bytes, kNcclUint8, b->comm->comm, s));
-        cands_for_decide = b->d_cands_all.p;
+        da.cands = b->d_cands_all.p;
       }
     }
-    LAUNCH_CHECK(b2_launch_decide(ctl + cur, ctl + nxt, b->d_seg[cur].p, b->d_seg[nxt].p, b->d_ev[cur].p, b->d_ev[nxt].p,
-                                  cands_for_decide, b->cpn, b->shards, cand_rank_stride, can_split ? 1 : 0, tree,
-                                  b->d_split_work.p, b->d_pair_parent.p, b->d_leaves.p,
-                                  d_n_leaves, m->d_has_missing.p, b->d_qexp.p, p.qbits, cp, can_split ? b->d_counters.p : nullptr, b->d_cands.p,
-                                  (p2p && can_split) ? &b->p2p.pp : nullptr, s));
-    st.kernel_launches++;
+    if (!fold_decide) {
+      LAUNCH_CHECK(b2_launch_decide(&da, (p2p && can_split) ? &b->p2p.pp : nullptr, s));
+      st.kernel_launches++;
+    }
     mark_phase(b, 4);
     if (!can_split) break;
     const int32_t* ridx_in = d == 0 ? nullptr : b->ridx[cur].p;
diff --git a/xgboost_ray_b200/csrc/partition_kernel.cu b/xgboost_ray_b200/csrc/partition_kernel.cu
--- a/xgboost_ray_b200/csrc/partition_kernel.cu
+++ b/xgboost_ray_b200/csrc/partition_kernel.cu
@@ -235,11 +235,11 @@
 #pragma unroll
       for (int k = 0; k < kBatch; ++k) {
         const int r = r0 + k * kPartThreads;
-        rid[k] = r < nrows ? (kRoot ? w.seg_begin + row0 + r : __ldg(ridx_in + w.seg_begin + row0 + r)) : -1;
+        rid[k] = r < nrows ? (kRoot ? w.seg_begin + row0 + r : __ldcs(ridx_in + w.seg_begin + row0 + r)) : -1;
       }
 #pragma unroll
       for (int k = 0; k < kBatch; ++k) {
-        bin[k] = (int)__ldg(col + (rid[k] < 0 ? 0 : rid[k]));
+        bin[k] = (int)__ldcs(col + (rid[k] < 0 ? 0 : rid[k]));
         if (kSums) v[k] = __ldg(gh + (rid[k] < 0 ? 0 : rid[k]));
       }
 #pragma unroll
diff --git a/xgboost_ray_b200/csrc/split_kernel.cu b/xgboost_ray_b200/csrc/split_kernel.cu
--- a/xgboost_ray_b200/csrc/split_kernel.cu
+++ b/xgboost_ray_b200/csrc/split_kernel.cu
@@ -1,6 +1,9 @@
+#include <string.h>
+
 #include <cub/block/block_scan.cuh>
 
 #include "common.cuh"
+#include "decide.cuh"
 #include "sampling.cuh"
 
 namespace b2 {
@@ -21,11 +24,211 @@
   if (key > b.key) { b.key = key; b.bin = bin; b.default_left = dl; b.lg = lg; b.lh = lh; }
 }
 
-constexpr int kEvalChunks = 32;
-constexpr int kEvalBinsPerChunk = 256 / kEvalChunks;
-
-__global__ void __launch_bounds__(32 * kEvalChunks)
+constexpr int kEvalSlots = 4;
+constexpr int kEvalBinsPerThread = 2;
+constexpr int kEvalThreads = kEvalSlots * B2_BINS / kEvalBinsPerThread;
+constexpr int kEvalWarps = kEvalThreads / 32;
+constexpr int kNarrowMaxNodes = 16;
+
+__host__ __device__ __forceinline__ int eval_ctas_per_node(int n_groups, int sp, int slots) { return (n_groups * sp + slots - 1) / slots; }
+
+__device__ __forceinline__ void write_candidate(B2SplitCand* out, unsigned long long kmax, const Best& best, int f) {
+  if (kmax == 0) {
+    if (threadIdx.x == 0) {
+      out->loss_chg = 0.0f; out->feature = -1; out->bin = 0; out->default_left = 0; out->left_g = 0; out->left_h = 0;
+      out->order = 0xffffffffu; out->is_cat = 0;
+      __threadfence();
+    }
+  } else if (best.key == kmax) {
+    out->loss_chg = __uint_as_float((uint32_t)(kmax >> 32));
+    out->feature = f; out->bin = best.bin; out->default_left = best.default_left;
+    out->left_g = best.lg; out->left_h = best.lh; out->order = 0xffffffffu - (uint32_t)(kmax & 0xffffffffu); out->is_cat = 0;
+    __threadfence();
+  }
+}
+
+template <int kThreads>
+__device__ __forceinline__ void decide_in_last_cta(const B2DecideArgs& dec, uint32_t* done) {
+  __shared__ DecideScratch<kThreads> s_dec;
+  __shared__ bool s_last;
+  __syncthreads();
+  if (threadIdx.x == 0) {
+    const unsigned prev = atomicAdd(done, 1u);
+    s_last = prev == gridDim.x - 1;
+    if (s_last) { __threadfence(); *done = 0u; }
+  }
+  __syncthreads();
+  if (!s_last) return;
+  B2P2P none;
+  memset(&none, 0, sizeof(none));
+  decide_block<kThreads>(s_dec, dec, false, none);
+}
+
+__device__ __forceinline__ void eval_node_cta(const long long* __restrict__ level_hist, int n_groups, const B2EvalNode& nd, int node,
+                                              int cta_in_node, const int32_t* __restrict__ group_first,
+                                              const int32_t* __restrict__ group_size, const int32_t* __restrict__ nbins,
+                                              const uint8_t* __restrict__ has_missing, const uint8_t* __restrict__ is_cat,
+                                              const int32_t* __restrict__ qexp, int qbits, B2TrainParamDev p, B2SplitCand* cands,
+                                              int cand_stride, int log2_shards, int shard_rank, const B2ColSample& cs,
+                                              const B2NodeSeg* __restrict__ seg, const B2SiblingSub& sub) {
+  __shared__ long long s_wg[kEvalWarps][kEvalSlots], s_wh[kEvalWarps][kEvalSlots];
+  __shared__ long long s_tg[kEvalSlots], s_th[kEvalSlots];
+  __shared__ unsigned long long s_key[kEvalWarps];
+  __shared__ uint8_t s_allowed[kEvalSlots];
+  const int sp = B2_GROUP_SLOTS >> log2_shards;
+  const int lane = threadIdx.x & 31, warp = threadIdx.x >> 5;
+  const int s = threadIdx.x & (kEvalSlots - 1), b0 = (threadIdx.x / kEvalSlots) * kEvalBinsPerThread;
+  p.inv_scale_g = ldexp(1.0, qexp[0] - qbits);
+  p.inv_scale_h = ldexp(1.0, qexp[1] - qbits);
+  const int v = cta_in_node * kEvalSlots + s;
+  const bool v_ok = v < n_groups * sp;
+  const int group = v_ok ? v / sp : 0, sl = v_ok ? v % sp : 0;
+  const int slot = (sl << log2_shards) + shard_rank;
+  const size_t slice_elems = (size_t)n_groups * 2 * B2_BINS * sp;
+  const size_t in_slice = (size_t)(group * 2) * B2_BINS * sp + sl;
+  const bool fused = sub.parent_level != nullptr && nd.hist_index >= sub.sib_base;
+  const int pair = fused ? nd.hist_index - sub.sib_base : 0;
+  const long long* hg = level_hist + (size_t)(fused ? sub.triples[3 * pair + 1] : nd.hist_index) * slice_elems + in_slice;
+  const long long* hh = hg + (size_t)B2_BINS * sp;
+  const long long* pgp = fused ? sub.parent_level + (size_t)sub.triples[3 * pair] * slice_elems + in_slice : nullptr;
+  const long long* php = fused ? pgp + (size_t)B2_BINS * sp : nullptr;
+  long long* sgp = (fused && sub.sib_out) ? sub.sib_out + (size_t)nd.hist_index * slice_elems + in_slice : nullptr;
+  long long* shp = sgp ? sgp + (size_t)B2_BINS * sp : nullptr;
+  const int f = group_first[group] + slot;
+  bool active = v_ok && slot < group_size[group] && !(is_cat && is_cat[f]);
+  if (active && cs.level_mask) active = cs.level_mask[f] != 0;
+  if (cs.bynode < 1.0) {
+    if (threadIdx.x < kEvalSlots)
+      s_allowed[s] = active && b2_col_selected(cs.seed, cs.tree, B2_SCOPE_NODE(seg[node].nid), f, cs.level_mask, cs.fwq,
+                                               cs.n_features, b2_sample_count(cs.bynode, cs.n_level));
+    __syncthreads();
+    active = active && s_allowed[s];
+  }
+  const int nf = active ? nbins[f] : 0;
+  const bool fmiss = active ? (has_missing[f] != 0) : false;
+
+  long long g[kEvalBinsPerThread], h[kEvalBinsPerThread];
+#pragma unroll
+  for (int i = 0; i < kEvalBinsPerThread; ++i) { g[i] = 0; h[i] = 0; }
+  if (fused) {
+    if (v_ok && (sgp || active)) {
+#pragma unroll
+      for (int i = 0; i < kEvalBinsPerThread; ++i) {
+        const int b = b0 + i;
+        g[i] = pgp[b * sp] - hg[b * sp]; h[i] = php[b * sp] - hh[b * sp];
+      }
+      if (sgp) {
+#pragma unroll
+        for (int i = 0; i < kEvalBinsPerThread; ++i) { sgp[(b0 + i) * sp] = g[i]; shp[(b0 + i) * sp] = h[i]; }
+      }
+#pragma unroll
+      for (int i = 0; i < kEvalBinsPerThread; ++i)
+        if (b0 + i >= nf) { g[i] = 0; h[i] = 0; }
+    }
+  } else if (active) {
+#pragma unroll
+    for (int i = 0; i < kEvalBinsPerThread; ++i) {
+      const int b = b0 + i;
+      if (b < nf) { g[i] = hg[b * sp]; h[i] = hh[b * sp]; }
+    }
+  }
+  long long tg = 0, th = 0;
+#pragma unroll
+  for (int i = 0; i < kEvalBinsPerThread; ++i) { tg += g[i]; th += h[i]; }
+  long long ig = tg, ih = th;
+#pragma unroll
+  for (int o = kEvalSlots; o < 32; o <<= 1) {
+    const long long ug = __shfl_up_sync(0xffffffffu, ig, o), uh = __shfl_up_sync(0xffffffffu, ih, o);
+    if (lane >= o) { ig += ug; ih += uh; }
+  }
+  if (lane >= 32 - kEvalSlots) { s_wg[warp][s] = ig; s_wh[warp][s] = ih; }
+  __syncthreads();
+  if (threadIdx.x < kEvalSlots) {
+    long long cg = 0, ch = 0;
+#pragma unroll
+    for (int w = 0; w < kEvalWarps; ++w) {
+      const long long a = s_wg[w][threadIdx.x], c = s_wh[w][threadIdx.x];
+      s_wg[w][threadIdx.x] = cg; s_wh[w][threadIdx.x] = ch;
+      cg += a; ch += c;
+    }
+    s_tg[threadIdx.x] = cg; s_th[threadIdx.x] = ch;
+  }
+  __syncthreads();
+  long long pg = s_wg[warp][s] + ig - tg, ph = s_wh[warp][s] + ih - th;
+  const long long real_g = s_tg[s], real_h = s_th[s];
+  const long long tot_g = nd.sum_g, tot_h = nd.sum_h;
+  const double G = __dmul_rn(__ll2double_rn(tot_g), p.inv_scale_g), H = __dmul_rn(__ll2double_rn(tot_h), p.inv_scale_h);
+  const double root_gain = (double)nd.root_gain;
+  const bool node_has_missing = fmiss && (real_g != tot_g || real_h != tot_h);
+  Best best; best.key = 0; best.bin = 0; best.default_left = 0; best.lg = 0; best.lh = 0;
+#pragma unroll
+  for (int i = 0; i < kEvalBinsPerThread; ++i) {
+    const int b = b0 + i;
+    if (b >= nf) break;
+    const long long eg_excl = pg, eh_excl = ph;
+    pg += g[i]; ph += h[i];
+    {
+      const double lh_d = __dmul_rn(__ll2double_rn(ph), p.inv_scale_h);
+      if (lh_d >= p.min_child_weight) {
+        const double rh_d = __dadd_rn(H, -lh_d);
+        if (rh_d >= p.min_child_weight) {
+          const double lg_d = __dmul_rn(__ll2double_rn(pg), p.inv_scale_g);
+          const double rg_d = __dadd_rn(G, -lg_d);
+          const double gain = __dadd_rn(__dadd_rn(calc_gain(lg_d, lh_d, p), calc_gain(rg_d, rh_d, p)), -root_gain);
+          consider(best, __double2float_rn(gain), (uint32_t)f * 1024u + (uint32_t)b, b, 0, pg, ph);
+        }
+      }
+    }
+    if (node_has_missing) {
+      const long long rg_i = real_g - eg_excl, rh_i = real_h - eh_excl;
+      const double rh_d = __dmul_rn(__ll2double_rn(rh_i), p.inv_scale_h);
+      if (rh_d >= p.min_child_weight) {
+        const double lh_d = __dadd_rn(H, -rh_d);
+        if (lh_d >= p.min_child_weight) {
+          const double rg_d = __dmul_rn(__ll2double_rn(rg_i), p.inv_scale_g);
+          const double lg_d = __dadd_rn(G, -rg_d);
+          const double gain = __dadd_rn(__dadd_rn(calc_gain(lg_d, lh_d, p), calc_gain(rg_d, rh_d, p)), -root_gain);
+          consider(best, __double2float_rn(gain), (uint32_t)f * 1024u + 512u + (uint32_t)(255 - b), b - 1, 1,
+                   tot_g - rg_i, tot_h - rh_i);
+        }
+      }
+    }
+  }
+  unsigned long long k = best.key;
+#pragma unroll
+  for (int o = 16; o > 0; o >>= 1) {
+    unsigned long long other = __shfl_xor_sync(0xffffffffu, k, o);
+    k = other > k ? other : k;
+  }
+  if (lane == 0) s_key[warp] = k;
+  __syncthreads();
+  unsigned long long kmax = 0;
+#pragma unroll
+  for (int i = 0; i < kEvalWarps; ++i) kmax = s_key[i] > kmax ? s_key[i] : kmax;
+  write_candidate(cands + (size_t)node * cand_stride + cta_in_node, kmax, best, f);
+}
+
+__global__ void __launch_bounds__(kEvalThreads, 2)
 eval_splits_kernel(const long long* __restrict__ level_hist, int n_groups, const B2EvalNode* __restrict__ nodes,
+                   const int32_t* __restrict__ group_first, const int32_t* __restrict__ group_size,
+                   const int32_t* __restrict__ nbins, const uint8_t* __restrict__ has_missing,
+                   const uint8_t* __restrict__ is_cat ,
+                   const int32_t* __restrict__ qexp, int qbits, B2TrainParamDev p, B2SplitCand* cands,
+                   int cand_stride, const B2LevelCtl* ctl, int log2_shards, int shard_rank, B2ColSample cs,
+                   const B2NodeSeg* __restrict__ seg, B2SiblingSub sub, int fold_decide, B2DecideArgs dec, uint32_t* done) {
+  const int cpn = eval_ctas_per_node(n_groups, B2_GROUP_SLOTS >> log2_shards, kEvalSlots);
+  const int node = blockIdx.x / cpn;
+  if (!ctl || node < ctl->n_nodes)
+    eval_node_cta(level_hist, n_groups, nodes[node], node, blockIdx.x % cpn, group_first, group_size, nbins, has_missing, is_cat,
+                  qexp, qbits, p, cands, cand_stride, log2_shards, shard_rank, cs, seg, sub);
+  if (fold_decide) decide_in_last_cta<kEvalThreads>(dec, done);
+}
+
+constexpr int kWideChunks = 32;
+constexpr int kWideBinsPerChunk = 256 / kWideChunks;
+
+__global__ void __launch_bounds__(32 * kWideChunks)
+eval_splits_wide_kernel(const long long* __restrict__ level_hist, int n_groups, const B2EvalNode* __restrict__ nodes,
                    const int32_t* __restrict__ group_first, const int32_t* __restrict__ group_size,
                    const int32_t* __restrict__ nbins, const uint8_t* __restrict__ has_missing,
                    const uint8_t* __restrict__ is_cat ,
@@ -37,8 +240,8 @@
   const int node = blockIdx.x / cpn, cta_in_node = blockIdx.x % cpn;
   if (ctl && node >= ctl->n_nodes) return;
   const int s = threadIdx.x & 31, q = threadIdx.x >> 5;
-  __shared__ long long cs_g[kEvalChunks][32], cs_h[kEvalChunks][32];
-  __shared__ unsigned long long wkey[kEvalChunks];
+  __shared__ long long cs_g[kWideChunks][32], cs_h[kWideChunks][32];
+  __shared__ unsigned long long wkey[kWideChunks];
   const B2EvalNode nd = nodes[node];
   p.inv_scale_g = ldexp(1.0, qexp[0] - qbits);
   p.inv_scale_h = ldexp(1.0, qexp[1] - qbits);
@@ -74,8 +277,8 @@
   if (fused) {
     if (v_ok && (sgp || active)) {
 #pragma unroll
-      for (int i = 0; i < kEvalBinsPerChunk; ++i) {
-        const int b = q * kEvalBinsPerChunk + i;
+      for (int i = 0; i < kWideBinsPerChunk; ++i) {
+        const int b = q * kWideBinsPerChunk + i;
         const long long g = pgp[b * sp] - hg[b * sp], h = php[b * sp] - hh[b * sp];
         if (sgp) { sgp[b * sp] = g; shp[b * sp] = h; }
         if (active && b < nf) { sg += g; sh += h; }
@@ -83,8 +286,8 @@
     }
   } else if (active) {
 #pragma unroll
-    for (int i = 0; i < kEvalBinsPerChunk; ++i) {
-      int b = q * kEvalBinsPerChunk + i;
+    for (int i = 0; i < kWideBinsPerChunk; ++i) {
+      int b = q * kWideBinsPerChunk + i;
       if (b < nf) { sg += hg[b * sp]; sh += hh[b * sp]; }
     }
   }
@@ -92,7 +295,7 @@
   __syncthreads();
   long long pg = 0, ph = 0, real_g = 0, real_h = 0;
 #pragma unroll 8
-  for (int k = 0; k < kEvalChunks; ++k) {
+  for (int k = 0; k < kWideChunks; ++k) {
     long long a = cs_g[k][s], b = cs_h[k][s];
     if (k < q) { pg += a; ph += b; }
     real_g += a; real_h += b;
@@ -104,8 +307,8 @@
   Best best; best.key = 0; best.bin = 0; best.default_left = 0; best.lg = 0; best.lh = 0;
   if (active) {
 #pragma unroll 2
-    for (int i = 0; i < kEvalBinsPerChunk; ++i) {
-      const int b = q * kEvalBinsPerChunk + i;
+    for (int i = 0; i < kWideBinsPerChunk; ++i) {
+      const int b = q * kWideBinsPerChunk + i;
       if (b >= nf) break;
       const long long eg_excl = pg, eh_excl = ph;
       if (!fused) { pg += hg[b * sp]; ph += hh[b * sp]; }
@@ -149,7 +352,7 @@
   __syncthreads();
   unsigned long long kmax = 0;
 #pragma unroll 8
-  for (int i = 0; i < kEvalChunks; ++i) kmax = wkey[i] > kmax ? wkey[i] : kmax;
+  for (int i = 0; i < kWideChunks; ++i) kmax = wkey[i] > kmax ? wkey[i] : kmax;
   B2SplitCand* out = cands + (size_t)node * cand_stride + cta_in_node;
   if (kmax == 0) {
     if (threadIdx.x == 0) {
@@ -353,16 +556,31 @@
 }
 
 extern "C" {
+int b2_eval_ctas_per_node(int n_groups, int log2_shards, int max_nodes) {
+  return b2::eval_ctas_per_node(n_groups, B2_GROUP_SLOTS >> log2_shards, max_nodes <= b2::kNarrowMaxNodes ? b2::kEvalSlots : 32);
+}
+int b2_eval_narrow_max_nodes() { return b2::kNarrowMaxNodes; }
 int b2_launch_eval_splits(const long long* level_hist, int n_groups, const B2EvalNode* nodes, int n_nodes,
                           const int32_t* group_first, const int32_t* group_size, const int32_t* nbins,
                           const uint8_t* has_missing, const uint8_t* is_cat, const int32_t* qexp, int qbits, B2TrainParamDev p,
                           B2SplitCand* cands, int cand_stride, const B2LevelCtl* ctl, int log2_shards, int shard_rank,
-                          B2ColSample cs, const B2NodeSeg* seg, B2SiblingSub sub, cudaStream_t stream) {
+                          B2ColSample cs, const B2NodeSeg* seg, B2SiblingSub sub, const B2DecideArgs* dec, uint32_t* done,
+                          cudaStream_t stream) {
   if (n_nodes <= 0) return 0;
-  const int sp = B2_GROUP_SLOTS >> log2_shards, cpn = (n_groups * sp + 31) >> 5;
-  b2::eval_splits_kernel<<<n_nodes * cpn, 32 * b2::kEvalChunks, 0, stream>>>(level_hist, n_groups, nodes, group_first, group_size,
-                                                                         nbins, has_missing, is_cat, qexp, qbits, p, cands,
-                                                                         cand_stride, ctl, log2_shards, shard_rank, cs, seg, sub);
+  B2DecideArgs d;
+  if (dec) d = *dec; else memset(&d, 0, sizeof(d));
+  const int cpn = b2_eval_ctas_per_node(n_groups, log2_shards, n_nodes);
+  if (n_nodes <= b2::kNarrowMaxNodes)
+    b2::eval_splits_kernel<<<n_nodes * cpn, b2::kEvalThreads, 0, stream>>>(level_hist, n_groups, nodes, group_first, group_size,
+                                                                           nbins, has_missing, is_cat, qexp, qbits, p, cands,
+                                                                           cand_stride, ctl, log2_shards, shard_rank, cs, seg, sub,
+                                                                           dec ? 1 : 0, d, done);
+  else if (dec) return (int)cudaErrorInvalidValue;
+  else
+    b2::eval_splits_wide_kernel<<<n_nodes * cpn, 32 * b2::kWideChunks, 0, stream>>>(level_hist, n_groups, nodes, group_first,
+                                                                                     group_size, nbins, has_missing, is_cat, qexp,
+                                                                                     qbits, p, cands, cand_stride, ctl,
+                                                                                     log2_shards, shard_rank, cs, seg, sub);
   return (int)cudaGetLastError();
 }
 int b2_cat_ctas() { return b2::kCatCtas; }
```
